# ZrrSkywalker/MonoDETR

Hardware: AMD Instinct MI355X
Metric: training images/sec at B=8 per GPU, KITTI 384x1280 (higher is better)
Workload: dtype bf16; 1 GPU; full MonoDETR training step (ResNet-50 + depth predictor + 3 enc / 3 dec layers, 550 train queries, 4 levels, criterion + AdamW) = BASELINE configs[2] (1 GPU) / configs[3] (DDP); global_batch=8, per_gpu_batch=8, image=3x384x1280, queries=50, precision=bf16, parallelism=dp1, grad_sync=none, prime_steps=12, launch=one hipGraph replay per iteration, cpu_affinity=NUMA node 1 of the GPU

## Files before the change

include/monodetr_amd.h:

```cpp
#ifndef MONODETR_AMD_H
#define MONODETR_AMD_H

#include <stdint.h>

#ifdef __cplusplus
extern "C" {
#endif

#define MDETR_ABI_VERSION 13

#define MDETR_F32 0
#define MDETR_F64 1
#define MDETR_BF16 2

#define MDETR_OK            0
#define MDETR_E_ARG        -1
#define MDETR_E_HIP        -2
#define MDETR_E_ALIGN      -3

int mdetr_abi_version(void);
const char *mdetr_last_error(void);

int mdetr_msda_forward(int dtype,
                       const void *value, const int64_t *spatial_shapes, const int64_t *level_start,
                       const void *loc, const void *attn, void *out,
                       int B, int S, int M, int D, int L, int Lq, int P,
                       int device, void *stream);

int mdetr_msda_backward(int dtype,
                        const void *value, const int64_t *spatial_shapes, const int64_t *level_start,
                        const void *loc, const void *attn, const void *grad_out,
                        void *grad_value, void *grad_loc, void *grad_attn,
                        int B, int S, int M, int D, int L, int Lq, int P,
                        int device, void *stream);

int mdetr_msda_forward_cpu(int dtype,
                           const void *value, const int64_t *spatial_shapes, const int64_t *level_start,
                           const void *loc, const void *attn, void *out,
                           int B, int S, int M, int D, int L, int Lq, int P);
int mdetr_msda_backward_cpu(int dtype,
                            const void *value, const int64_t *spatial_shapes, const int64_t *level_start,
                            const void *loc, const void *attn, const void *grad_out,
                            void *grad_value, void *grad_loc, void *grad_attn,
                            int B, int S, int M, int D, int L, int Lq, int P);

int mdetr_msda_backward_ex(int dtype,
                           const void *value, const int64_t *spatial_shapes, const int64_t *level_start,
                           const void *loc, const void *attn, const void *grad_out,
                           void *grad_value, void *grad_loc, void *grad_attn,
                           int B, int S, int M, int D, int L, int Lq, int P,
                           const int64_t *spatial_shapes_host, const int64_t *level_start_host,
                           void *workspace, int64_t workspace_bytes,
                           int device, void *stream);

int64_t mdetr_msda_backward_workspace_bytes(int dtype, const int64_t *spatial_shapes_host,
                                            const int64_t *level_start_host,
                                            int B, int S, int M, int D, int L, int Lq, int P);

int mdetr_msda_indices(int dtype, const int64_t *spatial_shapes, const void *loc, int32_t *idx,
                       int B, int M, int L, int Lq, int P, int device, void *stream);

int mdetr_msda_variant(int dtype, int M, int D, int L, int P);

int mdetr_attn_forward(int dtype, const void *q, const void *k, const void *v, const uint8_t *key_padding_mask,
                       void *out, float *lse, int B, int H, int Lq, int Lk,
                       int64_t q_bs, int64_t k_bs, int64_t v_bs, int q_rs, int k_rs, int v_rs,
                       float scale, float dropout_p, uint64_t seed, const uint64_t *seed_dev, int device, void *stream);

int mdetr_attn_backward(int dtype, const void *q, const void *k, const void *v, const uint8_t *key_padding_mask,
                        const void *out, const void *d_out, const float *lse, float *dsum,
                        void *dq, void *dk, void *dv, int B, int H, int Lq, int Lk,
                        int64_t q_bs, int64_t k_bs, int64_t v_bs, int q_rs, int k_rs, int v_rs,
                        float scale, float dropout_p, uint64_t seed, const uint64_t *seed_dev, int device, void *stream);

int64_t mdetr_pair_losses_workspace_bytes(int L, int B);
int mdetr_pair_losses_forward(const float *logits, const float *boxes, const float *dims, const float *depths,
                              const float *angles, const int32_t *assign, const int64_t *labels, const float *boxes3d,
                              const float *depth, const float *size3d, const int64_t *heading_bin,
                              const float *heading_res, const uint8_t *valid, const int32_t *num,
                              int L, int B, int Q, int C, int G, int K, float focal_alpha,
                              float num_boxes, const float *num_boxes_dev, float *out, float *comp, void *workspace,
                              int device, void *stream);
int mdetr_pair_losses_backward(const float *logits, const float *boxes, const float *dims, const float *depths,
                               const float *angles, const int32_t *assign, const int64_t *labels, const float *boxes3d,
                               const float *depth, const float *size3d, const int64_t *heading_bin,
                               const float *heading_res, const uint8_t *valid,
                               int L, int B, int Q, int C, int G, int K, float focal_alpha,
                               float num_boxes, const float *num_boxes_dev, const float *grad_out, const float *comp,
                               float *g_logits, float *g_boxes, float *g_dims, float *g_depths, float *g_angles,
                               int device, void *stream);

int mdetr_msda_forward_bf16(const void *value, const int64_t *spatial_shapes, const int64_t *level_start,
                            const float *loc, const float *attn, void *out,
                            int B, int S, int M, int D, int L, int Lq, int P, int device, void *stream);
int mdetr_msda_backward_bf16(const void *value, const int64_t *spatial_shapes, const int64_t *level_start,
                             const float *loc, const float *attn, const void *grad_out,
                             float *grad_value, float *grad_loc, float *grad_attn,
                             int B, int S, int M, int D, int L, int Lq, int P,
                             const int64_t *spatial_shapes_host, const int64_t *level_start_host,
                             void *workspace, int64_t workspace_bytes, int device, void *stream);

int mdetr_msda_prologue_forward(int io_dtype, int ref_dtype, const void *offsets, const void *logits, const void *ref,
                                const int64_t *spatial_shapes, float *sampling_loc, float *attn_weight,
                                int B, int Lq, int M, int L, int P, int R, int64_t ref_sb, int64_t ref_sq, int64_t ref_sl,
                                int device, void *stream);
int mdetr_msda_prologue_backward(int io_dtype, int ref_dtype, const void *offsets, const void *ref, const int64_t *spatial_shapes,
                                 const float *attn_weight, const float *grad_loc, const float *grad_attn,
                                 void *grad_offsets, void *grad_logits, float *grad_ref,
                                 int B, int Lq, int M, int L, int P, int R, int64_t ref_sb, int64_t ref_sq, int64_t ref_sl,
                                 int device, void *stream);
int mdetr_msda_prologue_forward_packed(int io_dtype, int ref_dtype, const void *packed, const void *ref, const int64_t *spatial_shapes,
                                       float *sampling_loc, float *attn_weight, int B, int Lq, int M, int L, int P, int R,
                                       int64_t ref_sb, int64_t ref_sq, int64_t ref_sl, int device, void *stream);
int mdetr_msda_prologue_backward_packed(int io_dtype, int ref_dtype, const void *packed, const void *ref, const int64_t *spatial_shapes,
                                        const float *attn_weight, const float *grad_loc, const float *grad_attn, void *grad_packed,
                                        float *grad_ref, int B, int Lq, int M, int L, int P, int R,
                                        int64_t ref_sb, int64_t ref_sq, int64_t ref_sl, int device, void *stream);

int mdetr_lsa_forward_fused(const float *logits, const float *boxes, const int64_t *labels, const float *boxes3d,
                            const int32_t *num_targets, int32_t *assign, int layers, int images, int groups, int n,
                            int kmax, int num_classes, float w_class, float w_bbox, float w_center, float w_giou,
                            float focal_alpha, int device, void *stream);

int mdetr_ddn_loss_forward(const float *logits, const float *boxes, const float *depth, const uint8_t *valid,
                           int B, int C, int H, int W, int K, int64_t sb, int64_t sc, int64_t sh, int64_t sw,
                           float alpha, float fg_weight, float bg_weight, float depth_min, float depth_max,
                           float *out, void *workspace, int device, void *stream);
int mdetr_ddn_loss_backward(const float *logits, const float *boxes, const float *depth, const uint8_t *valid,
                            int B, int C, int H, int W, int K, int64_t sb, int64_t sc, int64_t sh, int64_t sw,
                            float alpha, float fg_weight, float bg_weight, float depth_min, float depth_max,
                            const float *grad_out, float *grad_logits, int device, void *stream);

int mdetr_adamw_step(int param_dtype, void *param, float *master, const void *grad, float *exp_avg, float *exp_avg_sq,
                     int64_t n, int64_t n_no_decay, float beta1, float beta2, float eps, float weight_decay,
                     float step_size, const float *step_size_dev, int device, void *stream);
int mdetr_adamw_step_counted(int param_dtype, void *param, float *master, const void *grad, float *exp_avg, float *exp_avg_sq,
                             int64_t n, int64_t n_no_decay, float beta1, float beta2, float eps, float weight_decay,
                             const double *step_count_dev, float lr, const double *lr_dev, int device, void *stream);
int mdetr_adamw_step_gathered(int param_dtype, void *param, float *master, const void *const *grad_ptrs, int ntensors,
                              const int *tensor_block_begin, const int64_t *flat_offsets, const int64_t *nbytes, const int *block_tensor,
                              const int64_t *block_start, int chunk_bytes, float *exp_avg, float *exp_avg_sq, int64_t n_no_decay,
                              float beta1, float beta2, float eps, float weight_decay, float step_size, const float *step_size_dev,
                              const double *step_count_dev, float lr, const double *lr_dev, int device, void *stream);

#define MDETR_TGEMM_RELU 1
#define MDETR_TGEMM_NN 2
#define MDETR_TGEMM_BIAS_F32 4
#define MDETR_TGEMM_OUT_F32 8
int mdetr_tgemm(const void *a, const void *w, const void *bias, const void *res, void *y, int64_t T, int N, int K,
                int64_t lda, int64_t ldw, int64_t ldr, int64_t ldy, int flags, float dropout_p, uint64_t seed,
                const void *seed_dev, int device, void *stream);
int mdetr_tgemm_masked(const void *a, const void *w, const void *res, const void *mask, void *y, int64_t T, int N, int K,
                       int64_t lda, int64_t ldw, int64_t ldr, int64_t ldm, int64_t ldy, int device, void *stream);
int mdetr_tgemm_f32(const void *a, const void *w, const void *bias, const void *res, void *y, int64_t T, int N, int K,
                    int64_t lda, int64_t ldw, int64_t ldr, int64_t ldy, int flags, float dropout_p, uint64_t seed,
                    const void *seed_dev, int device, void *stream);
int mdetr_tgemm_f32_masked(const void *a, const void *w, const void *res, const void *mask, void *y, int64_t T, int N, int K,
                           int64_t lda, int64_t ldw, int64_t ldr, int64_t ldm, int64_t ldy, int device, void *stream);

#define MDETR_SGEMM_NT 0
#define MDETR_SGEMM_NN 1
#define MDETR_SGEMM_TN 2
#define MDETR_SGEMM_MAX_PROBLEMS 10
#define MDETR_SGEMM_MAX_TERMS 5
typedef struct {
    const void *a, *b;
    int64_t lda, ldb;
    int32_t k, a_dtype, b_dtype, pad_;
} mdetr_sgemm_term;
typedef struct {
    mdetr_sgemm_term term[MDETR_SGEMM_MAX_TERMS];
    void *c;
    const float *bias;
    float *colsum;
    const float *mask;
    const void *res;
    int64_t ldc, ldm, ldr;
    int32_t nterm, m, n, relu_cols, c_dtype, res_dtype;
} mdetr_sgemm_problem;
int64_t mdetr_sgemm_workspace_bytes(int mode, const mdetr_sgemm_problem *problems, int nprob);
int mdetr_sgemm_grouped(int mode, const mdetr_sgemm_problem *problems, int nprob, void *workspace, int64_t workspace_bytes, int device, void *stream);

#define MDETR_KITTI_FLIP 1u
#define MDETR_KITTI_DISTORT 2u
#define MDETR_KITTI_CONTRAST_FIRST 4u
#define MDETR_KITTI_BRIGHTNESS 8u
#define MDETR_KITTI_CONTRAST 16u
#define MDETR_KITTI_SATURATION 32u
#define MDETR_KITTI_HUE 64u
typedef struct MdetrKittiImage {
    int64_t pixel_offset;
    int32_t width, height;
    uint32_t flags;
    uint32_t perm;
    float brightness, contrast, saturation, hue;
    double inv[6];
} MdetrKittiImage;
int mdetr_kitti_preprocess(const uint8_t *pixels, const MdetrKittiImage *images, int n_images, void *out,
                           int out_dtype, int out_h, int out_w, int channels_last, const float *mean, const float *std,
                           int device, void *stream);

int mdetr_rotate_iou_eval(const float *boxes, const float *qboxes, const int64_t *box_start, const int64_t *qbox_start,
                          const int64_t *out_start, int n_frames, int64_t total_pairs, int criterion, float *out,
                          int device, void *stream);
int mdetr_box3d_overlap_eval(const double *boxes, const double *qboxes, const int64_t *box_start, const int64_t *qbox_start,
                             const int64_t *out_start, int n_frames, int64_t total_pairs, int criterion, double *out,
                             int device, void *stream);
int mdetr_kitti_pr_curve(const double *overlaps, const int64_t *ov_start, const double *gt_datas, const double *dt_datas,
                         const int64_t *gt_start, const int64_t *dt_start, const int64_t *ignored_gt,
                         const int64_t *ignored_det, const double *dontcares, const int64_t *dc_start, int n_frames,
                         int metric, double min_overlap, int64_t num_valid_gt, int compute_aos, int max_thresholds,
                         double *pr, double *thresholds, int *n_thresholds);

int mdetr_add_layernorm_forward(int io_dtype, int param_dtype, const void *a, const void *b, const void *gamma, const void *beta, void *y,
                                void *s, float *stats, int64_t rows, int cols, float eps, float dropout_p, uint64_t seed,
                                const uint64_t *seed_dev, int device, void *stream);
int64_t mdetr_add_layernorm_partial_rows(int64_t rows);
int mdetr_add_layernorm_backward(int io_dtype, int param_dtype, const void *dy, const void *s, const void *gamma, const float *stats,
                                 void *da, void *db, float *partial, int64_t rows, int cols, float dropout_p,
                                 uint64_t seed, const uint64_t *seed_dev, int device, void *stream);

int64_t mdetr_column_sum_workspace_bytes(int64_t rows, int cols);
int mdetr_column_sum(int dtype, const void *x, float *out, void *workspace, int64_t workspace_bytes,
                     int64_t rows, int cols, int64_t ld, int device, void *stream);
int mdetr_box_refine(const float *delta, const float *ref, float *out, int64_t rows, int nd, int device, void *stream);
int mdetr_head_tail_forward(const float *delta, const float *init_ref, const float *inter_refs, const float *size3d, const float *depth_reg,
                            const float *depth_map, const float *img_h, const float *focal, float *coord, float *depth_ave,
                            int L, int B, int Q, int nd0, int H, int W, int device, void *stream);
int mdetr_head_tail_backward(const float *init_ref, const float *size3d, const float *depth_reg, const float *img_h, const float *focal,
                             const float *coord, const float *g_coord, const float *g_depth, float *g_delta, float *g_init_ref,
                             float *g_size3d, float *g_depth_reg, float *g_map, int L, int B, int Q, int nd0, int H, int W, int device, void *stream);

typedef struct {
    const float *part;
    void *out;
    int64_t cols;
    int32_t chunks, out_dtype;
} mdetr_chunk_job;
int mdetr_chunk_sums(const mdetr_chunk_job *jobs, int njobs, int device, void *stream);
int mdetr_column_sum_to(int dtype, const void *x, void *out, int out_dtype, void *workspace, int64_t workspace_bytes,
                        int64_t rows, int cols, int64_t ld, int device, void *stream);

int mdetr_conv3x3_forward(const void *x, const void *w, const float *shift, void *y, int B, int H, int W, int C, int N,
                          int relu, int device, void *stream);
int mdetr_conv3x3_plan(int B, int H, int W, int N);
int mdetr_conv3x3_masked(const void *x, const void *w, const float *shift, const void *mask, void *y, int B, int H, int W, int C, int N,
                         int relu, int device, void *stream);

int mdetr_conv_taps(const void *x, const void *w, const float *shift, void *y, const int64_t *dims, int relu, int device, void *stream);

int mdetr_conv_taps_split(const void *x, const void *w, const float *shift, float *partial, int64_t partial_floats, const int64_t *dims,
                          int ksplit, int device, void *stream);

int mdetr_conv_dgrad_s2(const void *dy, const void *wt, void *dx, int B, int OH, int OW, int N, int H, int W, int C, int K, int device, void *stream);

int mdetr_conv_stem(const void *x, const void *w_packed, const float *shift, void *y, int B, int H, int W, int device, void *stream);

int mdetr_conv_wgrad_chunks(int B, int H, int W, int C, int OH, int OW, int N, int K, int SI);
int mdetr_conv_wgrad(const void *x, const void *dy, float *partial, int64_t partial_floats, int B, int H, int W, int C, int OH, int OW, int N,
                     int K, int SI, int device, void *stream);

int mdetr_token_wgrad_chunks(int64_t T, int C, int N);
int mdetr_token_wgrad(const void *x, const void *dy, float *partial, int64_t partial_floats, int64_t T, int C, int N, int with_bias,
                      int device, void *stream);

int mdetr_bias_act_forward(int io_dtype, int bias_dtype, const void *x, const void *bias, const void *skip, void *y,
                           int64_t rows, int cols, int relu, float dropout_p, uint64_t seed, const uint64_t *seed_dev,
                           int device, void *stream);
int mdetr_bias_act_backward(int io_dtype, const void *dy, const void *y, void *dx, int64_t rows, int cols, float scale,
                            int device, void *stream);

int mdetr_fold_weights(int n, const void *const *w, const void *const *scale, void *const *folded, void *const *folded_t,
                       const int *O, const int *C, const int *taps, int device, void *stream);
int mdetr_unfold_grads(int n, const void *const *dfolded, const void *const *scale, void *const *dw,
                       const int *O, const int *C, const int *taps, int device, void *stream);

int mdetr_gather_flat(const void *const *src_ptrs, int ntensors, const int *tensor_block_begin, void *dst, const int64_t *dst_offsets,
                      const int64_t *nbytes, const int *block_tensor, const int64_t *block_start, int chunk_bytes, int device, void *stream);

int mdetr_maxpool3x3s2_bf16(const void *x, void *y, int B, int H, int W, int C, int device, void *stream);
int mdetr_decimate2(int backward, const void *src, void *dst, int B, int H, int W, int64_t pixel_bytes, int device, void *stream);

int64_t mdetr_small_wgrad_workspace_bytes(int64_t rows, int n, int k);
int mdetr_small_wgrad(int io_dtype, const void *dy, const void *x, void *out, int out_dtype, void *workspace, int64_t workspace_bytes,
                      int64_t rows, int n, int k, int64_t ldy, int64_t ldx, int device, void *stream);

int64_t mdetr_group_norm_workspace_bytes(int n, int64_t hw, int c, int groups);
int mdetr_group_norm_forward(int io_dtype, int param_dtype, const void *x, const void *gamma, const void *beta, void *y, float *stats,
                             void *workspace, int64_t workspace_bytes, int n, int64_t hw, int c, int groups, float eps, int relu,
                             int device, void *stream);
int mdetr_group_norm_backward(int io_dtype, int param_dtype, const void *dy, const void *x, const void *gamma, const void *beta,
                              const float *stats, void *dx, void *dparams, void *workspace, int64_t workspace_bytes,
                              int n, int64_t hw, int c, int groups, int relu, int device, void *stream);

int mdetr_lsa_forward(const float *cost, const int32_t *num_targets, int32_t *assign,
                      int layers, int images, int groups, int n, int kmax,
                      int64_t img_stride, int64_t q_stride, int64_t t_stride, int device, void *stream);

int mdetr_profile_enable(int on);
int mdetr_profile_read(double *rows, int cap);
int mdetr_profile_read_work(double *rows, int cap);

#ifdef __cplusplus
}
#endif
#endif
```

monodetr_amd/_capi.py:

```python
import ctypes
import os
import threading

_HERE = os.path.dirname(os.path.abspath(__file__))
LIB_PATH = os.environ.get("MDETR_LIB_PATH") or os.path.join(_HERE, "libmonodetr_amd.so")

MDETR_F32, MDETR_F64, MDETR_BF16 = 0, 1, 2
ABI_VERSION = 13

_c_int, _c_vp = ctypes.c_int, ctypes.c_void_p

SIGNATURES = {
    "mdetr_abi_version": (_c_int, []),
    "mdetr_last_error": (ctypes.c_char_p, []),
    "mdetr_msda_variant": (_c_int, [_c_int] * 5),
    "mdetr_msda_forward": (_c_int, [_c_int] + [_c_vp] * 6 + [_c_int] * 7 + [_c_int, _c_vp]),
    "mdetr_msda_backward": (_c_int, [_c_int] + [_c_vp] * 9 + [_c_int] * 7 + [_c_int, _c_vp]),
    "mdetr_msda_forward_cpu": (_c_int, [_c_int] + [_c_vp] * 6 + [_c_int] * 7),
    "mdetr_msda_backward_cpu": (_c_int, [_c_int] + [_c_vp] * 9 + [_c_int] * 7),
    "mdetr_msda_backward_ex": (_c_int, [_c_int] + [_c_vp] * 9 + [_c_int] * 7 + [_c_vp, _c_vp, _c_vp, ctypes.c_int64] + [_c_int, _c_vp]),
    "mdetr_msda_backward_workspace_bytes": (ctypes.c_int64, [_c_int, _c_vp, _c_vp] + [_c_int] * 7),
    "mdetr_msda_indices": (_c_int, [_c_int] + [_c_vp] * 3 + [_c_int] * 5 + [_c_int, _c_vp]),
    "mdetr_attn_forward": (_c_int, [_c_int] + [_c_vp] * 6 + [_c_int] * 4 + [ctypes.c_int64] * 3 + [_c_int] * 3
                           + [ctypes.c_float, ctypes.c_float, ctypes.c_uint64, _c_vp, _c_int, _c_vp]),
    "mdetr_attn_backward": (_c_int, [_c_int] + [_c_vp] * 11 + [_c_int] * 4 + [ctypes.c_int64] * 3 + [_c_int] * 3
                            + [ctypes.c_float, ctypes.c_float, ctypes.c_uint64, _c_vp, _c_int, _c_vp]),
    "mdetr_lsa_forward": (_c_int, [_c_vp] * 3 + [_c_int] * 5 + [ctypes.c_int64] * 3 + [_c_int, _c_vp]),
    "mdetr_ddn_loss_forward": (_c_int, [_c_vp] * 4 + [_c_int] * 5 + [ctypes.c_int64] * 4 + [ctypes.c_float] * 5 + [_c_vp, _c_vp, _c_int, _c_vp]),
    "mdetr_ddn_loss_backward": (_c_int, [_c_vp] * 4 + [_c_int] * 5 + [ctypes.c_int64] * 4 + [ctypes.c_float] * 5 + [_c_vp, _c_vp, _c_int, _c_vp]),
    "mdetr_pair_losses_workspace_bytes": (ctypes.c_int64, [_c_int, _c_int]),
    "mdetr_pair_losses_forward": (_c_int, [_c_vp] * 14 + [_c_int] * 6 + [ctypes.c_float, ctypes.c_float] + [_c_vp] * 4 + [_c_int, _c_vp]),
    "mdetr_pair_losses_backward": (_c_int, [_c_vp] * 13 + [_c_int] * 6 + [ctypes.c_float, ctypes.c_float] + [_c_vp] * 8 + [_c_int, _c_vp]),
    "mdetr_adamw_step": (_c_int, [_c_int] + [_c_vp] * 5 + [ctypes.c_int64] * 2 + [ctypes.c_float] * 5 + [_c_vp, _c_int, _c_vp]),
    "mdetr_adamw_step_gathered": (_c_int, [_c_int, _c_vp, _c_vp, _c_vp, _c_int] + [_c_vp] * 5 + [_c_int, _c_vp, _c_vp, ctypes.c_int64] + [ctypes.c_float] * 5
                                  + [_c_vp, _c_vp, ctypes.c_float, _c_vp, _c_int, _c_vp]),
    "mdetr_adamw_step_counted": (_c_int, [_c_int] + [_c_vp] * 5 + [ctypes.c_int64] * 2 + [ctypes.c_float] * 4 + [_c_vp, ctypes.c_float, _c_vp, _c_int, _c_vp]),
    "mdetr_tgemm": (_c_int, [_c_vp] * 5 + [ctypes.c_int64, _c_int, _c_int] + [ctypes.c_int64] * 4 + [_c_int, ctypes.c_float, ctypes.c_uint64, _c_vp, _c_int, _c_vp]),
    "mdetr_sgemm_workspace_bytes": (ctypes.c_int64, [_c_int, _c_vp, _c_int]),
    "mdetr_sgemm_grouped": (_c_int, [_c_int, _c_vp, _c_int, _c_vp, ctypes.c_int64, _c_int, _c_vp]),
    "mdetr_tgemm_masked": (_c_int, [_c_vp] * 5 + [ctypes.c_int64, _c_int, _c_int] + [ctypes.c_int64] * 5 + [_c_int, _c_vp]),
    "mdetr_tgemm_f32": (_c_int, [_c_vp] * 5 + [ctypes.c_int64, _c_int, _c_int] + [ctypes.c_int64] * 4 + [_c_int, ctypes.c_float, ctypes.c_uint64, _c_vp, _c_int, _c_vp]),
    "mdetr_tgemm_f32_masked": (_c_int, [_c_vp] * 5 + [ctypes.c_int64, _c_int, _c_int] + [ctypes.c_int64] * 5 + [_c_int, _c_vp]),
    "mdetr_column_sum_workspace_bytes": (ctypes.c_int64, [ctypes.c_int64, _c_int]),
    "mdetr_column_sum": (_c_int, [_c_int, _c_vp, _c_vp, _c_vp, ctypes.c_int64, ctypes.c_int64, _c_int, ctypes.c_int64, _c_int, _c_vp]),
    "mdetr_box_refine": (_c_int, [_c_vp] * 3 + [ctypes.c_int64, _c_int, _c_int, _c_vp]),
    "mdetr_head_tail_forward": (_c_int, [_c_vp] * 10 + [_c_int] * 6 + [_c_int, _c_vp]),
    "mdetr_head_tail_backward": (_c_int, [_c_vp] * 13 + [_c_int] * 6 + [_c_int, _c_vp]),
    "mdetr_chunk_sums": (_c_int, [_c_vp, _c_int, _c_int, _c_vp]),
    "mdetr_column_sum_to": (_c_int, [_c_int, _c_vp, _c_vp, _c_int, _c_vp, ctypes.c_int64, ctypes.c_int64, _c_int, ctypes.c_int64, _c_int, _c_vp]),
    "mdetr_add_layernorm_forward": (_c_int, [_c_int, _c_int] + [_c_vp] * 7 + [ctypes.c_int64, _c_int, ctypes.c_float, ctypes.c_float, ctypes.c_uint64, _c_vp, _c_int, _c_vp]),
    "mdetr_add_layernorm_partial_rows": (ctypes.c_int64, [ctypes.c_int64]),
    "mdetr_add_layernorm_backward": (_c_int, [_c_int, _c_int] + [_c_vp] * 7 + [ctypes.c_int64, _c_int, ctypes.c_float, ctypes.c_uint64, _c_vp, _c_int, _c_vp]),
    "mdetr_conv3x3_forward": (_c_int, [_c_vp] * 4 + [_c_int] * 6 + [_c_int, _c_vp]),
    "mdetr_conv3x3_plan": (_c_int, [_c_int] * 4),
    "mdetr_conv3x3_masked": (_c_int, [_c_vp] * 5 + [_c_int] * 6 + [_c_int, _c_vp]),
    "mdetr_conv_taps": (_c_int, [_c_vp] * 5 + [_c_int, _c_int, _c_vp]),
    "mdetr_conv_taps_split": (_c_int, [_c_vp] * 4 + [ctypes.c_int64, _c_vp, _c_int, _c_int, _c_vp]),
    "mdetr_conv_dgrad_s2": (_c_int, [_c_vp] * 3 + [_c_int] * 8 + [_c_int, _c_vp]),
    "mdetr_conv_stem": (_c_int, [_c_vp] * 4 + [_c_int] * 3 + [_c_int, _c_vp]),
    "mdetr_conv_wgrad_chunks": (_c_int, [_c_int] * 9),
    "mdetr_conv_wgrad": (_c_int, [_c_vp] * 3 + [ctypes.c_int64] + [_c_int] * 9 + [_c_int, _c_vp]),
    "mdetr_token_wgrad_chunks": (_c_int, [ctypes.c_int64, _c_int, _c_int]),
    "mdetr_token_wgrad": (_c_int, [_c_vp, _c_vp, _c_vp, ctypes.c_int64, ctypes.c_int64, _c_int, _c_int, _c_int, _c_int, _c_vp]),
    "mdetr_small_wgrad_workspace_bytes": (ctypes.c_int64, [ctypes.c_int64, _c_int, _c_int]),
    "mdetr_small_wgrad": (_c_int, [_c_int, _c_vp, _c_vp, _c_vp, _c_int, _c_vp, ctypes.c_int64, ctypes.c_int64, _c_int, _c_int, ctypes.c_int64, ctypes.c_int64, _c_int, _c_vp]),
    "mdetr_group_norm_workspace_bytes": (ctypes.c_int64, [_c_int, ctypes.c_int64, _c_int, _c_int]),
    "mdetr_group_norm_forward": (_c_int, [_c_int, _c_int] + [_c_vp] * 6 + [ctypes.c_int64, _c_int, ctypes.c_int64, _c_int, _c_int, ctypes.c_float, _c_int, _c_int, _c_vp]),
    "mdetr_group_norm_backward": (_c_int, [_c_int, _c_int] + [_c_vp] * 8 + [ctypes.c_int64, _c_int, ctypes.c_int64, _c_int, _c_int, _c_int, _c_int, _c_vp]),
    "mdetr_bias_act_forward": (_c_int, [_c_int, _c_int] + [_c_vp] * 4 + [ctypes.c_int64, _c_int, _c_int, ctypes.c_float, ctypes.c_uint64, _c_vp, _c_int, _c_vp]),
    "mdetr_bias_act_backward": (_c_int, [_c_int] + [_c_vp] * 3 + [ctypes.c_int64, _c_int, ctypes.c_float, _c_int, _c_vp]),
    "mdetr_rotate_iou_eval": (_c_int, [_c_vp] * 5 + [_c_int, ctypes.c_int64, _c_int, _c_vp, _c_int, _c_vp]),
    "mdetr_box3d_overlap_eval": (_c_int, [_c_vp] * 5 + [_c_int, ctypes.c_int64, _c_int, _c_vp, _c_int, _c_vp]),
    "mdetr_kitti_pr_curve": (_c_int, [_c_vp] * 10 + [_c_int, _c_int, ctypes.c_double, ctypes.c_int64, _c_int, _c_int, _c_vp, _c_vp, _c_vp]),
    "mdetr_kitti_preprocess": (_c_int, [_c_vp, _c_vp, _c_int, _c_vp, _c_int, _c_int, _c_int, _c_int, _c_vp, _c_vp, _c_int, _c_vp]),
    "mdetr_msda_forward_bf16": (_c_int, [_c_vp] * 6 + [_c_int] * 7 + [_c_int, _c_vp]),
    "mdetr_msda_backward_bf16": (_c_int, [_c_vp] * 9 + [_c_int] * 7 + [_c_vp, _c_vp, _c_vp, ctypes.c_int64, _c_int, _c_vp]),
    "mdetr_msda_prologue_forward": (_c_int, [_c_int, _c_int] + [_c_vp] * 6 + [_c_int] * 6 + [ctypes.c_int64] * 3 + [_c_int, _c_vp]),
    "mdetr_gather_flat": (_c_int, [_c_vp, _c_int] + [_c_vp] * 6 + [_c_int, _c_int, _c_vp]),
    "mdetr_fold_weights": (_c_int, [_c_int] + [_c_vp] * 7 + [_c_int, _c_vp]),
    "mdetr_unfold_grads": (_c_int, [_c_int] + [_c_vp] * 6 + [_c_int, _c_vp]),
    "mdetr_maxpool3x3s2_bf16": (_c_int, [_c_vp, _c_vp, _c_int, _c_int, _c_int, _c_int, _c_int, _c_vp]),
    "mdetr_decimate2": (_c_int, [_c_int, _c_vp, _c_vp, _c_int, _c_int, _c_int, ctypes.c_int64, _c_int, _c_vp]),
    "mdetr_msda_prologue_forward_packed": (_c_int, [_c_int, _c_int] + [_c_vp] * 5 + [_c_int] * 6 + [ctypes.c_int64] * 3 + [_c_int, _c_vp]),
    "mdetr_msda_prologue_backward_packed": (_c_int, [_c_int, _c_int] + [_c_vp] * 8 + [_c_int] * 6 + [ctypes.c_int64] * 3 + [_c_int, _c_vp]),
    "mdetr_msda_prologue_backward": (_c_int, [_c_int, _c_int] + [_c_vp] * 9 + [_c_int] * 6 + [ctypes.c_int64] * 3 + [_c_int, _c_vp]),
    "mdetr_lsa_forward_fused": (_c_int, [_c_vp] * 6 + [_c_int] * 6 + [ctypes.c_float] * 5 + [_c_int, _c_vp]),
    "mdetr_profile_enable": (_c_int, [_c_int]),
    "mdetr_profile_read": (_c_int, [_c_vp, _c_int]),
    "mdetr_profile_read_work": (_c_int, [_c_vp, _c_int]),
}

_lib = None
_lock = threading.Lock()


def lib():
    global _lib
    if _lib is None:
        with _lock:
            if _lib is None:
                if not os.path.exists(LIB_PATH):
                    raise RuntimeError(
                        "monodetr_amd: %s is missing -- the HIP extension is not built. Run "
                        "`python -m monodetr_amd.build` (needs hipcc). There is no CPU/PyTorch fallback." % LIB_PATH)
                handle = ctypes.CDLL(LIB_PATH)
                for name, (res, args) in SIGNATURES.items():
                    fn = getattr(handle, name)
                    fn.restype, fn.argtypes = res, args
                got = handle.mdetr_abi_version()
                if got != ABI_VERSION:
                    raise RuntimeError("monodetr_amd: ABI version mismatch (lib %d, python %d); rebuild" % (got, ABI_VERSION))
                _lib = handle
    return _lib


def check(rc, what):
    if rc != 0:
        msg = lib().mdetr_last_error()
        raise RuntimeError("%s failed (code %d): %s" % (what, rc, msg.decode() if msg else "?"))


def dtype_code(t):
    import torch
    if t.dtype == torch.float32:
        return MDETR_F32
    if t.dtype == torch.float64:
        return MDETR_F64
    raise RuntimeError('"ms_deform_attn" not implemented for \'%s\'' % str(t.dtype).replace("torch.", ""))


def profile_enable(on):
    check(lib().mdetr_profile_enable(1 if on else 0), "mdetr_profile_enable")


def profile_read(cap=64):
    buf = (ctypes.c_double * (4 * cap))()
    n = lib().mdetr_profile_read(ctypes.cast(buf, ctypes.c_void_p), cap)
    if n < 0:
        check(n, "mdetr_profile_read")
    return [(int(buf[4 * i]), int(buf[4 * i + 1]), int(buf[4 * i + 2]), float(buf[4 * i + 3])) for i in range(n)]


def profile_read_work(cap=256):
    buf = (ctypes.c_double * (6 * cap))()
    n = lib().mdetr_profile_read_work(ctypes.cast(buf, ctypes.c_void_p), cap)
    if n < 0:
        check(n, "mdetr_profile_read_work")
    return [(int(buf[6 * i]), int(buf[6 * i + 1]), int(buf[6 * i + 2]), float(buf[6 * i + 3]), float(buf[6 * i + 4]), float(buf[6 * i + 5])) for i in range(n)]
```

monodetr_amd/add_ln_ext.py:

```python
import os

import torch
import torch.nn.functional as F

from . import _capi
from .attn_ext import _next_seed

_backend = None
ENABLED = os.environ.get("MDETR_FUSED_LN") == "1"


_seed_counter = None


def _host_seed():
    global _seed_counter
    if _seed_counter is None:
        _seed_counter = int(torch.randint(0, 2 ** 62, (1,), dtype=torch.int64))
    _seed_counter = (_seed_counter + 0x9E3779B97F4A7C15) & 0x7FFFFFFFFFFFFFFF
    return _seed_counter


def _lib():
    return _backend if _backend is not None else _capi.lib()


def supported(a, b, norm):
    return ((a.is_cuda or _backend is not None) and a.dtype in (torch.float32, torch.bfloat16) and b.dtype == a.dtype
            and a.shape == b.shape and a.shape[-1] in (128, 256, 512) and len(norm.normalized_shape) == 1
            and norm.normalized_shape[0] == a.shape[-1] and norm.elementwise_affine and norm.bias is not None)


def _rows(t, C):
    t = t.reshape(-1, C).contiguous()
    return t if t.data_ptr() % 16 == 0 else t.clone()


def _dev(t):
    cuda = t.is_cuda
    return (t.device.index if cuda else -1), (torch.cuda.current_stream(t.device).cuda_stream if cuda else None)


def _column_sum_f32(x, out_dtype=torch.float32):
    if x.is_cuda and _backend is None:
        from .colsum_ext import column_sum
        return column_sum(x, out_dtype if out_dtype in (torch.float32, torch.bfloat16) else torch.float32)
    return x.sum(0).to(out_dtype)


class _AddLayerNorm(torch.autograd.Function):
    @staticmethod
    def forward(ctx, a, b, gamma, beta, eps, p, seed, seed_dev):
        shape = a.shape
        C = shape[-1]
        a2, b2 = _rows(a, C), _rows(b, C)
        rows = a2.shape[0]
        if gamma.dtype == beta.dtype and gamma.dtype in (torch.float32, torch.bfloat16):
            gp, bp = gamma.contiguous(), beta.contiguous()
        else:
            gp, bp = gamma.float().contiguous(), beta.float().contiguous()
        pcode = _capi.MDETR_BF16 if gp.dtype == torch.bfloat16 else _capi.MDETR_F32
        y, s = torch.empty_like(a2), torch.empty_like(a2)
        stats = torch.empty((rows, 2), dtype=torch.float32, device=a.device)
        io = _capi.MDETR_BF16 if a.dtype == torch.bfloat16 else _capi.MDETR_F32
        dev, stream = _dev(a2)
        rc = _lib().mdetr_add_layernorm_forward(io, pcode, a2.data_ptr(), b2.data_ptr(), gp.data_ptr(), bp.data_ptr(), y.data_ptr(), s.data_ptr(),
                                                stats.data_ptr(), rows, C, float(eps), float(p), int(seed),
                                                seed_dev.data_ptr() if seed_dev is not None else None, dev, stream)
        if rc != 0:
            _capi.check(rc, "mdetr_add_layernorm_forward")
        ctx.save_for_backward(s, gp, stats)
        ctx.seed_dev = seed_dev
        ctx.meta = (io, pcode, rows, C, float(p), int(seed), shape, gamma.dtype, beta.dtype)
        return y.view(shape)

    @staticmethod
    @torch.autograd.function.once_differentiable
    def backward(ctx, dy):
        s, gp, stats = ctx.saved_tensors
        io, pcode, rows, C, p, seed, shape, g_dtype, b_dtype = ctx.meta
        dy2 = _rows(dy, C)
        da, db = torch.empty_like(s), torch.empty_like(s)
        lib = _lib()
        nb = lib.mdetr_add_layernorm_partial_rows(rows)
        partial = torch.empty((nb, 2 * C), dtype=torch.float32, device=s.device)
        dev, stream = _dev(s)
        rc = lib.mdetr_add_layernorm_backward(io, pcode, dy2.data_ptr(), s.data_ptr(), gp.data_ptr(), stats.data_ptr(), da.data_ptr(), db.data_ptr(),
                                              partial.data_ptr(), rows, C, p, seed,
                                              ctx.seed_dev.data_ptr() if ctx.seed_dev is not None else None, dev, stream)
        if rc != 0:
            _capi.check(rc, "mdetr_add_layernorm_backward")
        sums = _column_sum_f32(partial, g_dtype if g_dtype == b_dtype else torch.float32)
        return da.view(shape), db.view(shape), sums[:C].to(g_dtype), sums[C:].to(b_dtype), None, None, None, None


def fused_add_layernorm(a, b, gamma, beta, eps=1e-5, dropout_p=0.0, seed=None):
    seed_dev = None
    if dropout_p > 0.0 and seed is None:
        if a.is_cuda and torch.cuda.is_current_stream_capturing():
            from .attn_ext import site_seed
            seed, seed_dev = site_seed(a.device)
        else:
            seed = _host_seed()
    return _AddLayerNorm.apply(a, b, gamma, beta, eps, dropout_p, seed or 0, seed_dev)


def residual_layernorm(a, b, norm, dropout):
    if ENABLED and supported(a, b, norm):
        p = dropout.p if (dropout is not None and dropout.training) else 0.0
        return fused_add_layernorm(a, b, norm.weight, norm.bias, norm.eps, p)
    return norm(a + (dropout(b) if dropout is not None else b))
```

monodetr_amd/csrc/add_ln.hip:

```cpp
#include <hip/hip_runtime.h>
#include <hip/hip_bf16.h>
#include <stdint.h>

#include "add_ln.h"
#include "add_ln_math.h"

namespace mdetr {
namespace {

constexpr int kWavesLn = 4;
constexpr int kMaxBwdBlocks = 1024;

template <typename T> __device__ __forceinline__ float ld1(const T *p);
template <> __device__ __forceinline__ float ld1<float>(const float *p) { return *p; }
template <> __device__ __forceinline__ float ld1<__hip_bfloat16>(const __hip_bfloat16 *p) { return __bfloat162float(*p); }
template <typename T> __device__ __forceinline__ void st1(T *p, float v);
template <> __device__ __forceinline__ void st1<float>(float *p, float v) { *p = v; }
template <> __device__ __forceinline__ void st1<__hip_bfloat16>(__hip_bfloat16 *p, float v) { *p = __float2bfloat16(v); }

template <typename T, int E> struct alignas(sizeof(T) * E > 16 ? 16 : sizeof(T) * E) RowVec { T v[E]; };

template <typename T, int E> __device__ __forceinline__ void load_row(const T *p, float (&v)[E])
{
    const RowVec<T, E> t = *reinterpret_cast<const RowVec<T, E> *>(p);
#pragma unroll
    for (int i = 0; i < E; ++i) v[i] = ld1<T>(&t.v[i]);
}
template <typename T, int E> __device__ __forceinline__ void store_row(T *p, const float (&v)[E])
{
    RowVec<T, E> t;
#pragma unroll
    for (int i = 0; i < E; ++i) st1<T>(&t.v[i], v[i]);
    *reinterpret_cast<RowVec<T, E> *>(p) = t;
}

__device__ __forceinline__ float wave_sum(float v)
{
#pragma unroll
    for (int o = 32; o > 0; o >>= 1) v += __shfl_xor(v, o);
    return v;
}

template <typename T, typename PT, int E>
__global__ __launch_bounds__(kWavesLn * 64)
void add_ln_fwd_kernel(const T *__restrict__ a, const T *__restrict__ b, const PT *__restrict__ gamma,
                       const PT *__restrict__ beta, T *__restrict__ y, T *__restrict__ s, float *__restrict__ stats,
                       int64_t rows, float eps, uint32_t thresh, float keep_scale, uint64_t seed,
                       const uint64_t *__restrict__ seed_dev)
{
    constexpr int C = 64 * E;
    const int lane = threadIdx.x & 63, wave = threadIdx.x >> 6;
    const int64_t row = static_cast<int64_t>(blockIdx.x) * kWavesLn + wave;
    if (row >= rows) return;
    const uint64_t sd = seed + (seed_dev ? *seed_dev : 0ull);
    const int64_t at = row * C + lane * E;
    float v[E];
    load_row<T, E>(a + at, v);
    if (b) {
        float r[E];
        load_row<T, E>(b + at, r);
#pragma unroll
        for (int i = 0; i < E; ++i) {
            const bool keep = thresh == 0u || ln_hash(sd, static_cast<uint64_t>(at + i)) >= thresh;
            v[i] += keep ? r[i] * keep_scale : 0.f;
        }
        if (s) {
            store_row<T, E>(s + at, v);
#pragma unroll
            for (int i = 0; i < E; ++i) { T t; st1<T>(&t, v[i]); v[i] = ld1<T>(&t); }
        }
    }
    float sum = 0.f;
#pragma unroll
    for (int i = 0; i < E; ++i) sum += v[i];
    const float mean = wave_sum(sum) * (1.0f / C);
    float sq = 0.f;
#pragma unroll
    for (int i = 0; i < E; ++i) { const float d = v[i] - mean; sq += d * d; }
    const float rstd = 1.0f / sqrtf(wave_sum(sq) * (1.0f / C) + eps);
    float o[E];
#pragma unroll
    for (int i = 0; i < E; ++i) o[i] = (v[i] - mean) * rstd * ld1<PT>(gamma + lane * E + i) + ld1<PT>(beta + lane * E + i);
    store_row<T, E>(y + at, o);
    if (lane == 0) { stats[2 * row] = mean; stats[2 * row + 1] = rstd; }
}

template <typename T, typename PT, int E>
__global__ __launch_bounds__(kWavesLn * 64)
void add_ln_bwd_kernel(const T *__restrict__ dy, const T *__restrict__ s, const PT *__restrict__ gamma,
                       const float *__restrict__ stats, T *__restrict__ da, T *__restrict__ db,
                       float *__restrict__ partial, int64_t rows, uint32_t thresh, float keep_scale, uint64_t seed,
                       const uint64_t *__restrict__ seed_dev)
{
    constexpr int C = 64 * E;
    __shared__ float red[kWavesLn][2 * C];
    const int lane = threadIdx.x & 63, wave = threadIdx.x >> 6;
    const uint64_t sd = seed + (seed_dev ? *seed_dev : 0ull);
    float g[E], acc_g[E], acc_b[E];
#pragma unroll
    for (int i = 0; i < E; ++i) { g[i] = ld1<PT>(gamma + lane * E + i); acc_g[i] = 0.f; acc_b[i] = 0.f; }
    for (int64_t row = static_cast<int64_t>(blockIdx.x) * kWavesLn + wave; row < rows; row += static_cast<int64_t>(gridDim.x) * kWavesLn) {
        const int64_t at = row * C + lane * E;
        const float mean = stats[2 * row], rstd = stats[2 * row + 1];
        float d[E], x[E];
        load_row<T, E>(dy + at, d);
        load_row<T, E>(s + at, x);
        float s1 = 0.f, s2 = 0.f;
#pragma unroll
        for (int i = 0; i < E; ++i) {
            x[i] = (x[i] - mean) * rstd;
            acc_g[i] += d[i] * x[i];
            acc_b[i] += d[i];
            d[i] *= g[i];
            s1 += d[i];
            s2 += d[i] * x[i];
        }
        s1 = wave_sum(s1) * (1.0f / C);
        s2 = wave_sum(s2) * (1.0f / C);
        float o[E];
#pragma unroll
        for (int i = 0; i < E; ++i) o[i] = rstd * (d[i] - s1 - x[i] * s2);
        store_row<T, E>(da + at, o);
        if (db) {
#pragma unroll
            for (int i = 0; i < E; ++i) {
                const bool keep = thresh == 0u || ln_hash(sd, static_cast<uint64_t>(at + i)) >= thresh;
                o[i] = keep ? o[i] * keep_scale : 0.f;
            }
            store_row<T, E>(db + at, o);
        }
    }
#pragma unroll
    for (int i = 0; i < E; ++i) { red[wave][lane * E + i] = acc_g[i]; red[wave][C + lane * E + i] = acc_b[i]; }
    __syncthreads();
    for (int c = threadIdx.x; c < 2 * C; c += kWavesLn * 64)
        partial[static_cast<int64_t>(blockIdx.x) * 2 * C + c] = red[0][c] + red[1][c] + red[2][c] + red[3][c];
}

template <typename T, typename PT, int E>
hipError_t launch_fwd(const AddLnProblem &p, const void *a, const void *b, const void *gamma, const void *beta, void *y, void *s,
                      float *stats, hipStream_t st)
{
    const uint32_t thresh = b ? ln_threshold(p.dropout_p) : 0u;
    const float scale = p.dropout_p > 0.f ? 1.0f / (1.0f - p.dropout_p) : 1.0f;
    hipLaunchKernelGGL((add_ln_fwd_kernel<T, PT, E>), dim3(static_cast<unsigned>((p.rows + kWavesLn - 1) / kWavesLn)), dim3(kWavesLn * 64), 0, st,
                       static_cast<const T *>(a), static_cast<const T *>(b), static_cast<const PT *>(gamma), static_cast<const PT *>(beta),
                       static_cast<T *>(y), static_cast<T *>(s), stats,
                       p.rows, p.eps, thresh, scale, p.seed, p.seed_dev);
    return hipGetLastError();
}

template <typename T, typename PT, int E>
hipError_t launch_bwd(const AddLnProblem &p, const void *dy, const void *s, const void *gamma, const float *stats, void *da, void *db,
                      float *partial, hipStream_t st)
{
    const uint32_t thresh = db ? ln_threshold(p.dropout_p) : 0u;
    const float scale = p.dropout_p > 0.f ? 1.0f / (1.0f - p.dropout_p) : 1.0f;
    hipLaunchKernelGGL((add_ln_bwd_kernel<T, PT, E>), dim3(static_cast<unsigned>(add_ln_partial_rows(p.rows))), dim3(kWavesLn * 64), 0, st,
                       static_cast<const T *>(dy), static_cast<const T *>(s), static_cast<const PT *>(gamma), stats, static_cast<T *>(da),
                       static_cast<T *>(db), partial,
                       p.rows, thresh, scale, p.seed, p.seed_dev);
    return hipGetLastError();
}

}

int64_t add_ln_partial_rows(int64_t rows)
{
    const int64_t blocks = (rows + kWavesLn - 1) / kWavesLn;
    return blocks < 1 ? 1 : (blocks > kMaxBwdBlocks ? kMaxBwdBlocks : blocks);
}

template <int E>
hipError_t dispatch_fwd(const AddLnProblem &p, const void *a, const void *b, const void *gamma, const void *beta, void *y, void *s,
                        float *stats, hipStream_t st)
{
    using BF = __hip_bfloat16;
    if (p.io_dtype == 2) return p.param_dtype == 2 ? launch_fwd<BF, BF, E>(p, a, b, gamma, beta, y, s, stats, st) : launch_fwd<BF, float, E>(p, a, b, gamma, beta, y, s, stats, st);
    return p.param_dtype == 2 ? launch_fwd<float, BF, E>(p, a, b, gamma, beta, y, s, stats, st) : launch_fwd<float, float, E>(p, a, b, gamma, beta, y, s, stats, st);
}

template <int E>
hipError_t dispatch_bwd(const AddLnProblem &p, const void *dy, const void *s, const void *gamma, const float *stats, void *da, void *db,
                        float *partial, hipStream_t st)
{
    using BF = __hip_bfloat16;
    if (p.io_dtype == 2) return p.param_dtype == 2 ? launch_bwd<BF, BF, E>(p, dy, s, gamma, stats, da, db, partial, st) : launch_bwd<BF, float, E>(p, dy, s, gamma, stats, da, db, partial, st);
    return p.param_dtype == 2 ? launch_bwd<float, BF, E>(p, dy, s, gamma, stats, da, db, partial, st) : launch_bwd<float, float, E>(p, dy, s, gamma, stats, da, db, partial, st);
}

hipError_t add_ln_forward_launch(const AddLnProblem &p, const void *a, const void *b, const void *gamma, const void *beta,
                                 void *y, void *s, float *stats, hipStream_t st)
{
    if (p.rows == 0) return hipSuccess;
    switch (p.cols) {
    case 128: return dispatch_fwd<2>(p, a, b, gamma, beta, y, s, stats, st);
    case 256: return dispatch_fwd<4>(p, a, b, gamma, beta, y, s, stats, st);
    case 512: return dispatch_fwd<8>(p, a, b, gamma, beta, y, s, stats, st);
    default: return hipErrorNotSupported;
    }
}

hipError_t add_ln_backward_launch(const AddLnProblem &p, const void *dy, const void *s, const void *gamma, const float *stats,
                                  void *da, void *db, float *partial, hipStream_t st)
{
    if (p.rows == 0) return hipSuccess;
    switch (p.cols) {
    case 128: return dispatch_bwd<2>(p, dy, s, gamma, stats, da, db, partial, st);
    case 256: return dispatch_bwd<4>(p, dy, s, gamma, stats, da, db, partial, st);
    case 512: return dispatch_bwd<8>(p, dy, s, gamma, stats, da, db, partial, st);
    default: return hipErrorNotSupported;
    }
}

}
```

monodetr_amd/csrc/add_ln_math.h:

```cpp
#pragma once
#include <stdint.h>

#if defined(__HIPCC__)
#define MDETR_HD __host__ __device__ __forceinline__
#else
#define MDETR_HD inline
#endif

namespace mdetr {

MDETR_HD uint32_t ln_hash(uint64_t seed, uint64_t index)
{
    uint64_t z = index * 0x9E3779B97F4A7C15ull + seed;
    uint32_t x = static_cast<uint32_t>(z) ^ static_cast<uint32_t>(z >> 32);
    x ^= x >> 16;
    x *= 0x7FEB352Du;
    x ^= x >> 15;
    x *= 0x846CA68Bu;
    x ^= x >> 16;
    return x;
}

MDETR_HD uint32_t ln_threshold(float p)
{
    const double t = static_cast<double>(p) * 4294967296.0;
    return t >= 4294967295.0 ? 0xFFFFFFFFu : static_cast<uint32_t>(t);
}

}
```

monodetr_amd/csrc/capi.hip:

```cpp
#include <hip/hip_runtime.h>
#include <stdarg.h>
#include <stdio.h>

#include <atomic>
#include <map>
#include <mutex>
#include <utility>
#include <vector>

#include "../../include/monodetr_amd.h"
#include "attn.h"
#include "adamw.h"
#include "add_ln.h"
#include "bias_act.h"
#include "colsum.h"
#include "group_norm.h"
#include "small_wgrad.h"
#include "decimate.h"
#include "wfold.h"
#include "conv3x3.h"
#include "conv_stem.h"
#include "conv_taps.h"
#include "conv_wgrad.h"
#include "ddn_loss.h"
// ... 394 lines not shown
{
    if (int rc = pair_losses_args("mdetr_pair_losses_backward", L, B, Q, C, G, K)) return rc;
    if (!logits || !boxes || !dims || !depths || !angles || !assign || !labels || !boxes3d || !depth || !size3d ||
        !heading_bin || !heading_res || !valid || !grad_out || !comp || !g_logits || !g_boxes || !g_dims || !g_depths || !g_angles)
        return fail(MDETR_E_ARG, "mdetr_pair_losses_backward: null pointer");
    DeviceScope dev(device);
    if (dev.err != hipSuccess) return fail(MDETR_E_HIP, "mdetr_pair_losses_backward: set device %d: %s", device, hipGetErrorString(dev.err));
    const mdetr::PairLossDims d{L, B, Q, C, G, K, focal_alpha};
    const mdetr::PairLossIn in{logits, boxes, dims, depths, angles, assign, reinterpret_cast<const long long *>(labels),
                               reinterpret_cast<const long long *>(heading_bin), boxes3d, depth, size3d, heading_res, valid};
    const hipError_t e = mdetr::pair_losses_backward_launch(d, in, grad_out, comp, num_boxes, num_boxes_dev, g_logits,
                                                            g_boxes, g_dims, g_depths, g_angles,
                                                            static_cast<hipStream_t>(stream));
    if (e != hipSuccess) return fail(MDETR_E_HIP, "mdetr_pair_losses_backward: launch failed: %s", hipGetErrorString(e));
    return MDETR_OK;
}

int mdetr_adamw_step(int param_dtype, void *param, float *master, const void *grad, float *exp_avg, float *exp_avg_sq,
                     int64_t n, int64_t n_no_decay, float beta1, float beta2, float eps, float weight_decay,
                     float step_size, const float *step_size_dev, int device, void *stream)
{
    if (param_dtype != MDETR_F32 && param_dtype != MDETR_BF16)
        return fail(MDETR_E_ARG, "mdetr_adamw_step: parameter dtype must be f32 or bf16");
    if (n < 0 || n_no_decay < 0 || n_no_decay > n) return fail(MDETR_E_ARG, "mdetr_adamw_step: bad sizes");
    if (n == 0) return MDETR_OK;
    if (!param || !master || !grad || !exp_avg || !exp_avg_sq) return fail(MDETR_E_ARG, "mdetr_adamw_step: null pointer");
    if (param_dtype == MDETR_F32 && static_cast<void *>(master) != param)
        return fail(MDETR_E_ARG, "mdetr_adamw_step: an f32 parameter is its own master copy");
    if (!aligned16(param) || !aligned16(master) || !aligned16(grad) || !aligned16(exp_avg) || !aligned16(exp_avg_sq))
        return fail(MDETR_E_ALIGN, "mdetr_adamw_step: buffers must be 16-byte aligned");
    DeviceScope dev(device);
    if (dev.err != hipSuccess) return fail(MDETR_E_HIP, "mdetr_adamw_step: set device %d: %s", device, hipGetErrorString(dev.err));
    const hipError_t e = mdetr::adamw_launch(param_dtype, param, master, grad, exp_avg, exp_avg_sq, n, n_no_decay,
                                             beta1, beta2, eps, weight_decay, step_size, step_size_dev,
                                             static_cast<hipStream_t>(stream));
    if (e != hipSuccess) return fail(MDETR_E_HIP, "mdetr_adamw_step: launch failed: %s", hipGetErrorString(e));
    return MDETR_OK;
}

int mdetr_adamw_step_counted(int param_dtype, void *param, float *master, const void *grad, float *exp_avg, float *exp_avg_sq,
                             int64_t n, int64_t n_no_decay, float beta1, float beta2, float eps, float weight_decay,
                             const double *step_count_dev, float lr, const double *lr_dev, int device, void *stream)
{
    if (param_dtype != MDETR_F32 && param_dtype != MDETR_BF16)
        return fail(MDETR_E_ARG, "mdetr_adamw_step_counted: parameter dtype must be f32 or bf16");
    if (n < 0 || n_no_decay < 0 || n_no_decay > n) return fail(MDETR_E_ARG, "mdetr_adamw_step_counted: bad sizes");
    if (n == 0) return MDETR_OK;
    if (!param || !master || !grad || !exp_avg || !exp_avg_sq || !step_count_dev) return fail(MDETR_E_ARG, "mdetr_adamw_step_counted: null pointer");
    if (param_dtype == MDETR_F32 && static_cast<void *>(master) != param)
        return fail(MDETR_E_ARG, "mdetr_adamw_step_counted: an f32 parameter is its own master copy");
    if (!aligned16(param) || !aligned16(master) || !aligned16(grad) || !aligned16(exp_avg) || !aligned16(exp_avg_sq))
        return fail(MDETR_E_ALIGN, "mdetr_adamw_step_counted: buffers must be 16-byte aligned");
    DeviceScope dev(device);
    if (dev.err != hipSuccess) return fail(MDETR_E_HIP, "mdetr_adamw_step_counted: set device %d: %s", device, hipGetErrorString(dev.err));
    const hipError_t e = mdetr::adamw_launch(param_dtype, param, master, grad, exp_avg, exp_avg_sq, n, n_no_decay, beta1, beta2, eps,
                                             weight_decay, 0.f, nullptr, static_cast<hipStream_t>(stream), step_count_dev, lr_dev, lr);
    if (e != hipSuccess) return fail(MDETR_E_HIP, "mdetr_adamw_step_counted: launch failed: %s", hipGetErrorString(e));
    return MDETR_OK;
}

int mdetr_adamw_step_gathered(int param_dtype, void *param, float *master, const void *const *grad_ptrs, int ntensors,
                              const int *tensor_block_begin, const int64_t *flat_offsets, const int64_t *nbytes, const int *block_tensor,
                              const int64_t *block_start, int chunk_bytes, float *exp_avg, float *exp_avg_sq, int64_t n_no_decay,
                              float beta1, float beta2, float eps, float weight_decay, float step_size, const float *step_size_dev,
                              const double *step_count_dev, float lr, const double *lr_dev, int device, void *stream)
{
    if (param_dtype != MDETR_F32 && param_dtype != MDETR_BF16)
        return fail(MDETR_E_ARG, "mdetr_adamw_step_gathered: parameter dtype must be f32 or bf16");
    const int esz = param_dtype == MDETR_F32 ? 4 : 2;
    if (ntensors < 0 || n_no_decay < 0 || chunk_bytes <= 0 || chunk_bytes % 16 != 0)
        return fail(MDETR_E_ARG, "mdetr_adamw_step_gathered: ntensors %d / chunk_bytes %d (a positive multiple of 16)", ntensors, chunk_bytes);
    if (ntensors == 0) return MDETR_OK;
    if (!param || !master || !grad_ptrs || !tensor_block_begin || !flat_offsets || !nbytes || !block_tensor || !block_start || !exp_avg || !exp_avg_sq)
        return fail(MDETR_E_ARG, "mdetr_adamw_step_gathered: null pointer");
    if (param_dtype == MDETR_F32 && static_cast<void *>(master) != param)
        return fail(MDETR_E_ARG, "mdetr_adamw_step_gathered: an f32 parameter is its own master copy");
    if (!aligned16(param) || !aligned16(master) || !aligned16(exp_avg) || !aligned16(exp_avg_sq))
        return fail(MDETR_E_ALIGN, "mdetr_adamw_step_gathered: buffers must be 16-byte aligned");
    for (int i = 0; i < ntensors; ++i)
        if ((!grad_ptrs[i] && tensor_block_begin[i + 1] != tensor_block_begin[i]) || tensor_block_begin[i + 1] < tensor_block_begin[i] ||
            (reinterpret_cast<uintptr_t>(grad_ptrs[i]) & (esz - 1)))
            return fail(MDETR_E_ARG, "mdetr_adamw_step_gathered: tensor %d: null / misaligned gradient or decreasing block table", i);
    DeviceScope dev(device);
    if (dev.err != hipSuccess) return fail(MDETR_E_HIP, "mdetr_adamw_step_gathered: set device %d: %s", device, hipGetErrorString(dev.err));
    const hipError_t e = mdetr::adamw_gathered_launch(param_dtype, param, master, grad_ptrs, ntensors, tensor_block_begin, flat_offsets, nbytes, block_tensor,
                                                      block_start, chunk_bytes, exp_avg, exp_avg_sq, n_no_decay, beta1, beta2, eps, weight_decay,
                                                      step_size, step_size_dev, static_cast<hipStream_t>(stream), step_count_dev, lr_dev, lr);
    if (e != hipSuccess) return fail(MDETR_E_HIP, "mdetr_adamw_step_gathered: launch failed: %s", hipGetErrorString(e));
    return MDETR_OK;
}

int mdetr_tgemm(const void *a, const void *w, const void *bias, const void *res, void *y, int64_t T, int N, int K,
                int64_t lda, int64_t ldw, int64_t ldr, int64_t ldy, int flags, float dropout_p, uint64_t seed,
                const void *seed_dev, int device, void *stream)
{
    if (T < 0 || N <= 0 || K <= 0) return fail(MDETR_E_ARG, "mdetr_tgemm: bad shape T=%lld N=%d K=%d", static_cast<long long>(T), N, K);
    if (T == 0) return MDETR_OK;
    if (!a || !w || !y) return fail(MDETR_E_ARG, "mdetr_tgemm: null pointer");
    if (flags & ~(MDETR_TGEMM_RELU | MDETR_TGEMM_NN | MDETR_TGEMM_BIAS_F32 | MDETR_TGEMM_OUT_F32)) return fail(MDETR_E_ARG, "mdetr_tgemm: unknown flag bits 0x%x", flags);
    if (dropout_p > 0.f && !(flags & MDETR_TGEMM_RELU)) return fail(MDETR_E_ARG, "mdetr_tgemm: dropout is only fused behind the ReLU");
    mdetr::TgemmProblem p{a, w, bias, res, y, T, N, K, lda, ldw, res ? ldr : 0, ldy, flags, dropout_p, seed, static_cast<const uint64_t *>(seed_dev)};
    if (!mdetr::tgemm_supported(p))
        return fail(MDETR_E_ARG, "mdetr_tgemm: needs bf16 operands, K %% 8 == 0, N %% 8 == 0, row strides %% 8 == 0 and >= the row length, 16-byte aligned "
                    "pointers, 0 <= dropout_p < 1 (T=%lld N=%d K=%d lda=%lld ldw=%lld ldr=%lld ldy=%lld flags=0x%x)", static_cast<long long>(T), N, K,
                    static_cast<long long>(lda), static_cast<long long>(ldw), static_cast<long long>(ldr), static_cast<long long>(ldy), flags);
    DeviceScope dev(device);
    if (dev.err != hipSuccess) return fail(MDETR_E_HIP, "mdetr_tgemm: set device %d: %s", device, hipGetErrorString(dev.err));
    const hipError_t e = mdetr::tgemm_launch(p, static_cast<hipStream_t>(stream));
    if (e != hipSuccess) return fail(MDETR_E_HIP, "mdetr_tgemm: launch failed: %s", hipGetErrorString(e));
    return MDETR_OK;
}

int64_t mdetr_sgemm_workspace_bytes(int mode, const mdetr_sgemm_problem *problems, int nprob)
{
    const char *why = mdetr::sgemm_check(mode, problems, nprob);
    if (why) return fail(MDETR_E_ARG, "mdetr_sgemm_workspace_bytes: %s (mode %d, %d problems)", why, mode, nprob);
    return mdetr::sgemm_workspace_bytes(mode, problems, nprob);
}

int mdetr_sgemm_grouped(int mode, const mdetr_sgemm_problem *problems, int nprob, void *workspace, int64_t workspace_bytes, int device, void *stream)
{
    const char *why = mdetr::sgemm_check(mode, problems, nprob);
    if (why) return fail(MDETR_E_ARG, "mdetr_sgemm_grouped: %s (mode %d, %d problems)", why, mode, nprob);
    const int64_t need = mdetr::sgemm_workspace_bytes(mode, problems, nprob);
    if (need > 0 && (!workspace || workspace_bytes < need || !aligned16(workspace)))
        return fail(MDETR_E_ARG, "mdetr_sgemm_grouped: needs a 16-byte aligned workspace of %lld bytes (mdetr_sgemm_workspace_bytes), got %lld",
                    static_cast<long long>(need), static_cast<long long>(workspace ? workspace_bytes : 0));
    DeviceScope dev(device);
    if (dev.err != hipSuccess) return fail(MDETR_E_HIP, "mdetr_sgemm_grouped: set device %d: %s", device, hipGetErrorString(dev.err));
    const hipError_t e = mdetr::sgemm_launch(mode, problems, nprob, workspace, static_cast<hipStream_t>(stream));
    if (e != hipSuccess) return fail(MDETR_E_HIP, "mdetr_sgemm_grouped: launch failed: %s", hipGetErrorString(e));
    return MDETR_OK;
}

int mdetr_tgemm_masked(const void *a, const void *w, const void *res, const void *mask, void *y, int64_t T, int N, int K,
                       int64_t lda, int64_t ldw, int64_t ldr, int64_t ldm, int64_t ldy, int device, void *stream)
{
    if (T < 0 || N <= 0 || K <= 0) return fail(MDETR_E_ARG, "mdetr_tgemm_masked: bad shape T=%lld N=%d K=%d", static_cast<long long>(T), N, K);
    if (T == 0) return MDETR_OK;
    if (!a || !w || !y || !mask) return fail(MDETR_E_ARG, "mdetr_tgemm_masked: null pointer");
    mdetr::TgemmProblem p{a, w, nullptr, res, y, T, N, K, lda, ldw, res ? ldr : 0, ldy, MDETR_TGEMM_NN, 0.f, 0, nullptr};
    p.mask = mask; p.ldm = ldm;
    if (!mdetr::tgemm_supported(p))
        return fail(MDETR_E_ARG, "mdetr_tgemm_masked: needs bf16 operands, K %% 8 == 0, N %% 8 == 0, row strides %% 8 == 0 and >= the row length, 16-byte "
                    "aligned pointers (T=%lld N=%d K=%d lda=%lld ldw=%lld ldr=%lld ldm=%lld ldy=%lld)", static_cast<long long>(T), N, K,
                    static_cast<long long>(lda), static_cast<long long>(ldw), static_cast<long long>(ldr), static_cast<long long>(ldm), static_cast<long long>(ldy));
    DeviceScope dev(device);
    if (dev.err != hipSuccess) return fail(MDETR_E_HIP, "mdetr_tgemm_masked: set device %d: %s", device, hipGetErrorString(dev.err));
    const hipError_t e = mdetr::tgemm_launch(p, static_cast<hipStream_t>(stream));
    if (e != hipSuccess) return fail(MDETR_E_HIP, "mdetr_tgemm_masked: launch failed: %s", hipGetErrorString(e));
    return MDETR_OK;
}

int mdetr_tgemm_f32(const void *a, const void *w, const void *bias, const void *res, void *y, int64_t T, int N, int K,
                    int64_t lda, int64_t ldw, int64_t ldr, int64_t ldy, int flags, float dropout_p, uint64_t seed,
                    const void *seed_dev, int device, void *stream)
{
    if (T < 0 || N <= 0 || K <= 0) return fail(MDETR_E_ARG, "mdetr_tgemm_f32: bad shape T=%lld N=%d K=%d", static_cast<long long>(T), N, K);
    if (T == 0) return MDETR_OK;
    if (!a || !w || !y) return fail(MDETR_E_ARG, "mdetr_tgemm_f32: null pointer");
    if (flags & ~(MDETR_TGEMM_RELU | MDETR_TGEMM_NN | MDETR_TGEMM_BIAS_F32 | MDETR_TGEMM_OUT_F32)) return fail(MDETR_E_ARG, "mdetr_tgemm_f32: unknown flag bits 0x%x", flags);
    if (dropout_p > 0.f && !(flags & MDETR_TGEMM_RELU)) return fail(MDETR_E_ARG, "mdetr_tgemm_f32: dropout is only fused behind the ReLU");
    mdetr::TgemmProblem p{a, w, bias, res, y, T, N, K, lda, ldw, res ? ldr : 0, ldy, flags & (MDETR_TGEMM_RELU | MDETR_TGEMM_NN), dropout_p, seed,
                          static_cast<const uint64_t *>(seed_dev)};
    p.f32 = true;
    if (!mdetr::tgemm_supported(p))
        return fail(MDETR_E_ARG, "mdetr_tgemm_f32: needs fp32 operands, K %% 8 == 0, N %% 8 == 0, row strides %% 4 == 0 and >= the row length, 16-byte aligned "
                    "pointers, tensors below 2^31 bytes, 0 <= dropout_p < 1 (T=%lld N=%d K=%d lda=%lld ldw=%lld ldr=%lld ldy=%lld flags=0x%x)",
                    static_cast<long long>(T), N, K, static_cast<long long>(lda), static_cast<long long>(ldw), static_cast<long long>(ldr),
                    static_cast<long long>(ldy), flags);
    DeviceScope dev(device);
    if (dev.err != hipSuccess) return fail(MDETR_E_HIP, "mdetr_tgemm_f32: set device %d: %s", device, hipGetErrorString(dev.err));
    const hipError_t e = mdetr::tgemm_launch(p, static_cast<hipStream_t>(stream));
    if (e != hipSuccess) return fail(MDETR_E_HIP, "mdetr_tgemm_f32: launch failed: %s", hipGetErrorString(e));
    return MDETR_OK;
}

int mdetr_tgemm_f32_masked(const void *a, const void *w, const void *res, const void *mask, void *y, int64_t T, int N, int K,
                           int64_t lda, int64_t ldw, int64_t ldr, int64_t ldm, int64_t ldy, int device, void *stream)
{
    if (T < 0 || N <= 0 || K <= 0) return fail(MDETR_E_ARG, "mdetr_tgemm_f32_masked: bad shape T=%lld N=%d K=%d", static_cast<long long>(T), N, K);
    if (T == 0) return MDETR_OK;
    if (!a || !w || !y || !mask) return fail(MDETR_E_ARG, "mdetr_tgemm_f32_masked: null pointer");
    mdetr::TgemmProblem p{a, w, nullptr, res, y, T, N, K, lda, ldw, res ? ldr : 0, ldy, MDETR_TGEMM_NN, 0.f, 0, nullptr};
    p.mask = mask; p.ldm = ldm; p.f32 = true;
    if (!mdetr::tgemm_supported(p))
        return fail(MDETR_E_ARG, "mdetr_tgemm_f32_masked: needs fp32 operands, K %% 8 == 0, N %% 8 == 0, row strides %% 4 == 0 and >= the row length, 16-byte "
                    "aligned pointers, tensors below 2^31 bytes (T=%lld N=%d K=%d lda=%lld ldw=%lld ldr=%lld ldm=%lld ldy=%lld)", static_cast<long long>(T), N, K,
                    static_cast<long long>(lda), static_cast<long long>(ldw), static_cast<long long>(ldr), static_cast<long long>(ldm), static_cast<long long>(ldy));
    DeviceScope dev(device);
    if (dev.err != hipSuccess) return fail(MDETR_E_HIP, "mdetr_tgemm_f32_masked: set device %d: %s", device, hipGetErrorString(dev.err));
    const hipError_t e = mdetr::tgemm_launch(p, static_cast<hipStream_t>(stream));
    if (e != hipSuccess) return fail(MDETR_E_HIP, "mdetr_tgemm_f32_masked: launch failed: %s", hipGetErrorString(e));
    return MDETR_OK;
}

int64_t mdetr_column_sum_workspace_bytes(int64_t rows, int cols)
{
    if (rows < 0 || cols < 0) return -1;
    return mdetr::colsum_workspace_bytes(rows, cols);
}

static int column_sum_impl(const char *who, int dtype, const void *x, void *out, int out_dtype, void *workspace, int64_t workspace_bytes,
                           int64_t rows, int cols, int64_t ld, int device, void *stream)
{
    if (rows < 0 || cols < 0 || ld < cols) return fail(MDETR_E_ARG, "%s: bad shape rows=%lld cols=%d ld=%lld", who,
                                                      static_cast<long long>(rows), cols, static_cast<long long>(ld));
    if (out_dtype != MDETR_F32 && out_dtype != MDETR_BF16) return fail(MDETR_E_ARG, "%s: out_dtype must be MDETR_F32 or MDETR_BF16", who);
    if (cols == 0) return MDETR_OK;
    if (!out || !workspace || (rows > 0 && !x)) return fail(MDETR_E_ARG, "%s: null pointer", who);
    if (!mdetr::colsum_supported(dtype, cols, ld, x))
        return fail(MDETR_E_ARG, "%s: needs f32 (cols %% 4 == 0) or bf16 (cols %% 8 == 0), 16-byte aligned rows", who);
    if (workspace_bytes < mdetr::colsum_workspace_bytes(rows, cols))
        return fail(MDETR_E_ARG, "%s: workspace too small", who);
    DeviceScope dev(device);
    if (dev.err != hipSuccess) return fail(MDETR_E_HIP, "%s: set device %d: %s", who, device, hipGetErrorString(dev.err));
    mdetr::ProfileScope prof(12, cols, static_cast<hipStream_t>(stream), 0.0, static_cast<double>(rows) * cols * (dtype == MDETR_BF16 ? 2.0 : 4.0) / 1e3);
    const hipError_t e = mdetr::colsum_launch(dtype, x, out, workspace, rows, cols, ld, static_cast<hipStream_t>(stream), out_dtype);
    if (e != hipSuccess) return fail(MDETR_E_HIP, "%s: launch failed: %s", who, hipGetErrorString(e));
    return MDETR_OK;
}

int mdetr_column_sum(int dtype, const void *x, float *out, void *workspace, int64_t workspace_bytes,
                     int64_t rows, int cols, int64_t ld, int device, void *stream)
{
    return column_sum_impl("mdetr_column_sum", dtype, x, out, MDETR_F32, workspace, workspace_bytes, rows, cols, ld, device, stream);
}

int mdetr_column_sum_to(int dtype, const void *x, void *out, int out_dtype, void *workspace, int64_t workspace_bytes,
                        int64_t rows, int cols, int64_t ld, int device, void *stream)
{
    return column_sum_impl("mdetr_column_sum_to", dtype, x, out, out_dtype, workspace, workspace_bytes, rows, cols, ld, device, stream);
}

int mdetr_box_refine(const float *delta, const float *ref, float *out, int64_t rows, int nd, int device, void *stream)
{
    if (rows < 0 || (nd != 2 && nd != 6)) return fail(MDETR_E_ARG, "mdetr_box_refine: bad sizes rows=%lld nd=%d (2 or 6)", static_cast<long long>(rows), nd);
    if (rows == 0) return MDETR_OK;
    if (!delta || !ref || !out) return fail(MDETR_E_ARG, "mdetr_box_refine: null pointer");
    DeviceScope dev(device);
    if (dev.err != hipSuccess) return fail(MDETR_E_HIP, "mdetr_box_refine: set device %d: %s", device, hipGetErrorString(dev.err));
    const hipError_t e = mdetr::box_refine_launch(delta, ref, out, rows, nd, static_cast<hipStream_t>(stream));
    if (e != hipSuccess) return fail(MDETR_E_HIP, "mdetr_box_refine: launch failed: %s", hipGetErrorString(e));
    return MDETR_OK;
}

static int head_tail_dims(const char *who, int L, int B, int Q, int nd0, int H, int W, mdetr::HeadTailDims *d)
{
    if (L <= 0 || B <= 0 || Q <= 0 || H <= 0 || W <= 0 || (nd0 != 2 && nd0 != 6) || static_cast<int64_t>(L) * B * Q * 6 >= (1ll << 31))
        return fail(MDETR_E_ARG, "%s: bad sizes L=%d B=%d Q=%d nd0=%d H=%d W=%d", who, L, B, Q, nd0, H, W);
    d->L = L; d->B = B; d->Q = Q; d->nd0 = nd0; d->H = H; d->W = W;
    return MDETR_OK;
}

int mdetr_head_tail_forward(const float *delta, const float *init_ref, const float *inter_refs, const float *size3d, const float *depth_reg,
                            const float *depth_map, const float *img_h, const float *focal, float *coord, float *depth_ave,
                            int L, int B, int Q, int nd0, int H, int W, int device, void *stream)
{
    mdetr::HeadTailDims d;
    if (int rc = head_tail_dims("mdetr_head_tail_forward", L, B, Q, nd0, H, W, &d)) return rc;
    if (!delta || !init_ref || (L > 1 && !inter_refs) || !size3d || !depth_reg || !depth_map || !img_h || !focal || !coord || !depth_ave)
        return fail(MDETR_E_ARG, "mdetr_head_tail_forward: null pointer");
    DeviceScope dev(device);
    if (dev.err != hipSuccess) return fail(MDETR_E_HIP, "mdetr_head_tail_forward: set device %d: %s", device, hipGetErrorString(dev.err));
    const hipError_t e = mdetr::head_tail_forward_launch(d, delta, init_ref, inter_refs, size3d, depth_reg, depth_map, img_h, focal, coord, depth_ave,
                                                         static_cast<hipStream_t>(stream));
    if (e != hipSuccess) return fail(MDETR_E_HIP, "mdetr_head_tail_forward: launch failed: %s", hipGetErrorString(e));
    return MDETR_OK;
}

int mdetr_head_tail_backward(const float *init_ref, const float *size3d, const float *depth_reg, const float *img_h, const float *focal,
                             const float *coord, const float *g_coord, const float *g_depth, float *g_delta, float *g_init_ref,
                             float *g_size3d, float *g_depth_reg, float *g_map, int L, int B, int Q, int nd0, int H, int W, int device, void *stream)
{
    mdetr::HeadTailDims d;
    if (int rc = head_tail_dims("mdetr_head_tail_backward", L, B, Q, nd0, H, W, &d)) return rc;
    if (!init_ref || !size3d || !depth_reg || !img_h || !focal || !coord || !g_delta || !g_init_ref || !g_size3d || !g_depth_reg)
        return fail(MDETR_E_ARG, "mdetr_head_tail_backward: null pointer");
    DeviceScope dev(device);
    if (dev.err != hipSuccess) return fail(MDETR_E_HIP, "mdetr_head_tail_backward: set device %d: %s", device, hipGetErrorString(dev.err));
    const hipError_t e = mdetr::head_tail_backward_launch(d, init_ref, size3d, depth_reg, img_h, focal, coord, g_coord, g_depth, g_delta, g_init_ref,
                                                          g_size3d, g_depth_reg, g_map, static_cast<hipStream_t>(stream));
    if (e != hipSuccess) return fail(MDETR_E_HIP, "mdetr_head_tail_backward: launch failed: %s", hipGetErrorString(e));
    return MDETR_OK;
}

int mdetr_chunk_sums(const mdetr_chunk_job *jobs, int njobs, int device, void *stream)
{
    if (njobs == 0) return MDETR_OK;
    const char *why = mdetr::chunk_sums_check(jobs, njobs);
    if (why) return fail(MDETR_E_ARG, "mdetr_chunk_sums: %s (%d jobs)", why, njobs);
    DeviceScope dev(device);
    if (dev.err != hipSuccess) return fail(MDETR_E_HIP, "mdetr_chunk_sums: set device %d: %s", device, hipGetErrorString(dev.err));
    double kb = 0.0;
    for (int i = 0; i < njobs; ++i) kb += (static_cast<double>(jobs[i].chunks) * jobs[i].cols * 4.0 + jobs[i].cols * (jobs[i].out_dtype == 2 ? 2.0 : 4.0)) / 1e3;
    mdetr::ProfileScope prof(12, njobs, static_cast<hipStream_t>(stream), 0.0, kb);
    const hipError_t e = mdetr::chunk_sums_launch(jobs, njobs, static_cast<hipStream_t>(stream));
    if (e != hipSuccess) return fail(MDETR_E_HIP, "mdetr_chunk_sums: launch failed: %s", hipGetErrorString(e));
    return MDETR_OK;
}

static int conv3x3_any(const char *who, const void *x, const void *w, const float *shift, const void *mask, void *y, int B, int H, int W, int C, int N,
                       int relu, int device, void *stream)
{
    if (B < 0 || H < 0 || W < 0 || C <= 0 || N <= 0) return fail(MDETR_E_ARG, "%s: bad sizes B=%d H=%d W=%d C=%d N=%d", who, B, H, W, C, N);
    if (B == 0 || H == 0 || W == 0) return MDETR_OK;
// ... 686 lines not shown
```

monodetr_amd/csrc/tgemm.h:

```cpp
#pragma once
#include <hip/hip_runtime.h>
#include <stdint.h>

namespace mdetr {

constexpr int kTgemmRelu = 1, kTgemmNN = 2, kTgemmBiasF32 = 4, kTgemmOutF32 = 8;

struct TgemmProblem {
    const void *a;
    const void *w;
    const void *bias;
    const void *res;
    void *y;
    int64_t T;
    int N, K;
    int64_t lda, ldw, ldr, ldy;
    int flags;
    float dropout_p;
    uint64_t seed;
    const uint64_t *seed_dev;
    const void *mask = nullptr;
    int64_t ldm = 0;
    bool f32 = false;
};

bool tgemm_supported(const TgemmProblem &p);
hipError_t tgemm_launch(const TgemmProblem &p, hipStream_t st);

}
```

monodetr_amd/csrc/tgemm.hip:

```cpp
#include <hip/hip_runtime.h>
#include <stdint.h>
#include <stdio.h>
#include <stdlib.h>
#include <string.h>

#include <mdetr_wave.h>

#include "add_ln_math.h"
#include "mdetr_transpose.h"
#include "msda.h"
#include "tgemm.h"
#include "mdetr_tune.h"

namespace mdetr {
namespace {

constexpr int kThreadsT = 256;
constexpr int kBK = 64;
constexpr int kLd = kBK + 8;
constexpr int kCPad = 4;

struct TgemmArgs {
    const __bf16 *a, *w, *res, *mask;
    const void *bias;
    void *y;
    int64_t T, lda, ldw, ldr, ldy, ldm;
    int N, K, gx, ny, flags, tiles_m;
    uint32_t thresh;
    float keep_scale;
    uint64_t seed;
    const uint64_t *seed_dev;
};

template <int BM, int BN>
constexpr size_t tgemm_lds()
{
    constexpr size_t slabs = static_cast<size_t>(2) * (BM + BN) * kLd * 2, tile = static_cast<size_t>(BM) * (BN + kCPad) * 4;
    return slabs > tile ? slabs : tile;
}

__device__ __forceinline__ void transpose4x8(const bf16x8 (&in)[4], unsigned (&out)[8][2])
{
    unsigned d[4][4];
#pragma unroll
    for (int i = 0; i < 4; ++i) __builtin_memcpy(d[i], &in[i], 16);
#pragma unroll
    for (int q = 0; q < 8; ++q)
#pragma unroll
        for (int m = 0; m < 2; ++m) {
            const unsigned lo = d[2 * m][q >> 1], hi = d[2 * m + 1][q >> 1];
            out[q][m] = (q & 1) ? ((lo >> 16) | (hi & 0xffff0000u)) : ((lo & 0xffffu) | (hi << 16));
        }
}

#ifdef MDETR_TGEMM_TIMELINE
__device__ long long tgemm_tl[64];
#define TG_MARK(i) do { if (blockIdx.x == 3 && threadIdx.x == 0 && (i) < 64) tgemm_tl[(i)] = clock64(); } while (0)
#else
#define TG_MARK(i) do { } while (0)
#endif

template <int BM, int BN, bool NN, int PF, int TAIL, int NTH = 256>
__global__ __launch_bounds__(NTH, NTH == 512 ? 4 : 2)
void tgemm_kernel(const TgemmArgs g)
{
    TG_MARK(0);
    constexpr int kThreadsT = NTH;
    constexpr int WNW = NTH / 128;
    constexpr int TM = BM / 64, TN = BN / (32 * WNW);
    constexpr int XCH = BM * 8 / kThreadsT;
    constexpr int WCH = NN ? 4 : BN * 8 / kThreadsT;
    constexpr int WTHR = NN ? 2 * BN : kThreadsT;
    static_assert(TM >= 1 && TN >= 1 && XCH >= 1 && WCH >= 1 && WTHR <= kThreadsT, "tile / workgroup shape");
    MDETR_DYNAMIC_LDS(unsigned char, tg_smem);
    __bf16 *Xs = reinterpret_cast<__bf16 *>(tg_smem);
    __bf16 *Ws = Xs + 2 * BM * kLd;
    float *Cs = reinterpret_cast<float *>(tg_smem);
    const int tid = threadIdx.x, lane = tid & 63, wave = tid >> 6, half = lane >> 5, l31 = lane & 31;
    const int wm = wave & 1, wn = wave >> 1;
    const int KT = (g.K + kBK - 1) / kBK;
    const int G = gridDim.x, vtiles = g.gx * g.ny;
    const int tiles_m = g.tiles_m;
    auto tile_of = [&](int v, int &col, int64_t &m0) __attribute__((always_inline)) {
        const int grp = v >> 3;
        col = grp % g.ny;
        m0 = (static_cast<int64_t>(grp / g.ny) * 8 + (v & 7)) * BM;
    };
    auto next_tile = [&](int v) __attribute__((always_inline)) {
        for (; v < vtiles; v += G) {
            if ((v >> 3) / g.ny * 8 + (v & 7) < tiles_m) break;
        }
        return v;
    };

    const unsigned a_bytes = static_cast<unsigned>(((g.T - 1) * g.lda + g.K) * 2);
    const unsigned w_bytes = static_cast<unsigned>(NN ? ((static_cast<int64_t>(g.K) - 1) * g.ldw + g.N) * 2 : ((static_cast<int64_t>(g.N) - 1) * g.ldw + g.K) * 2);
    const mdetr_rsrc ar = make_rsrc(g.a, a_bytes), wr_ = make_rsrc(g.w, w_bytes);
    const int xk = (tid & 7) * 8;
    const int wkg = tid & 15, wnb = tid >> 4;
    unsigned xoff[XCH], woff[NN ? 1 : WCH];
    int xdst[XCH], wdst[NN ? 1 : WCH];
#pragma unroll
    for (int j = 0; j < XCH; ++j) {
        const int c = tid + kThreadsT * j;
        xdst[j] = (c >> 3) * kLd + (c & 7) * 8;
    }
    if (NN) {
        wdst[0] = wnb * 8 * kLd + wkg * 4;
    } else {
#pragma unroll
        for (int j = 0; j < (NN ? 1 : WCH); ++j) {
            const int c = tid + kThreadsT * j;
            wdst[j] = (c >> 3) * kLd + (c & 7) * 8;
        }
    }
    auto aim = [&](int v) __attribute__((always_inline)) {
        int col; int64_t m0;
        tile_of(v, col, m0);
        const int n0 = col * BN;
#pragma unroll
        for (int j = 0; j < XCH; ++j) {
            const int c = tid + kThreadsT * j;
            const int64_t t = m0 + (c >> 3);
            xoff[j] = t < g.T ? (static_cast<unsigned>(t) * static_cast<unsigned>(g.lda) + (c & 7) * 8) * 2u : kRsrcOob;
        }
        if (NN) {
            woff[0] = (tid < WTHR && n0 + wnb * 8 < g.N) ? static_cast<unsigned>((static_cast<int64_t>(wkg * 4) * g.ldw + n0 + wnb * 8) * 2) : kRsrcOob;
        } else {
#pragma unroll
            for (int j = 0; j < (NN ? 1 : WCH); ++j) {
                const int c = tid + kThreadsT * j, row = n0 + (c >> 3);
                woff[j] = row < g.N ? (static_cast<unsigned>(row) * static_cast<unsigned>(g.ldw) + (c & 7) * 8) * 2u : kRsrcOob;
            }
        }
    };

    bf16x8 xr[PF][XCH], wr[PF][WCH];
    auto fetch = [&](int kt, bf16x8 (&xs_)[XCH], bf16x8 (&ws_)[WCH]) __attribute__((always_inline)) {
        const int k0 = kt * kBK;
        const bool xin = k0 + xk < g.K;
#pragma unroll
        for (int j = 0; j < XCH; ++j) xs_[j] = rsrc_load_bf16x8(ar, xin ? xoff[j] : kRsrcOob, static_cast<unsigned>(k0 * 2));
        if (NN) {
            if (tid < WTHR) {
#pragma unroll
                for (int i = 0; i < 4; ++i)
                    ws_[i] = rsrc_load_bf16x8(wr_, k0 + wkg * 4 + i < g.K ? woff[0] : kRsrcOob,
                                              static_cast<unsigned>((static_cast<int64_t>(k0 + i) * g.ldw) * 2));
            }
        } else {
#pragma unroll
            for (int j = 0; j < WCH; ++j) ws_[j] = rsrc_load_bf16x8(wr_, xin ? woff[NN ? 0 : j] : kRsrcOob, static_cast<unsigned>(k0 * 2));
        }
    };
    auto deposit = [&](int buf, const bf16x8 (&xs_)[XCH], const bf16x8 (&ws_)[WCH]) __attribute__((always_inline)) {
        __bf16 *xb = Xs + buf * BM * kLd, *wb = Ws + buf * BN * kLd;
#pragma unroll
        for (int j = 0; j < XCH; ++j) *reinterpret_cast<bf16x8 *>(xb + xdst[j]) = xs_[j];
        if (NN) {
            if (tid < WTHR) {
                bf16x8 in[4];
                unsigned tr[8][2];
#pragma unroll
                for (int i = 0; i < 4; ++i) in[i] = ws_[i];
                transpose4x8(in, tr);
#pragma unroll
                for (int q = 0; q < 8; ++q) __builtin_memcpy(wb + wdst[0] + q * kLd, tr[q], 8);
            }
        } else {
#pragma unroll
            for (int j = 0; j < WCH; ++j) *reinterpret_cast<bf16x8 *>(wb + wdst[NN ? 0 : j]) = ws_[j];
        }
    };

    f32x16 acc[TN][TM];
    auto clear = [&]() __attribute__((always_inline)) {
#pragma unroll
        for (int a_ = 0; a_ < TN; ++a_)
#pragma unroll
            for (int b_ = 0; b_ < TM; ++b_)
#pragma unroll
                for (int i = 0; i < 16; ++i) acc[a_][b_][i] = 0.f;
    };
    auto products = [&](int buf) __attribute__((always_inline)) {
        const __bf16 *xl = Xs + (buf * BM + wm * (BM / 2) + l31) * kLd + half * 8;
        const __bf16 *wl = Ws + (buf * BN + wn * (BN / WNW) + l31) * kLd + half * 8;
#pragma unroll
        for (int ks = 0; ks < kBK / 16; ++ks) {
            bf16x8 xf[TM], wf[TN];
#pragma unroll
            for (int b_ = 0; b_ < TM; ++b_) xf[b_] = *reinterpret_cast<const bf16x8 *>(xl + b_ * 32 * kLd + ks * 16);
#pragma unroll
            for (int a_ = 0; a_ < TN; ++a_) wf[a_] = *reinterpret_cast<const bf16x8 *>(wl + a_ * 32 * kLd + ks * 16);
#pragma unroll
            for (int a_ = 0; a_ < TN; ++a_)
#pragma unroll
                for (int b_ = 0; b_ < TM; ++b_) acc[a_][b_] = mfma_bf16(wf[a_], xf[b_], acc[a_][b_]);
        }
    };

    constexpr int PR = BN / 8, NP = BM * PR / kThreadsT;
    constexpr bool RES = TAIL != 0;
    constexpr bool MASK = TAIL == 3;
    const int pc = tid % PR;
    const float lo = (g.flags & kTgemmRelu) ? 0.f : -__builtin_inff();
    const bool out32 = TAIL == 2 && (g.flags & kTgemmOutF32) != 0;
    const bool has_res = TAIL == 1 || ((TAIL == 2 || TAIL == 3) && g.res != nullptr);
    const uint64_t sd = (TAIL == 2 && g.thresh) ? g.seed + (g.seed_dev ? *g.seed_dev : 0ull) : 0ull;
    const mdetr_rsrc yr = make_rsrc(g.y, static_cast<unsigned>(((g.T - 1) * g.ldy + g.N) * (out32 ? 4 : 2)));
    const mdetr_rsrc rr_ = make_rsrc(has_res ? static_cast<const void *>(g.res) : static_cast<const void *>(g.a),
                                     has_res ? static_cast<unsigned>(((g.T - 1) * g.ldr + g.N) * 2) : 0u);
    const mdetr_rsrc mr_ = make_rsrc(MASK ? static_cast<const void *>(g.mask) : static_cast<const void *>(g.a),
                                     MASK ? static_cast<unsigned>(((g.T - 1) * g.ldm + g.N) * 2) : 0u);
    constexpr int NPB = NP < 4 ? NP : 4;
    bf16x8 rq[RES ? NP : 1];
    bf16x8 mq[MASK ? NP : 1];
    float bv[8];
    unsigned yoff[NP];
    int64_t tail_m0 = 0;
    int tail_n = 0;
    auto aim_tail = [&](int v) __attribute__((always_inline)) {
        int col;
        tile_of(v, col, tail_m0);
        tail_n = col * BN + pc * 8;
        const bool ncol = tail_n < g.N;
#pragma unroll
        for (int j = 0; j < NP; ++j) {
            const int64_t t = tail_m0 + (tid + kThreadsT * j) / PR;
            yoff[j] = (ncol && t < g.T) ? static_cast<unsigned>(t * g.ldy + tail_n) : kRsrcOob;
            if (RES && !MASK) rq[j] = rsrc_load_bf16x8(rr_, (has_res && ncol && t < g.T) ? static_cast<unsigned>((t * g.ldr + tail_n) * 2) : kRsrcOob, 0u);
        }
#pragma unroll
        for (int i = 0; i < 8; ++i) bv[i] = 0.f;
        if (g.bias && ncol) {
            if (TAIL == 2 && (g.flags & kTgemmBiasF32)) {
#pragma unroll
                for (int i = 0; i < 8; ++i) bv[i] = static_cast<const float *>(g.bias)[tail_n + i];
            } else {
                const bf16x8 b8 = *reinterpret_cast<const bf16x8 *>(static_cast<const __bf16 *>(g.bias) + tail_n);
#pragma unroll
                for (int i = 0; i < 8; ++i) bv[i] = static_cast<float>(b8[i]);
            }
        }
    };
    auto park = [&]() __attribute__((always_inline)) {
#pragma unroll
        for (int a_ = 0; a_ < TN; ++a_)
#pragma unroll
            for (int b_ = 0; b_ < TM; ++b_) {
                float *cr = Cs + (wm * (BM / 2) + b_ * 32 + l31) * (BN + kCPad) + wn * (BN / WNW) + a_ * 32 + 4 * half;
#pragma unroll
                for (int q = 0; q < 4; ++q) {
                    f32x4 o;
                    o.x = acc[a_][b_][4 * q]; o.y = acc[a_][b_][4 * q + 1]; o.z = acc[a_][b_][4 * q + 2]; o.w = acc[a_][b_][4 * q + 3];
                    *reinterpret_cast<f32x4 *>(cr + 8 * q) = o;
                }
            }
    };
    auto aim_mask = [&]() __attribute__((always_inline)) {
        const bool ncol = tail_n < g.N;
#pragma unroll
        for (int j = 0; j < NP; ++j) {
            const int64_t t = tail_m0 + (tid + kThreadsT * j) / PR;
            const bool in = ncol && t < g.T;
            mq[MASK ? j : 0] = rsrc_load_bf16x8(mr_, in ? static_cast<unsigned>((t * g.ldm + tail_n) * 2) : kRsrcOob, 0u);
            rq[RES ? j : 0] = rsrc_load_bf16x8(rr_, (has_res && in) ? static_cast<unsigned>((t * g.ldr + tail_n) * 2) : kRsrcOob, 0u);
        }
    };
    auto drain = [&]() __attribute__((always_inline)) {
#pragma unroll
        for (int j0 = 0; j0 < NP; j0 += NPB) {
            f32x4 cq[NPB][2];
#pragma unroll
            for (int u = 0; u < NPB; ++u) {
                const float *cr = Cs + ((tid + kThreadsT * (j0 + u)) / PR) * (BN + kCPad) + pc * 8;
                cq[u][0] = *reinterpret_cast<const f32x4 *>(cr);
                cq[u][1] = *reinterpret_cast<const f32x4 *>(cr + 4);
            }
#pragma unroll
            for (int u = 0; u < NPB; ++u) {
                const int j = j0 + u;
                float o[8] = {cq[u][0].x, cq[u][0].y, cq[u][0].z, cq[u][0].w, cq[u][1].x, cq[u][1].y, cq[u][1].z, cq[u][1].w};
#pragma unroll
                for (int i = 0; i < 8; ++i) {
                    float f = o[i] + bv[i];
                    if (RES) f += static_cast<float>(rq[j][i]);
                    if (MASK) f = static_cast<float>(mq[j][i]) <= 0.f ? 0.f : f;
                    f = f < lo ? lo : f;
                    if (TAIL == 2 && g.thresh) {
                        const uint64_t t = static_cast<uint64_t>(tail_m0 + (tid + kThreadsT * j) / PR);
                        f = ln_hash(sd, t * static_cast<uint64_t>(g.N) + static_cast<uint64_t>(tail_n + i)) >= g.thresh ? f * g.keep_scale : 0.f;
                    }
                    o[i] = f;
                }
                if (out32) {
                    f32x4 o0, o1;
                    o0.x = o[0]; o0.y = o[1]; o0.z = o[2]; o0.w = o[3]; o1.x = o[4]; o1.y = o[5]; o1.z = o[6]; o1.w = o[7];
                    const unsigned off = yoff[j] == kRsrcOob ? kRsrcOob : yoff[j] * 4u;
                    rsrc_store_f32x4(yr, o0, off, 0u);
                    rsrc_store_f32x4(yr, o1, off, 16u);
                } else {
                    bf16x8 ob;
#pragma unroll
                    for (int i = 0; i < 8; ++i) ob[i] = static_cast<__bf16>(o[i]);
                    rsrc_store_bf16x8(yr, ob, yoff[j] == kRsrcOob ? kRsrcOob : yoff[j] * 2u, 0u);
                }
            }
        }
    };

    int cv = next_tile(static_cast<int>(blockIdx.x));
    if (cv >= vtiles) return;
    int ck = 0, fv = cv, fk = 0;
    auto advance = [&]() __attribute__((always_inline)) {
        if (++fk == KT) {
            fk = 0;
            fv = next_tile(fv + G);
            if (fv < vtiles) aim(fv);
        }
    };
    TG_MARK(1);
    aim(fv);
    fetch(0, xr[PF - 1], wr[PF - 1]);
    advance();
#pragma unroll
    for (int p = 0; p < PF - 1; ++p)
        if (fv < vtiles) { fetch(fk, xr[p], wr[p]); advance(); }
    TG_MARK(2);
    deposit(0, xr[PF - 1], wr[PF - 1]);
    TG_MARK(3);
    if (fv < vtiles) { fetch(fk, xr[PF - 1], wr[PF - 1]); advance(); }
    clear();
    __syncthreads();
    TG_MARK(4);
    for (int s = 0;; s += PF) {
#pragma unroll
        for (int p = 0; p < PF; ++p) {
            const bool last = ck == KT - 1;
            if (!last) {
                deposit((s + p + 1) & 1, xr[p], wr[p]);
                if (fv < vtiles) { fetch(fk, xr[p], wr[p]); advance(); }
            }
            TG_MARK(5 + 3 * (s + p));
            products((s + p) & 1);
            TG_MARK(6 + 3 * (s + p));
            __syncthreads();
            TG_MARK(7 + 3 * (s + p));
            ++ck;
            if (last) {
                aim_tail(cv);
                park();
                TG_MARK(40);
                if (MASK) {
                    __builtin_amdgcn_sched_barrier(0);
                    aim_mask();
                }
                __syncthreads();
                TG_MARK(41);
                drain();
                TG_MARK(42);
                cv = next_tile(cv + G);
                if (cv >= vtiles) return;
                __syncthreads();
                deposit((s + p + 1) & 1, xr[p], wr[p]);
                if (fv < vtiles) { fetch(fk, xr[p], wr[p]); advance(); }
                clear();
                ck = 0;
                __syncthreads();
            }
        }
    }
}

template <int BM, int BN, bool NN, int PF, int TAIL, int NTH = 256>
hipError_t launch_tile(TgemmArgs g, hipStream_t st)
{
    constexpr size_t lds = tgemm_lds<BM, BN>();
    static_assert(lds <= 80 * 1024, "two workgroups per CU");
    constexpr int kThreadsT = NTH;
    auto kern = tgemm_kernel<BM, BN, NN, PF, TAIL, NTH>;
    static bool attr_set[64] = {};
    int dev_ = 0;
    if (hipGetDevice(&dev_) != hipSuccess) dev_ = -1;
    if (dev_ < 0 || dev_ >= 64 || !attr_set[dev_]) {
        const hipError_t e = hipFuncSetAttribute(reinterpret_cast<const void *>(kern), hipFuncAttributeMaxDynamicSharedMemorySize,
                                                 static_cast<int>(lds));
        if (e != hipSuccess) return e;
        if (dev_ >= 0 && dev_ < 64) attr_set[dev_] = true;
    }
    const int64_t tiles_m = (g.T + BM - 1) / BM;
    g.tiles_m = static_cast<int>(tiles_m);
    g.ny = (g.N + BN - 1) / BN;
    g.gx = static_cast<int>((tiles_m + 7) / 8 * 8);
    const int64_t vtiles = static_cast<int64_t>(g.gx) * g.ny;
    int per_cu = static_cast<int>((160 * 1024) / lds);
    per_cu = per_cu > 4 ? 4 : per_cu;
    int64_t grid = static_cast<int64_t>(256) * per_cu;
    { const int f = tune_int("tgemm_grid", 0); if (f >= 8 && f % 8 == 0) grid = f; }
    if (grid > vtiles) grid = vtiles;
    hipLaunchKernelGGL(kern, dim3(static_cast<unsigned>(grid)), dim3(kThreadsT), lds, st, g);
    return hipGetLastError();
}

template <bool NN, int PF, int TAIL>
hipError_t launch_any(const TgemmArgs &g, int bm, int bn, hipStream_t st)
{
    if (bm == 128 && bn == 128) {
        if constexpr (!NN && PF == 1 && TAIL == 0) {
            if (tune_int("tgemm_waves", 8) != 4) return launch_tile<128, 128, NN, PF, TAIL, 512>(g, st);
        }
        return launch_tile<128, 128, NN, PF, TAIL>(g, st);
    }
    if (bm == 128) return launch_tile<128, 64, NN, PF, TAIL>(g, st);
    if (bn == 128) return launch_tile<64, 128, NN, PF, TAIL>(g, st);
    return launch_tile<64, 64, NN, PF, TAIL>(g, st);
}

template <bool NN, int PF>
hipError_t launch_tail(const TgemmArgs &g, int bm, int bn, hipStream_t st)
{
    if ((g.flags & (kTgemmBiasF32 | kTgemmOutF32)) || g.thresh) return launch_any<NN, PF, 2>(g, bm, bn, st);
    if constexpr (NN) {
        if (g.mask) return launch_any<NN, PF, 3>(g, bm, bn, st);
    }
    return g.res ? launch_any<NN, PF, 1>(g, bm, bn, st) : launch_any<NN, PF, 0>(g, bm, bn, st);
}


struct Tgemm32Args {
    const float *a, *w, *res, *mask, *bias;
    float *y;
    int64_t T, lda, ldw, ldr, ldy, ldm;
    int N, K, gx, ny, flags, tiles_m;
    uint32_t thresh;
    float keep_scale;
    uint64_t seed;
    const uint64_t *seed_dev;
};

template <int BM, int BN, int BK>
constexpr size_t tgemm32_lds()
{
    constexpr size_t slabs = static_cast<size_t>(2) * 3 * (BM + BN) * (BK + 8) * 2, tile = static_cast<size_t>(BM) * (BN + kCPad) * 4;
    return slabs > tile ? slabs : tile;
}

__device__ __forceinline__ void split4(const float (&x)[4], bf16x4 &h, bf16x4 &m, bf16x4 &l)
{
#pragma unroll
    for (int i = 0; i < 4; ++i) {
        const __bf16 hi = static_cast<__bf16>(x[i]);
        const float r1 = x[i] - static_cast<float>(hi);
        const __bf16 mi = static_cast<__bf16>(r1);
        h[i] = hi; m[i] = mi; l[i] = static_cast<__bf16>(r1 - static_cast<float>(mi));
    }
}

template <int BM, int BN, int BK, bool NN, int PF, bool MASK>
__global__ __launch_bounds__(256, 2)
void tgemm32_kernel(const Tgemm32Args g)
{
    constexpr int LD = BK + 8;
    constexpr int QK = BK / 4;
    constexpr int TM = BM / 64, TN = BN / 64;
    constexpr int XCH = BM * QK / kThreadsT;
    constexpr int WCH = NN ? 4 : BN * QK / kThreadsT;
    constexpr int WTHR = NN ? QK * (BN / 4) : kThreadsT;
    static_assert(TM >= 1 && TN >= 1 && XCH >= 1 && WCH >= 1 && WTHR <= kThreadsT && kThreadsT % QK == 0 && BK % 16 == 0, "tile / workgroup shape");
    MDETR_DYNAMIC_LDS(unsigned char, tg_smem);
    __bf16 *Xs = reinterpret_cast<__bf16 *>(tg_smem);
    __bf16 *Ws = Xs + 2 * 3 * BM * LD;
    float *Cs = reinterpret_cast<float *>(tg_smem);
    const int tid = threadIdx.x, lane = tid & 63, wave = tid >> 6, half = lane >> 5, l31 = lane & 31;
    const int wm = wave & 1, wn = wave >> 1;
    const int KT = (g.K + BK - 1) / BK;
    const int G = gridDim.x, vtiles = g.gx * g.ny;
    const int tiles_m = g.tiles_m;
    auto tile_of = [&](int v, int &col, int64_t &m0) __attribute__((always_inline)) {
        const int grp = v >> 3;
        col = grp % g.ny;
        m0 = (static_cast<int64_t>(grp / g.ny) * 8 + (v & 7)) * BM;
    };
    auto next_tile = [&](int v) __attribute__((always_inline)) {
        for (; v < vtiles; v += G) {
            if ((v >> 3) / g.ny * 8 + (v & 7) < tiles_m) break;
        }
        return v;
    };

    const unsigned a_bytes = static_cast<unsigned>(((g.T - 1) * g.lda + g.K) * 4);
    const unsigned w_bytes = static_cast<unsigned>(NN ? ((static_cast<int64_t>(g.K) - 1) * g.ldw + g.N) * 4 : ((static_cast<int64_t>(g.N) - 1) * g.ldw + g.K) * 4);
    const mdetr_rsrc ar = make_rsrc(g.a, a_bytes), wr_ = make_rsrc(g.w, w_bytes);
    const int xq = tid % QK, xk = xq * 4;
    const int wkg = tid % QK, wnb = tid / QK;
    unsigned xoff[XCH], woff[NN ? 1 : WCH];
    int xdst[XCH], wdst[NN ? 1 : WCH];
#pragma unroll
    for (int j = 0; j < XCH; ++j) xdst[j] = ((tid + kThreadsT * j) / QK) * LD + xk;
    if (NN) {
        wdst[0] = wnb * 4 * LD + wkg * 4;
    } else {
#pragma unroll
        for (int j = 0; j < (NN ? 1 : WCH); ++j) wdst[j] = ((tid + kThreadsT * j) / QK) * LD + xk;
    }
    auto aim = [&](int v) __attribute__((always_inline)) {
        int col; int64_t m0;
        tile_of(v, col, m0);
        const int n0 = col * BN;
#pragma unroll
        for (int j = 0; j < XCH; ++j) {
            const int64_t t = m0 + (tid + kThreadsT * j) / QK;
            xoff[j] = t < g.T ? (static_cast<unsigned>(t) * static_cast<unsigned>(g.lda) + xk) * 4u : kRsrcOob;
        }
        if (NN) {
            woff[0] = (tid < WTHR && n0 + wnb * 4 < g.N) ? static_cast<unsigned>((static_cast<int64_t>(wkg * 4) * g.ldw + n0 + wnb * 4) * 4) : kRsrcOob;
        } else {
#pragma unroll
            for (int j = 0; j < (NN ? 1 : WCH); ++j) {
                const int row = n0 + (tid + kThreadsT * j) / QK;
                woff[j] = row < g.N ? (static_cast<unsigned>(row) * static_cast<unsigned>(g.ldw) + xk) * 4u : kRsrcOob;
            }
        }
    };

    bf16x8 xr[PF][XCH], wr[PF][WCH];
    auto fetch = [&](int kt, bf16x8 (&xs_)[XCH], bf16x8 (&ws_)[WCH]) __attribute__((always_inline)) {
        const int k0 = kt * BK;
        const bool xin = k0 + xk < g.K;
#pragma unroll
        for (int j = 0; j < XCH; ++j) xs_[j] = rsrc_load_bf16x8(ar, xin ? xoff[j] : kRsrcOob, static_cast<unsigned>(k0 * 4));
        if (NN) {
            if (tid < WTHR) {
                const bool kin = k0 + wkg * 4 < g.K;
// ... 150 lines not shown
                    __builtin_memcpy(mk, &mq[MASK ? u : 0][0], 16);
                    __builtin_memcpy(mk + 4, &mq[MASK ? u : 0][1], 16);
                }
#pragma unroll
                for (int i = 0; i < 8; ++i) {
                    float f = o[i] + bv[i] + r[i];
                    if (MASK) f = mk[i] <= 0.f ? 0.f : f;
                    f = f < lo ? lo : f;
                    if (g.thresh) {
                        const uint64_t t = static_cast<uint64_t>(tail_m0 + (tid + kThreadsT * (j0 + u)) / PR);
                        f = ln_hash(sd, t * static_cast<uint64_t>(g.N) + static_cast<uint64_t>(tail_n + i)) >= g.thresh ? f * g.keep_scale : 0.f;
                    }
                    o[i] = f;
                }
                f32x4 o0, o1;
                o0.x = o[0]; o0.y = o[1]; o0.z = o[2]; o0.w = o[3]; o1.x = o[4]; o1.y = o[5]; o1.z = o[6]; o1.w = o[7];
                rsrc_store_f32x4(yr, o0, yoff[u], 0u);
                rsrc_store_f32x4(yr, o1, yoff[u], 16u);
            }
        }
    };

    int cv = next_tile(static_cast<int>(blockIdx.x));
    if (cv >= vtiles) return;
    int ck = 0, fv = cv, fk = 0;
    auto advance = [&]() __attribute__((always_inline)) {
        if (++fk == KT) {
            fk = 0;
            fv = next_tile(fv + G);
            if (fv < vtiles) aim(fv);
        }
    };
    aim(fv);
    fetch(0, xr[PF - 1], wr[PF - 1]);
    advance();
#pragma unroll
    for (int p = 0; p < PF - 1; ++p)
        if (fv < vtiles) { fetch(fk, xr[p], wr[p]); advance(); }
    deposit(0, xr[PF - 1], wr[PF - 1]);
    if (fv < vtiles) { fetch(fk, xr[PF - 1], wr[PF - 1]); advance(); }
    clear();
    __syncthreads();
    for (int s = 0;; s += PF) {
#pragma unroll
        for (int p = 0; p < PF; ++p) {
            const bool last = ck == KT - 1;
            if (!last) {
                deposit((s + p + 1) & 1, xr[p], wr[p]);
                if (fv < vtiles) { fetch(fk, xr[p], wr[p]); advance(); }
            }
            products((s + p) & 1);
            __syncthreads();
            ++ck;
            if (last) {
                aim_tail(cv);
                park();
                __syncthreads();
                drain();
                cv = next_tile(cv + G);
                if (cv >= vtiles) return;
                __syncthreads();
                deposit((s + p + 1) & 1, xr[p], wr[p]);
                if (fv < vtiles) { fetch(fk, xr[p], wr[p]); advance(); }
                clear();
                ck = 0;
                __syncthreads();
            }
        }
    }
}

template <int BM, int BN, int BK, bool NN, int PF, bool MASK>
hipError_t launch_tile32(Tgemm32Args g, hipStream_t st)
{
    constexpr size_t lds = tgemm32_lds<BM, BN, BK>();
    static_assert(lds <= 80 * 1024, "two workgroups per CU");
    auto kern = tgemm32_kernel<BM, BN, BK, NN, PF, MASK>;
    static bool attr_set[64] = {};
    int dev_ = 0;
    if (hipGetDevice(&dev_) != hipSuccess) dev_ = -1;
    if (dev_ < 0 || dev_ >= 64 || !attr_set[dev_]) {
        const hipError_t e = hipFuncSetAttribute(reinterpret_cast<const void *>(kern), hipFuncAttributeMaxDynamicSharedMemorySize,
                                                 static_cast<int>(lds));
        if (e != hipSuccess) return e;
        if (dev_ >= 0 && dev_ < 64) attr_set[dev_] = true;
    }
    const int64_t tiles_m = (g.T + BM - 1) / BM;
    g.tiles_m = static_cast<int>(tiles_m);
    g.ny = (g.N + BN - 1) / BN;
    g.gx = static_cast<int>((tiles_m + 7) / 8 * 8);
    const int64_t vtiles = static_cast<int64_t>(g.gx) * g.ny;
    int64_t grid = static_cast<int64_t>(256) * 2;
    { const int f = tune_int("tgemm_grid", 0); if (f >= 8 && f % 8 == 0) grid = f; }
    if (grid > vtiles) grid = vtiles;
    hipLaunchKernelGGL(kern, dim3(static_cast<unsigned>(grid)), dim3(kThreadsT), lds, st, g);
    return hipGetLastError();
}

template <bool NN, int PF, bool MASK>
hipError_t launch_any32(const Tgemm32Args &g, int bm, int bn, hipStream_t st)
{
    if (bm == 128 && bn == 128) return launch_tile32<128, 128, 16, NN, 1, MASK>(g, st);
    if (bm == 128) return launch_tile32<128, 64, 16, NN, PF, MASK>(g, st);
    return launch_tile32<64, 64, 32, NN, PF, MASK>(g, st);
}

bool tgemm32_supported(const TgemmProblem &p)
{
    const auto al = [](const void *q) { return (reinterpret_cast<uintptr_t>(q) & 15) == 0; };
    const bool nn = (p.flags & kTgemmNN) != 0;
    return p.T > 0 && p.T < (1ll << 31) - 256 && p.N > 0 && p.N % 8 == 0 && p.K > 0 && p.K % 8 == 0 && p.a && p.w && p.y && al(p.a) && al(p.w) &&
           al(p.y) && p.lda % 4 == 0 && p.lda >= p.K && p.ldw % 4 == 0 && p.ldw >= (nn ? p.N : p.K) && p.ldy % 4 == 0 && p.ldy >= p.N &&
           (!p.res || (al(p.res) && p.ldr % 4 == 0 && p.ldr >= p.N)) && (!p.bias || al(p.bias)) && p.dropout_p >= 0.f && p.dropout_p < 1.f &&
           !(p.flags & ~(kTgemmRelu | kTgemmNN)) &&
           (!p.mask || (nn && al(p.mask) && p.ldm % 4 == 0 && p.ldm >= p.N && p.T * p.ldm < (1ll << 29) && !p.bias && p.dropout_p == 0.f &&
                        !(p.flags & kTgemmRelu))) &&
           p.T * p.lda < (1ll << 29) && p.T * p.ldy < (1ll << 29) && p.T * p.ldr < (1ll << 29) && static_cast<int64_t>(nn ? p.K : p.N) * p.ldw < (1ll << 29);
}

hipError_t tgemm32_launch(const TgemmProblem &p, hipStream_t st)
{
    Tgemm32Args g;
    g.a = static_cast<const float *>(p.a); g.w = static_cast<const float *>(p.w); g.res = static_cast<const float *>(p.res);
    g.mask = static_cast<const float *>(p.mask); g.bias = static_cast<const float *>(p.bias); g.y = static_cast<float *>(p.y);
    g.T = p.T; g.lda = p.lda; g.ldw = p.ldw; g.ldr = p.ldr; g.ldy = p.ldy; g.ldm = p.ldm;
    g.N = p.N; g.K = p.K; g.gx = g.ny = g.tiles_m = 0; g.flags = p.flags;
    g.thresh = p.dropout_p > 0.f ? ln_threshold(p.dropout_p) : 0u;
    g.keep_scale = p.dropout_p > 0.f ? 1.f / (1.f - p.dropout_p) : 1.f;
    g.seed = p.seed; g.seed_dev = p.seed_dev;
    const auto wgs = [&](int m, int n) { return ((p.T + m - 1) / m) * ((p.N + n - 1) / n); };
    int bm = 64, bn = 64;
    if (p.N > 64 && wgs(128, 128) >= 400) { bm = 128; bn = 128; }
    else if (wgs(128, 64) >= 400) { bm = 128; bn = 64; }
    char tune_buf[16];
    if (const char *ev = tune_str("tgemm_f32_tile", tune_buf, sizeof(tune_buf))) {
        int m = 0, n = 0;
        if (sscanf(ev, "%dx%d", &m, &n) == 2 && ((m == 64 && n == 64) || (m == 128 && (n == 64 || n == 128)))) { bm = m; bn = n; }
    }
    int pf = 2;
    if (const int f = tune_int("tgemm_f32_pf", 0)) pf = f == 1 ? 1 : 2;
    ProfileScope prof(10, conv_mflop(p.T, static_cast<int64_t>(p.N) * p.K), st, 2.0 * p.T * p.N * p.K / 1e6,
                      (4.0 * p.T * p.K + 4.0 * p.T * p.N + (p.res ? 4.0 * p.T * p.N : 0.0) + (p.mask ? 4.0 * p.T * p.N : 0.0) + 4.0 * p.N * p.K) / 1e3);
    if (p.flags & kTgemmNN) {
        if (p.mask) return pf == 1 ? launch_any32<true, 1, true>(g, bm, bn, st) : launch_any32<true, 2, true>(g, bm, bn, st);
        return pf == 1 ? launch_any32<true, 1, false>(g, bm, bn, st) : launch_any32<true, 2, false>(g, bm, bn, st);
    }
    return pf == 1 ? launch_any32<false, 1, false>(g, bm, bn, st) : launch_any32<false, 2, false>(g, bm, bn, st);
}

}

bool tgemm_supported(const TgemmProblem &p)
{
    if (p.f32) return tgemm32_supported(p);
    const auto al = [](const void *q) { return (reinterpret_cast<uintptr_t>(q) & 15) == 0; };
    const bool nn = (p.flags & kTgemmNN) != 0;
    return p.T > 0 && p.T < (1ll << 31) - 256 && p.N > 0 && p.N % 8 == 0 && p.K > 0 && p.K % 8 == 0 && p.a && p.w && p.y && al(p.a) && al(p.w) &&
           al(p.y) && p.lda % 8 == 0 && p.lda >= p.K && p.ldw % 8 == 0 && p.ldw >= (nn ? p.N : p.K) &&
           p.ldy % ((p.flags & kTgemmOutF32) ? 4 : 8) == 0 && p.ldy >= p.N &&
           (!p.res || (al(p.res) && p.ldr % 8 == 0 && p.ldr >= p.N)) && (!p.bias || al(p.bias)) && p.dropout_p >= 0.f && p.dropout_p < 1.f &&
           (!p.mask || (nn && al(p.mask) && p.ldm % 8 == 0 && p.ldm >= p.N && p.T * p.ldm < (1ll << 30) && !p.bias && p.dropout_p == 0.f &&
                        !(p.flags & (kTgemmRelu | kTgemmBiasF32 | kTgemmOutF32)))) &&
           p.T * p.lda < (1ll << 30) && p.T * p.ldy < (1ll << 29) && p.T * p.ldr < (1ll << 30) && static_cast<int64_t>(nn ? p.K : p.N) * p.ldw < (1ll << 30);
}

hipError_t tgemm_launch(const TgemmProblem &p, hipStream_t st)
{
    if (p.f32) return tgemm32_launch(p, st);
    TgemmArgs g;
    g.a = static_cast<const __bf16 *>(p.a); g.w = static_cast<const __bf16 *>(p.w); g.res = static_cast<const __bf16 *>(p.res);
    g.mask = static_cast<const __bf16 *>(p.mask); g.ldm = p.ldm;
    g.bias = p.bias; g.y = p.y;
    g.T = p.T; g.lda = p.lda; g.ldw = p.ldw; g.ldr = p.ldr; g.ldy = p.ldy;
    g.N = p.N; g.K = p.K; g.gx = g.ny = 0; g.flags = p.flags;
    g.thresh = p.dropout_p > 0.f ? ln_threshold(p.dropout_p) : 0u;
    g.keep_scale = p.dropout_p > 0.f ? 1.f / (1.f - p.dropout_p) : 1.f;
    g.seed = p.seed; g.seed_dev = p.seed_dev;
    const bool generic_tail = (p.flags & (kTgemmBiasF32 | kTgemmOutF32)) != 0 || p.dropout_p > 0.f;
    const auto wgs = [&](int m, int n) { return ((p.T + m - 1) / m) * ((p.N + n - 1) / n); };
    int bm = 64, bn = 64;
    if (p.N > 64 && !generic_tail && !(p.T < 8192 && p.K <= 256)) {
        if (wgs(128, 128) >= 400) { bm = 128; bn = 128; }
        else if (wgs(128, 64) >= 400) { bm = 128; bn = 64; }
    }
    char tune_buf[16];
    if (const char *ev = tune_str("tgemm_tile", tune_buf, sizeof(tune_buf))) {
        int m = 0, n = 0;
        if (sscanf(ev, "%dx%d", &m, &n) == 2 && (m == 64 || m == 128) && (n == 64 || n == 128)) { bm = m; bn = n; }
    }
    int pf = 2;
    if (bm == 128 && bn == 128 && (p.res || p.mask || (p.flags & (kTgemmBiasF32 | kTgemmOutF32)) || p.dropout_p > 0.f)) pf = 1;
    if (bm == 128 && bn == 128 && !(p.flags & kTgemmNN) && !p.res && !generic_tail) pf = 1;
    if (const int f = tune_int("tgemm_pf", 0)) pf = f == 1 ? 1 : 2;
    ProfileScope prof(10, conv_mflop(p.T, static_cast<int64_t>(p.N) * p.K), st, 2.0 * p.T * p.N * p.K / 1e6,
                      (2.0 * p.T * p.K + ((p.flags & kTgemmOutF32) ? 4.0 : 2.0) * p.T * p.N + (p.res ? 2.0 * p.T * p.N : 0.0) + (p.mask ? 2.0 * p.T * p.N : 0.0) + 2.0 * p.N * p.K) / 1e3);
    if (p.flags & kTgemmNN) return pf == 1 ? launch_tail<true, 1>(g, bm, bn, st) : launch_tail<true, 2>(g, bm, bn, st);
    return pf == 1 ? launch_tail<false, 1>(g, bm, bn, st) : launch_tail<false, 2>(g, bm, bn, st);
}

}
```

monodetr_amd/monodetr/attention.py:

```python
import os

import torch
import torch.nn.functional as F
from torch import nn

from ..attn_ext import fused_attention
from .linear import Linear, split_rows, token_linear


def _sdpa(q, k, v, num_heads, dropout_p, key_padding_mask):
    B, Lq, E = q.shape
    Lk = k.shape[1]
    d = E // num_heads
    qh = q.reshape(B, Lq, num_heads, d).transpose(1, 2)
    kh = k.reshape(B, Lk, num_heads, d).transpose(1, 2)
    vh = v.reshape(B, Lk, num_heads, d).transpose(1, 2)
    mask = None
    if key_padding_mask is not None:
        mask = ~key_padding_mask.view(B, 1, 1, Lk)
    out = F.scaled_dot_product_attention(qh, kh, vh, attn_mask=mask, dropout_p=dropout_p)
    return out.transpose(1, 2).reshape(B, Lq, E)


def attention_core(q, k, v, num_heads, dropout_p=0.0, key_padding_mask=None):
    from .. import _tune
    if q.is_cuda and q.shape[-1] == 32 * num_heads and _tune.get("attn_backend", "hip") == "hip":
        if q.dtype not in (torch.float32, torch.bfloat16):
            q, k, v = q.float(), k.float(), v.float()
        if k.dtype != q.dtype or v.dtype != q.dtype:
            k, v = k.to(q.dtype), v.to(q.dtype)
        return fused_attention(q, k, v, num_heads, dropout_p, key_padding_mask)
    return _sdpa(q, k, v, num_heads, dropout_p, key_padding_mask)


class MultiheadAttention(nn.Module):
    def __init__(self, embed_dim, num_heads, dropout=0.0):
        super().__init__()
        if embed_dim % num_heads != 0:
            raise ValueError("embed_dim must be divisible by num_heads")
        self.embed_dim, self.num_heads, self.dropout = embed_dim, num_heads, dropout
        self.head_dim = embed_dim // num_heads
        self.in_proj_weight = nn.Parameter(torch.empty(3 * embed_dim, embed_dim))
        self.in_proj_bias = nn.Parameter(torch.zeros(3 * embed_dim))
        self.out_proj = Linear(embed_dim, embed_dim)
        nn.init.xavier_uniform_(self.in_proj_weight)
        nn.init.zeros_(self.out_proj.bias)

    def project(self, query, key, value):
        E = self.embed_dim
        W, b = self.in_proj_weight, self.in_proj_bias
        if query is key and key is value:
            return token_linear(query, W, b).split(E, -1)
        if query is key:
            (Wqk, Wv), (bqk, bv) = split_rows(W, 2 * E, E), split_rows(b, 2 * E, E)
            q, k = token_linear(query, Wqk, bqk).split(E, -1)
            return q, k, token_linear(value, Wv, bv)
        if key is value:
            (Wq, Wkv), (bq, bkv) = split_rows(W, E, 2 * E), split_rows(b, E, 2 * E)
            k, v = token_linear(key, Wkv, bkv).split(E, -1)
            return token_linear(query, Wq, bq), k, v
        (Wq, Wk, Wv), (bq, bk, bv) = split_rows(W, E, E, E), split_rows(b, E, E, E)
        return token_linear(query, Wq, bq), token_linear(key, Wk, bk), token_linear(value, Wv, bv)

    def forward_batch_first(self, query, key, value, key_padding_mask=None):
        q, k, v = self.project(query, key, value)
        p = self.dropout if self.training else 0.0
        return self.out_proj(attention_core(q, k, v, self.num_heads, p, key_padding_mask))

    def forward(self, query, key, value, key_padding_mask=None, need_weights=False, attn_mask=None):
        if attn_mask is not None:
            raise NotImplementedError("attn_mask is not used on the MonoDETR path")
        qb = query.transpose(0, 1)
        kb = qb if key is query else key.transpose(0, 1)
        vb = kb if value is key else value.transpose(0, 1)
        out = self.forward_batch_first(qb, kb, vb, key_padding_mask)
        return out.transpose(0, 1), None
```

monodetr_amd/monodetr/depth_predictor/transformer.py:

```python
import copy

import torch.nn.functional as F
from torch import nn

from ...add_ln_ext import residual_layernorm
from ..attention import MultiheadAttention
from ..linear import Linear, ffn_hidden


def _get_clones(module, N):
    return nn.ModuleList([copy.deepcopy(module) for _ in range(N)])


def _get_activation_fn(activation):
    try:
        return {"relu": F.relu, "gelu": F.gelu, "glu": F.glu}[activation]
    except KeyError:
        raise RuntimeError(f"activation should be relu/gelu, not {activation}.")


class TransformerEncoderLayer(nn.Module):
    def __init__(self, d_model, nhead, dim_feedforward=2048, dropout=0.1, activation="relu"):
        super().__init__()
        self.self_attn = MultiheadAttention(d_model, nhead, dropout=dropout)
        self.linear1 = Linear(d_model, dim_feedforward)
        self.dropout = nn.Dropout(dropout)
        self.linear2 = Linear(dim_feedforward, d_model)
        self.norm1 = nn.LayerNorm(d_model)
        self.norm2 = nn.LayerNorm(d_model)
        self.dropout1 = nn.Dropout(dropout)
        self.dropout2 = nn.Dropout(dropout)
        self.activation = _get_activation_fn(activation)

    def forward(self, src, src_key_padding_mask, pos):
        qk = src if pos is None else src + pos
        src = residual_layernorm(src, self.self_attn(qk, qk, src, key_padding_mask=src_key_padding_mask)[0], self.norm1, self.dropout1)
        ff = self.linear2(ffn_hidden(src, self.linear1, self.dropout, self.activation, tokenwise=False))
        return residual_layernorm(src, ff, self.norm2, self.dropout2)


    def forward_batch_first(self, src, src_key_padding_mask, pos):
        qk = src if pos is None else src + pos
        attn = self.self_attn.forward_batch_first(qk, qk, src, key_padding_mask=src_key_padding_mask)
        src = residual_layernorm(src, attn, self.norm1, self.dropout1)
        ff = self.linear2(ffn_hidden(src, self.linear1, self.dropout, self.activation, tokenwise=False))
        return residual_layernorm(src, ff, self.norm2, self.dropout2)


class TransformerEncoder(nn.Module):
    def __init__(self, encoder_layer, num_layers, norm=None):
        super().__init__()
        self.layers = _get_clones(encoder_layer, num_layers)
        self.num_layers = num_layers
        self.norm = norm

    def forward(self, src, src_key_padding_mask, pos):
        for layer in self.layers:
            src = layer(src, src_key_padding_mask=src_key_padding_mask, pos=pos)
        return src if self.norm is None else self.norm(src)

    def forward_batch_first(self, src, src_key_padding_mask, pos):
        for layer in self.layers:
            src = layer.forward_batch_first(src, src_key_padding_mask, pos)
        return src if self.norm is None else self.norm(src)
```

monodetr_amd/monodetr/depthaware_transformer.py:

```python
import copy

import torch
import torch.nn.functional as F
from torch import nn
from torch.nn.init import constant_, normal_, xavier_uniform_

from .. import head_tail_ext
from ..add_ln_ext import residual_layernorm
from . import _cut
from ..utils.misc import inverse_sigmoid, no_padding
from .attention import MultiheadAttention as FusedMultiheadAttention
from .heads import heads_level
from .. import _tune

_CHAIN_MEMORY = _tune.get("decoder_chain", "1") != "0"
from .linear import Linear, ffn_hidden, token_linear
from .ops.modules import MSDeformAttn, MSDeformAttn_cross, MultiheadAttention


class MLP(nn.Module):

    def __init__(self, input_dim, hidden_dim, output_dim, num_layers):
        super().__init__()
        self.num_layers = num_layers
        dims = [input_dim] + [hidden_dim] * (num_layers - 1) + [output_dim]
        self.layers = nn.ModuleList(Linear(a, b) for a, b in zip(dims[:-1], dims[1:]))

    def forward(self, x):
        x = x.to(self.layers[0].weight.dtype)
        for layer in self.layers[:-1]:
            x = F.relu(layer(x))
        return self.layers[-1](x)


def fused_first_layers(x, heads):
    firsts = [h.layers[0] if isinstance(h, MLP) else h for h in heads]
    x = x.to(firsts[0].weight.dtype)
    widths = [l.out_features for l in firsts]
    pad = -sum(widths) % 8
    ws, bs = [l.weight for l in firsts], [l.bias for l in firsts]
    if pad:
        zw, zb = _zero_rows(ws[0], pad)
        ws.append(zw)
        bs.append(zb)
    y = token_linear(x, torch.cat(ws, 0), torch.cat(bs, 0))
    return y.split(widths + ([pad] if pad else []), -1)[:len(widths)]


_ZERO_ROWS = {}


def _zero_rows(like, rows):
    key = (like.device, like.dtype, rows, like.shape[1])
    hit = _ZERO_ROWS.get(key)
    if hit is None:
        hit = _ZERO_ROWS[key] = (like.new_zeros(rows, like.shape[1]), like.new_zeros(rows))
    return hit


def mlp_rest(mlp, h):
    if mlp.num_layers == 1:
        return h
    x = F.relu(h)
    for layer in mlp.layers[1:-1]:
        x = F.relu(layer(x))
    return mlp.layers[-1](x)


class _SummedPair(torch.autograd.Function):

    @staticmethod
    def forward(ctx, w1, w2, w3, w4, b1, b2, b3, b4):
        ctx.rows = w1.shape[0]
        return torch.cat((w1 + w2, w3 + w4), 0), torch.cat((b1 + b2, b3 + b4), 0)

    @staticmethod
    @torch.autograd.function.once_differentiable
    def backward(ctx, gw, gb):
        from .. import chunk_sums
        chunk_sums.flush()
        n = ctx.rows
        return gw[:n], gw[:n], gw[n:], gw[n:], gb[:n], gb[:n], gb[n:], gb[n:]


class _LevelPos(torch.autograd.Function):

    @staticmethod
    def forward(ctx, level_embed, dtype, *pos):
        ctx.counts = [p.shape[-2] * p.shape[-1] for p in pos]
        ctx.embed_dtype = level_embed.dtype
        ctx.pos_meta = [(p.shape, p.dtype) for p in pos]
        return torch.cat([p.flatten(2).transpose(1, 2) + level_embed[l].view(1, 1, -1) for l, p in enumerate(pos)], 1).to(dtype)

    @staticmethod
    @torch.autograd.function.once_differentiable
    def backward(ctx, g):
        from .. import colsum_ext
        B, S, C = g.shape
        g = g.contiguous()
        flat = g.view(B, S * C)
        wide = torch.float64 if g.dtype == torch.float64 else torch.float32
        over_batch = (colsum_ext.column_sum(flat) if colsum_ext.supported(flat) else flat.to(wide).sum(0)).view(S, C)
        rows, start = [], 0
        for n in ctx.counts:
            part = over_batch[start:start + n]
            rows.append(colsum_ext.column_sum(part) if colsum_ext.supported(part) else part.sum(0))
            start += n
        gpos, start = [], 0
        for l, (n, (shape, dt)) in enumerate(zip(ctx.counts, ctx.pos_meta)):
            gpos.append(g[:, start:start + n].transpose(1, 2).reshape(shape).to(dt) if ctx.needs_input_grad[2 + l] else None)
            start += n
        return (torch.stack(rows).to(ctx.embed_dtype), None) + tuple(gpos)


def _get_clones(module, N):
    return nn.ModuleList([copy.deepcopy(module) for _ in range(N)])


def _get_activation_fn(activation):
    try:
        return {"relu": F.relu, "gelu": F.gelu, "glu": F.glu}[activation]
    except KeyError:
        raise RuntimeError(f"activation should be relu/gelu, not {activation}.")


def _shape_list(spatial_shapes):
    if torch.is_tensor(spatial_shapes):
        return [tuple(int(v) for v in hw) for hw in spatial_shapes.tolist()]
    return [tuple(int(v) for v in hw) for hw in spatial_shapes]


class VisualEncoderLayer(nn.Module):
    def __init__(self, d_model=256, d_ffn=1024, dropout=0.1, activation="relu", n_levels=4, n_heads=8, n_points=4):
        super().__init__()
        self.self_attn = MSDeformAttn(d_model, n_levels, n_heads, n_points)
        self.dropout1 = nn.Dropout(dropout)
        self.norm1 = nn.LayerNorm(d_model)
        self.linear1 = Linear(d_model, d_ffn)
        self.activation = _get_activation_fn(activation)
        self.dropout2 = nn.Dropout(dropout)
        self.linear2 = Linear(d_ffn, d_model)
        self.dropout3 = nn.Dropout(dropout)
        self.norm2 = nn.LayerNorm(d_model)

    @staticmethod
    def with_pos_embed(tensor, pos):
        return tensor if pos is None else tensor + pos

    def forward_ffn(self, src):
        h, src = ffn_hidden(src, self.linear1, self.dropout2, self.activation, skip=True)
        ff = token_linear(h, self.linear2.weight, self.linear2.bias)
        return residual_layernorm(src, ff, self.norm2, self.dropout3)

    def forward(self, src, pos, reference_points, spatial_shapes, level_start_index, padding_mask=None):
        attn, src = self.self_attn.forward_self(src, pos, reference_points, spatial_shapes, level_start_index, padding_mask)
        return self.forward_ffn(residual_layernorm(src, attn, self.norm1, self.dropout1))


class VisualEncoder(nn.Module):
    def __init__(self, encoder_layer, num_layers):
        super().__init__()
        self.layers = _get_clones(encoder_layer, num_layers)
        self.num_layers = num_layers
        self._ref_cache = {}

    @staticmethod
    def get_reference_points(spatial_shapes, valid_ratios, device):
        per_level = []
        for lvl, (H, W) in enumerate(_shape_list(spatial_shapes)):
            ys = torch.linspace(0.5, H - 0.5, H, dtype=torch.float32, device=device)
            xs = torch.linspace(0.5, W - 0.5, W, dtype=torch.float32, device=device)
            gy, gx = torch.meshgrid(ys, xs, indexing="ij")
            gy = gy.reshape(-1)[None] / (valid_ratios[:, None, lvl, 1] * H)
            gx = gx.reshape(-1)[None] / (valid_ratios[:, None, lvl, 0] * W)
            per_level.append(torch.stack((gx, gy), -1))
        return torch.cat(per_level, 1)[:, :, None] * valid_ratios[:, None]

    def _unpadded_reference_points(self, shapes, B, L, device):
        key = (tuple(shapes), L, str(device))
        ref = self._ref_cache.get(key)
        if ref is None:
            ones = torch.ones((1, L, 2), dtype=torch.float32, device=device)
            ref = self._ref_cache[key] = self.get_reference_points(shapes, ones, device)
        return ref.expand(B, -1, -1, -1)

    def forward(self, src, spatial_shapes, level_start_index, valid_ratios, pos=None, padding_mask=None,
                ref_token_index=None, ref_token_coord=None, shape_list=None):
        shapes = shape_list if shape_list is not None else _shape_list(spatial_shapes)
        if valid_ratios is None:
            reference_points = self._unpadded_reference_points(shapes, src.shape[0], len(shapes), src.device)
        else:
            reference_points = self.get_reference_points(shapes, valid_ratios, src.device)
        out = src
        for i, layer in enumerate(self.layers):
            with _cut.armed(i == len(self.layers) - 1):
                out = layer(out, pos, reference_points, spatial_shapes, level_start_index, padding_mask)
        return out


class DepthAwareDecoderLayer(nn.Module):
    def __init__(self, d_model=256, d_ffn=1024, dropout=0.1, activation="relu", n_levels=4, n_heads=8,
                 n_points=4, group_num=1):
        super().__init__()
        self.cross_attn = MSDeformAttn(d_model, n_levels, n_heads, n_points)
        self.dropout1 = nn.Dropout(dropout)
        self.norm1 = nn.LayerNorm(d_model)
        self.cross_attn_depth = FusedMultiheadAttention(d_model, n_heads, dropout=dropout)
        self.dropout_depth = nn.Dropout(dropout)
        self.norm_depth = nn.LayerNorm(d_model)
        self.self_attn = FusedMultiheadAttention(d_model, n_heads, dropout=dropout)
        self.dropout2 = nn.Dropout(dropout)
        self.norm2 = nn.LayerNorm(d_model)
        self.linear1 = Linear(d_model, d_ffn)
        self.activation = _get_activation_fn(activation)
        self.dropout3 = nn.Dropout(dropout)
        self.linear2 = Linear(d_ffn, d_model)
        self.dropout4 = nn.Dropout(dropout)
        self.norm3 = nn.LayerNorm(d_model)
        self.group_num = group_num
        self.sa_qcontent_proj = Linear(d_model, d_model)
        self.sa_qpos_proj = Linear(d_model, d_model)
        self.sa_kcontent_proj = Linear(d_model, d_model)
        self.sa_kpos_proj = Linear(d_model, d_model)
        self.sa_v_proj = nn.Linear(d_model, d_model)
        self.nhead = n_heads

    @staticmethod
    def with_pos_embed(tensor, pos):
        return tensor if pos is None else tensor + pos

    def forward_ffn(self, tgt):
        ff = self.linear2(ffn_hidden(tgt, self.linear1, self.dropout3, self.activation, tokenwise=False))
        return residual_layernorm(tgt, ff, self.norm3, self.dropout4)

    def _self_attention_inputs(self, x):
        w, b = _SummedPair.apply(self.sa_qcontent_proj.weight, self.sa_qpos_proj.weight, self.sa_kcontent_proj.weight, self.sa_kpos_proj.weight,
                                 self.sa_qcontent_proj.bias, self.sa_qpos_proj.bias, self.sa_kcontent_proj.bias, self.sa_kpos_proj.bias)
        q, k = token_linear(x, w, b).split(x.shape[-1], -1)
        return q, k

    def forward(self, tgt, query_pos, reference_points, src, src_spatial_shapes, level_start_index,
                src_padding_mask, depth_pos_embed, mask_depth, bs, query_sine_embed=None, is_first=None,
                depth_pos_embed_ip=None, pos_embeds=None, self_attn_mask=None, query_pos_un=None, chain_src=False):
        B, Nq, C = tgt.shape
        depth_tokens = depth_pos_embed.transpose(0, 1)
        d = self.cross_attn_depth.forward_batch_first(tgt, depth_tokens, depth_tokens, mask_depth)
        tgt = residual_layernorm(tgt, d, self.norm_depth, self.dropout_depth)
        q, k = self._self_attention_inputs(self.with_pos_embed(tgt, query_pos))
        v = tgt
        if self.training and self.group_num > 1:
            if Nq % self.group_num != 0:
                raise ValueError("training expects num_queries * group_num queries, got %d for %d groups" % (Nq, self.group_num))
            n = Nq // self.group_num
            q, k, v = (t.reshape(B * self.group_num, n, C) for t in (q, k, v))
        s = self.self_attn.forward_batch_first(q, k, v).reshape(B, Nq, C)
        tgt = residual_layernorm(tgt, s, self.norm2, self.dropout2)
        c = self.cross_attn(self.with_pos_embed(tgt, query_pos), reference_points, src, src_spatial_shapes,
                            level_start_index, src_padding_mask, chain_input=chain_src)
        if chain_src:
            c, src = c
        tgt = residual_layernorm(tgt, c, self.norm1, self.dropout1)
        return (self.forward_ffn(tgt), src) if chain_src else self.forward_ffn(tgt)


class DepthAwareDecoder(nn.Module):
    def __init__(self, decoder_layer, num_layers, return_intermediate=False, d_model=None, use_dab=False,
                 two_stage_dino=False):
        super().__init__()
        if use_dab or two_stage_dino:
            raise NotImplementedError("use_dab / two_stage_dino are off in configs/monodetr.yaml and not built")
        self.layers = _get_clones(decoder_layer, num_layers)
        self.num_layers = num_layers
        self.return_intermediate = return_intermediate
        self.bbox_embed = None
        self.dim_embed = None
        self.class_embed = None
        self.use_dab = use_dab
        self.two_stgae_dino = two_stage_dino
        self.query_scale = MLP(d_model, d_model, d_model, 2)
        self.ref_point_head = MLP(d_model, d_model, 2, 2)

    def forward(self, tgt, reference_points, src, src_spatial_shapes, src_level_start_index, src_valid_ratios,
                query_pos=None, src_padding_mask=None, depth_pos_embed=None, mask_depth=None, bs=None,
                depth_pos_embed_ip=None, pos_embeds=None, attn_mask=None):
        output = tgt
        bs = src.shape[0]
        L = src_spatial_shapes.shape[0]
        hs, refs, dims = [], [], []
        reference_dims = None
        head_out = self.__dict__["head_outputs"] = []
        for lid, layer in enumerate(self.layers):
            nd = reference_points.shape[-1]
            assert nd in (2, 6)
            if src_valid_ratios is None:
                ref_in = reference_points[:, :, None].expand(-1, -1, L, -1)
            else:
                ref_in = reference_points[:, :, None] * src_valid_ratios.repeat(1, 1, nd // 2)[:, None]
            output = layer(output, query_pos, ref_in, src, src_spatial_shapes, src_level_start_index,
                           src_padding_mask, depth_pos_embed, mask_depth, bs, query_sine_embed=None,
                           is_first=(lid == 0), depth_pos_embed_ip=depth_pos_embed_ip, pos_embeds=pos_embeds,
                           self_attn_mask=attn_mask, query_pos_un=None, chain_src=_CHAIN_MEMORY)
            if _CHAIN_MEMORY:
                output, src = output
            fused = self.__dict__.get("fused_heads")
            if fused is not None and self.bbox_embed is not None and self.dim_embed is not None:
                cls, dep, ang = (f[lid] for f in fused)
                grouped = heads_level(output, self.bbox_embed[lid], self.dim_embed[lid], dep, ang, cls)
                if grouped is not None:
                    delta, grouped_dims, dep_out, ang_out, cls_out, output = grouped
                    head_out.append((delta, dep_out, ang_out, cls_out))
                else:
                    parts = fused_first_layers(output, [self.bbox_embed[lid], self.dim_embed[lid], dep, ang, cls])
                    delta = mlp_rest(self.bbox_embed[lid], parts[0])
                    head_out.append((delta, mlp_rest(dep, parts[2]), mlp_rest(ang, parts[3]),
                                     mlp_rest(cls, parts[4]) if isinstance(cls, MLP) else parts[4]))
            elif self.bbox_embed is not None:
                delta = self.bbox_embed[lid](output)
            if self.bbox_embed is not None and head_tail_ext.usable(delta, reference_points) and delta.shape[-1] == 6:
                reference_points = head_tail_ext.box_refine(delta, reference_points)
            elif self.bbox_embed is not None:
                if nd == 6:
                    new_ref = (delta + inverse_sigmoid(reference_points)).sigmoid()
                else:
                    new_ref = torch.cat((delta[..., :2] + inverse_sigmoid(reference_points), delta[..., 2:]), -1).sigmoid()
                reference_points = new_ref.detach()
            if fused is not None and self.bbox_embed is not None and self.dim_embed is not None:
                reference_dims = grouped_dims if grouped is not None else mlp_rest(self.dim_embed[lid], parts[1])
            elif self.dim_embed is not None:
                reference_dims = self.dim_embed[lid](output)
            if self.return_intermediate:
                hs.append(output)
                refs.append(reference_points)
                dims.append(reference_dims)
        if self.return_intermediate:
            return torch.stack(hs), torch.stack(refs), torch.stack(dims)
        return output, reference_points


class DepthAwareTransformer(nn.Module):
    def __init__(self, d_model=256, nhead=8, num_encoder_layers=6, num_decoder_layers=6, dim_feedforward=1024,
                 dropout=0.1, activation="relu", return_intermediate_dec=False, num_feature_levels=4,
                 dec_n_points=4, enc_n_points=4, two_stage=False, two_stage_num_proposals=50, group_num=11,
                 use_dab=False, two_stage_dino=False):
        super().__init__()
        if two_stage or use_dab or two_stage_dino:
            raise NotImplementedError("two_stage / use_dab / two_stage_dino are off in configs/monodetr.yaml and not built")
        self.d_model, self.nhead = d_model, nhead
        self.two_stage, self.two_stage_num_proposals = two_stage, two_stage_num_proposals
        self.use_dab, self.two_stage_dino, self.group_num = use_dab, two_stage_dino, group_num

        self.encoder = VisualEncoder(
            VisualEncoderLayer(d_model, dim_feedforward, dropout, activation, num_feature_levels, nhead, enc_n_points),
            num_encoder_layers)
        self.decoder = DepthAwareDecoder(
            DepthAwareDecoderLayer(d_model, dim_feedforward, dropout, activation, num_feature_levels, nhead,
                                   dec_n_points, group_num=group_num),
            num_decoder_layers, return_intermediate_dec, d_model, use_dab=use_dab, two_stage_dino=two_stage_dino)
        self.level_embed = nn.Parameter(torch.Tensor(num_feature_levels, d_model))
        self.reference_points = nn.Linear(d_model, 2)
        self._shape_cache = {}
        self._reset_parameters()

    def _reset_parameters(self):
        for p in self.parameters():
            if p.dim() > 1:
                nn.init.xavier_uniform_(p)
        for m in self.modules():
            if isinstance(m, MSDeformAttn):
                m._reset_parameters()
        xavier_uniform_(self.reference_points.weight.data, gain=1.0)
        constant_(self.reference_points.bias.data, 0.)
        normal_(self.level_embed)

    def get_valid_ratio(self, mask):
        _, H, W = mask.shape
        vh = torch.sum(~mask[:, :, 0], 1).float() / H
        vw = torch.sum(~mask[:, 0, :], 1).float() / W
        return torch.stack([vw, vh], -1)

    def _level_tensors(self, shapes, device):
        key = (tuple(shapes), str(device))
        hit = self._shape_cache.get(key)
        if hit is None:
            ss = torch.as_tensor(shapes, dtype=torch.long, device=device)
            hit = self._shape_cache[key] = (ss, torch.cat((ss.new_zeros((1,)), ss.prod(1).cumsum(0)[:-1])))
        return hit

    def encode(self, srcs, masks, pos_embeds):
        unpadded = all(no_padding(m) for m in masks)
        shapes = [tuple(s.shape[-2:]) for s in srcs]
        src_flatten = torch.cat([s.flatten(2).transpose(1, 2) for s in srcs], 1)
        lvl_pos = _LevelPos.apply(self.level_embed, src_flatten.dtype, *pos_embeds)
        spatial_shapes, level_start_index = self._level_tensors(shapes, src_flatten.device)
        if unpadded:
            mask_flatten = valid_ratios = mask_depth = None
        else:
            mask_flatten = torch.cat([m.flatten(1) for m in masks], 1)
            valid_ratios = torch.stack([self.get_valid_ratio(m) for m in masks], 1)
            mask_depth = masks[1].flatten(1)

        memory = self.encoder(src_flatten, spatial_shapes, level_start_index, valid_ratios, lvl_pos, mask_flatten,
                              shape_list=shapes)
        return memory, spatial_shapes, level_start_index, valid_ratios, mask_flatten, mask_depth

    def forward(self, srcs, masks, pos_embeds, query_embed=None, depth_pos_embed=None, depth_pos_embed_ip=None,
                attn_mask=None):
        assert query_embed is not None
        B, C = srcs[0].shape[:2]
        memory, spatial_shapes, level_start_index, valid_ratios, mask_flatten, mask_depth = self.encode(srcs, masks, pos_embeds)

        query_pos, tgt = torch.split(query_embed, C, dim=1)
        reference_points = self.reference_points(query_pos.to(self.reference_points.weight.dtype)).sigmoid()
        reference_points = reference_points.unsqueeze(0).expand(B, -1, -1)
        query_pos = query_pos.to(memory.dtype).unsqueeze(0).expand(B, -1, -1)
# ... 21 lines not shown
```

monodetr_amd/monodetr/linear.py:

```python
import os

import torch
import torch.nn.functional as F
from torch import nn

from .. import colsum_ext, small_wgrad_ext

_MIN_TOKENS = 4096
_GEMM_RELU = os.environ.get("MDETR_GEMM_RELU") == "1"
_TGEMM = os.environ.get("MDETR_TGEMM") == "1"
_TGEMM_F32 = os.environ.get("MDETR_TGEMM_F32") == "1"


_TWGRAD_MIN_ROWS = 1024


_PREMASK = os.environ.get("MDETR_RELU_PREMASK") == "1"


class ReluToken:
    __slots__ = ("premasked",)

    def __init__(self):
        self.premasked = False
# ... 131 lines not shown
            y = F.linear(q, weight, bias)
        if relu:
            ctx.save_for_backward(q, weight, y)
        else:
            ctx.save_for_backward(q, weight)
        return y, x.view_as(x)

    @staticmethod
    @torch.autograd.function.once_differentiable
    def backward(ctx, dy, dskip):
        q, weight = ctx.saved_tensors[:2]
        if ctx.relu and not (ctx.out_token is not None and ctx.out_token.premasked and ctx.scale == 1.0):
            dy = _act_backward(dy.contiguous(), ctx.saved_tensors[2], ctx.scale)
        if ctx.wide_out:
            dy = dy.to(q.dtype)
        q2, dy2 = q.reshape(-1, q.shape[-1]), dy.reshape(-1, dy.shape[-1])
        dx = None
        if ctx.needs_input_grad[0]:
            ds2 = dskip.reshape(-1, q.shape[-1]) if dskip is not None else None
            dx = _input_gradient(dy2, weight, ds2, q2 if ctx.premask else None).view_as(q)
        dw, db = _weight_bias_grads(q2, dy2, weight, ctx.needs_input_grad[1], ctx.has_bias and ctx.needs_input_grad[2], ctx.bias_dtype)
        return dx, dw, db, None, None, None, None, None, None


def token_linear_skip(x, weight, bias=None, pos=None, relu=False, dropout_p=0.0, relu_token=None, wide_out=False, out_token=None):
    if (x.is_cuda or _tgemm_backend()) and x.dtype == weight.dtype and x.numel() // x.shape[-1] >= _MIN_TOKENS and torch.is_grad_enabled() and x.requires_grad \
            and not torch.is_autocast_enabled() and (pos is None or not pos.requires_grad) \
            and (not relu or skip_relu_fusable(bias, x, weight)) and (dropout_p <= 0.0 or skip_dropout_fusable(x, weight, bias)) \
            and (not wide_out or (not relu and x.is_cuda and x.dtype == torch.bfloat16 and _tgemm_ok(x.reshape(-1, x.shape[-1]), weight, bias))):
        premask = relu_token is not None and pos is None and _kernel_dtype(x.dtype) and _tgemm_ok(x.reshape(-1, x.shape[-1]), weight, bias) \
            and (x.dtype != torch.float32 or x.numel() // x.shape[-1] >= _F32_NN_MIN_TOKENS)
        if premask:
            relu_token.premasked = True
        return _TokenLinearSkip.apply(x, weight, bias, pos, relu, dropout_p, premask, wide_out, out_token if relu else None)
    if dropout_p > 0.0:
        raise RuntimeError("token_linear_skip: ask skip_dropout_fusable before passing dropout_p")
    return token_linear(x if pos is None else x + pos, weight, bias, relu=relu, wide_out=wide_out), x


def skip_relu_fusable(bias, x=None, weight=None):
    if x is not None and weight is not None and _tgemm_ok(x.reshape(-1, x.shape[-1]), weight, bias):
        return True
    return _GEMM_RELU and bias is not None and bias.dim() == 1 and bias.is_contiguous()


def skip_dropout_fusable(x, weight, bias):
    return (x.is_cuda or _tgemm_backend()) and x.dtype == weight.dtype and x.numel() // x.shape[-1] >= _MIN_TOKENS \
        and not torch.is_autocast_enabled() and _tgemm_ok(x.reshape(-1, x.shape[-1]), weight, bias)


class _TokenLinear(torch.autograd.Function):
    @staticmethod
    def forward(ctx, x, weight, bias, fused_relu=False, wide_out=False, dropout_p=0.0):
        ctx.has_bias = bias is not None
        ctx.bias_dtype = bias.dtype if bias is not None else None
        ctx.fused_relu = False
        ctx.wide_out = bool(wide_out)
        ctx.scale = 1.0 / (1.0 - dropout_p) if dropout_p > 0.0 else 1.0
        x2 = x.reshape(-1, x.shape[-1])
        if _tgemm_ok(x2, weight, bias):
            seed, seed_dev = _drop_seed(x, dropout_p)
            y = _fwd_product(x2, weight, bias, fused_relu, None, dropout_p, seed, seed_dev, torch.float32 if wide_out else x2.dtype)
            y = y.view(x.shape[:-1] + (weight.shape[0],))
            ctx.fused_relu = bool(fused_relu)
            if fused_relu:
                ctx.save_for_backward(x, weight, y)
            else:
                ctx.save_for_backward(x, weight)
            return y
        if dropout_p > 0.0:
            raise RuntimeError("token_linear: dropout is only fused into csrc/tgemm.hip's epilogue")
        if wide_out:
            y = torch.mm(x2, weight.t(), out_dtype=torch.float32)
            if bias is not None:
                y += bias.float()
            ctx.save_for_backward(x, weight)
            return y.view(x.shape[:-1] + (weight.shape[0],))
        if fused_relu:
            y = torch._addmm_activation(bias, x2, weight.t()).view(x.shape[:-1] + (weight.shape[0],))
            ctx.fused_relu = True
            ctx.save_for_backward(x, weight, y)
            return y
        ctx.save_for_backward(x, weight)
        return F.linear(x, weight, bias)

    @staticmethod
    @torch.autograd.function.once_differentiable
    def backward(ctx, dy):
        if ctx.fused_relu:
            x, weight, y = ctx.saved_tensors
            dy = _act_backward(dy.contiguous(), y, ctx.scale)
        else:
            x, weight = ctx.saved_tensors
        if ctx.wide_out:
            dy = dy.to(x.dtype)
        dx = dw = db = None
        x2 = x.reshape(-1, x.shape[-1])
        dy2 = dy.reshape(-1, dy.shape[-1])
        if ctx.needs_input_grad[0]:
            dx = _input_gradient(dy2, weight).view_as(x)
        dw, db = _weight_bias_grads(x2, dy2, weight, ctx.needs_input_grad[1], ctx.has_bias and ctx.needs_input_grad[2], ctx.bias_dtype)
        return dx, dw, db, None, None, None


class _TokenLinearResidualRelu(torch.autograd.Function):

    @staticmethod
    def forward(ctx, x2, weight, bias, res2, out_token=None, in_premask=False):
        out = _fwd_product(x2, weight, bias, True, res2)
        ctx.has_bias = bias is not None
        ctx.bias_dtype = bias.dtype if bias is not None else None
        ctx.out_token = out_token
        ctx.in_premask = bool(in_premask)
        ctx.save_for_backward(x2, weight, out)
        return out

    @staticmethod
    @torch.autograd.function.once_differentiable
    def backward(ctx, dout):
        x2, weight, out = ctx.saved_tensors
        if ctx.out_token is not None and ctx.out_token.premasked:
            g = dout.contiguous()
        else:
            g = torch.ops.aten.threshold_backward(dout.contiguous(), out, 0.0)
        dx = _input_gradient(g, weight, None, x2 if ctx.in_premask else None) if ctx.needs_input_grad[0] else None
        dw, db = _weight_bias_grads(x2, g, weight, ctx.needs_input_grad[1], ctx.has_bias and ctx.needs_input_grad[2], ctx.bias_dtype)
        return dx, dw, db, (g if ctx.needs_input_grad[3] else None), None, None


class _SplitRows(torch.autograd.Function):

    @staticmethod
    def forward(ctx, packed, *sizes):
        ctx.sizes = sizes
        ctx.meta = (packed.shape[1:], packed.dtype, packed.device)
        return tuple(p.view_as(p) for p in packed.split(list(sizes), 0))

    @staticmethod
    @torch.autograd.function.once_differentiable
    def backward(ctx, *grads):
        tail, dtype, device = ctx.meta
        from .. import chunk_sums
        chunk_sums.flush()
        parts = [g if g is not None else torch.zeros((n,) + tuple(tail), dtype=dtype, device=device) for g, n in zip(grads, ctx.sizes)]
        return (torch.cat(parts, 0),) + (None,) * len(ctx.sizes)


def split_rows(packed, *sizes):
    if not (torch.is_grad_enabled() and packed.requires_grad):
        return packed.split(list(sizes), 0)
    return _SplitRows.apply(packed, *sizes)


def _kernel_relu(x, weight, bias=None):
    if _tgemm_ok(x.reshape(-1, x.shape[-1]), weight, bias):
        return True
    return _GEMM_RELU and bias is not None and bias.dim() == 1 and bias.is_contiguous()


def dropout_fusable(x, weight, bias):
    return (x.is_cuda or _tgemm_backend()) and x.dtype == weight.dtype and x.numel() // x.shape[-1] >= _MIN_TOKENS and torch.is_grad_enabled() \
        and not torch.is_autocast_enabled() and _tgemm_ok(x.reshape(-1, x.shape[-1]), weight, bias)


def _tgemm_backend():
    from .. import tgemm_ext
    return tgemm_ext._backend is not None


def token_linear(x, weight, bias=None, relu=False, wide_out=False, dropout_p=0.0):
    if dropout_p > 0.0:
        if not (relu and dropout_fusable(x, weight, bias)):
            raise RuntimeError("token_linear: ask dropout_fusable before passing dropout_p (ReLU + Dropout ride in csrc/tgemm.hip's epilogue only)")
        return _TokenLinear.apply(x, weight, bias, True, False, dropout_p)
    if wide_out and not relu and x.is_cuda and x.dtype == weight.dtype == torch.bfloat16 and not torch.is_autocast_enabled():
        return _TokenLinear.apply(x, weight, bias, False, True)
    if (x.is_cuda or _tgemm_backend()) and x.dtype == weight.dtype and x.numel() // x.shape[-1] >= _MIN_TOKENS and torch.is_grad_enabled() \
            and not torch.is_autocast_enabled():
        if relu and _kernel_relu(x, weight, bias):
            return _TokenLinear.apply(x, weight, bias, True)
        y = _TokenLinear.apply(x, weight, bias, False)
    else:
        y = F.linear(x, weight, bias)
    return F.relu(y) if relu else y


def pointwise_eligible(x, kernel_size, stride, padding, groups):
    return ((x.is_cuda or _tgemm_backend()) and tuple(kernel_size) == (1, 1) and tuple(stride) == (1, 1) and tuple(padding) == (0, 0)
            and groups == 1 and x.dim() == 4 and x.is_contiguous(memory_format=torch.channels_last))


def pointwise_conv(x, weight, bias=None, relu=False):
    B, C, H, W = x.shape
    y = token_linear(x.permute(0, 2, 3, 1).reshape(B * H * W, C), weight.reshape(weight.shape[0], C), bias, relu=relu)
    return y.view(B, H, W, -1).permute(0, 3, 1, 2)


def pointwise_conv_skip(x, weight, bias=None, relu=False, relu_token=None, hand_out_token=False):
    B, C, H, W = x.shape
    token = ReluToken() if (_PREMASK and hand_out_token and relu) else None
    y, xs = token_linear_skip(x.permute(0, 2, 3, 1).reshape(B * H * W, C), weight.reshape(weight.shape[0], C), bias, relu=relu, relu_token=relu_token,
                              out_token=token)
    y = y.view(B, H, W, -1).permute(0, 3, 1, 2)
    if token is not None:
        y._mdetr_relu_token = token
    return y, xs.view(B, H, W, C).permute(0, 3, 1, 2)


def pointwise_residual_relu_eligible(x, weight, bias, identity):
    if not (x.dim() == 4 and identity.dim() == 4 and _kernel_dtype(x.dtype) and identity.dtype == x.dtype
            and weight.dtype == x.dtype and not torch.is_autocast_enabled()
            and x.is_contiguous(memory_format=torch.channels_last) and identity.is_contiguous(memory_format=torch.channels_last)):
        return False
    B, C, H, W = x.shape
    N = weight.shape[0]
    if identity.shape != (B, N, H, W):
        return False
    return _tgemm_ok(x.permute(0, 2, 3, 1).reshape(B * H * W, C), weight.reshape(N, C), bias,
                     identity.permute(0, 2, 3, 1).reshape(B * H * W, N))


def pointwise_conv_residual_relu(x, weight, bias, identity, in_token=None, hand_out_token=False):
    B, C, H, W = x.shape
    N = weight.shape[0]
    x2, r2 = x.permute(0, 2, 3, 1).reshape(B * H * W, C), identity.permute(0, 2, 3, 1).reshape(B * H * W, N)
    token = None
    if torch.is_grad_enabled() and (x.requires_grad or weight.requires_grad or identity.requires_grad):
        token = ReluToken() if (_PREMASK and hand_out_token) else None
        in_premask = in_token is not None and x.requires_grad
        if in_premask:
            in_token.premasked = True
        out = _TokenLinearResidualRelu.apply(x2, weight.reshape(N, C), bias, r2, token, in_premask)
    else:
        out = _fwd_product(x2, weight.reshape(N, C), bias, True, r2)
    out = out.view(B, H, W, N).permute(0, 3, 1, 2)
    if token is not None:
        out._mdetr_relu_token = token
    return out


def pointwise_relu_fusable(x, weight, bias):
    if not (_GEMM_RELU or _TGEMM or _TGEMM_F32):
        return False
    C = x.shape[1]
    return (x.numel() // C >= _MIN_TOKENS and torch.is_grad_enabled() and not torch.is_autocast_enabled()
            and _kernel_relu(x.permute(0, 2, 3, 1).reshape(-1, C), weight.reshape(weight.shape[0], C), bias))


def ffn_hidden(x, lin, dropout, activation=F.relu, tokenwise=True, skip=False):
    from .. import bias_act_ext
    p = dropout.p if (dropout is not None and dropout.training) else 0.0
    if skip:
        if activation is F.relu and tokenwise and torch.is_grad_enabled() and x.requires_grad and skip_dropout_fusable(x, lin.weight, lin.bias):
            return token_linear_skip(x, lin.weight, lin.bias, relu=True, dropout_p=p)
        h, x_out = token_linear_skip(x, lin.weight, lin.bias)
        if activation is F.relu and bias_act_ext.ENABLED and p > 0.0 and torch.is_grad_enabled() and bias_act_ext.supported(h):
            return bias_act_ext.bias_act(h, None, None, relu=True, dropout_p=p), x_out
        h = activation(h)
        return (dropout(h) if dropout is not None else h), x_out
    if activation is F.relu and tokenwise and p > 0.0 and dropout_fusable(x, lin.weight, lin.bias):
        return token_linear(x, lin.weight, lin.bias, relu=True, dropout_p=p)
    first = (lambda relu: token_linear(x, lin.weight, lin.bias, relu=relu)) if tokenwise else \
        (lambda relu: F.relu(lin(x)) if relu else lin(x))
    if activation is not F.relu:
        h = activation(first(False))
    elif bias_act_ext.ENABLED and p > 0.0 and torch.is_grad_enabled():
        h = first(False)
        if bias_act_ext.supported(h):
            return bias_act_ext.bias_act(h, None, None, relu=True, dropout_p=p)
        h = F.relu(h)
    else:
        h = first(True)
    return dropout(h) if dropout is not None else h


class Linear(nn.Linear):

    def forward(self, x):
        return token_linear(x, self.weight, self.bias)


class PointwiseConv2d(nn.Conv2d):

    def forward(self, x):
        if pointwise_eligible(x, self.kernel_size, self.stride, self.padding, self.groups) \
                and x.dtype == self.weight.dtype and not torch.is_autocast_enabled():
            return pointwise_conv(x, self.weight, self.bias)
        from .. import conv_taps_ext
        if conv_taps_ext.ENABLED and x.dtype == self.weight.dtype and not torch.is_autocast_enabled() and self.padding_mode == "zeros" \
                and conv_taps_ext.supported(x, self.weight, self.stride, self.padding, self.dilation, self.groups):
            return conv_taps_ext.conv_strided(x, self.weight, self.bias, relu=False)
        return super().forward(x)
```

monodetr_amd/monodetr/ops/modules/ms_deform_attn.py:

```python
import math
import os
import warnings

import torch
import torch.nn.functional as F
from torch import nn

from ..functions import MSDeformAttnFunction
from ... import _cut
from ...linear import Linear, token_linear, token_linear_skip
from .... import msda_prologue_ext


_FUSED_PROLOGUE = os.environ.get("MDETR_MSDA_PROLOGUE") == "1"
_PACKED_PROJECTION = True
_WIDE_CROSS_VALUE = True



def _check_token_count(spatial_shapes, S):
    seen = getattr(spatial_shapes, "_mdetr_token_count", None)
    if seen != (spatial_shapes._version, S):
        assert int((spatial_shapes[:, 0] * spatial_shapes[:, 1]).sum()) == S
        try:
            spatial_shapes._mdetr_token_count = (spatial_shapes._version, S)
        except AttributeError:
            pass


def _is_power_of_2(n):
    if not isinstance(n, int) or n < 0:
        raise ValueError("invalid input for _is_power_of_2: {} (type: {})".format(n, type(n)))
    return n != 0 and (n & (n - 1)) == 0


def _star_offsets(n_heads, n_levels, n_points):
    theta = torch.arange(n_heads, dtype=torch.float32) * (2.0 * math.pi / n_heads)
    d = torch.stack([theta.cos(), theta.sin()], -1)
    d = d / d.abs().max(-1, keepdim=True)[0]
    scale = torch.arange(1, n_points + 1, dtype=torch.float32).view(1, 1, n_points, 1)
    return (d.view(n_heads, 1, 1, 2) * scale).expand(n_heads, n_levels, n_points, 2).reshape(-1)


class MSDeformAttn(nn.Module):
    def __init__(self, d_model=256, n_levels=4, n_heads=8, n_points=4, conditional=False):
        super().__init__()
        if d_model % n_heads != 0:
            raise ValueError("d_model must be divisible by n_heads, but got {} and {}".format(d_model, n_heads))
        if not _is_power_of_2(d_model // n_heads):
            warnings.warn("MSDeformAttn: head dimension %d is not a power of 2; the gfx950 fast path "
                          "needs 32 channels per head, other sizes take the generic kernel." % (d_model // n_heads))
        self.im2col_step = 64
        self.d_model, self.n_levels, self.n_heads, self.n_points = d_model, n_levels, n_heads, n_points
        self.conditional = conditional
        d_value = d_model // 2 if conditional else d_model
        self.sampling_offsets = Linear(d_model, n_heads * n_levels * n_points * 2)
        self.attention_weights = Linear(d_model, n_heads * n_levels * n_points)
        self.value_proj = Linear(d_value, d_value)
        self.output_proj = Linear(d_value, d_value)
        self._reset_parameters()

    def _reset_parameters(self):
        with torch.no_grad():
            self.sampling_offsets.weight.zero_()
            self.sampling_offsets.bias = nn.Parameter(_star_offsets(self.n_heads, self.n_levels, self.n_points))
            self.attention_weights.weight.zero_()
            self.attention_weights.bias.zero_()
            nn.init.xavier_uniform_(self.value_proj.weight)
            self.value_proj.bias.zero_()
            nn.init.xavier_uniform_(self.output_proj.weight)
            self.output_proj.bias.zero_()

    def forward(self, query, reference_points, input_flatten, input_spatial_shapes,
                input_level_start_index, input_padding_mask=None, chain_input=False):
        N, Lq, _ = query.shape
        S = input_flatten.shape[1]
        M, L, P = self.n_heads, self.n_levels, self.n_points
        _check_token_count(input_spatial_shapes, S)

        wide = _WIDE_CROSS_VALUE and input_flatten.is_cuda and input_flatten.dtype == torch.bfloat16 and Lq * 8 <= S
        if chain_input:
            value, input_next = token_linear_skip(input_flatten, self.value_proj.weight, self.value_proj.bias, wide_out=wide)
        else:
            value, input_next = token_linear(input_flatten, self.value_proj.weight, self.value_proj.bias, wide_out=wide), input_flatten
        if input_padding_mask is not None:
            value = value.masked_fill(input_padding_mask[..., None], 0.0)
        value = value.view(N, S, M, -1)

        if reference_points.shape[-1] not in (2, 6):
            raise ValueError("Last dim of reference_points must be 2 or 4, but get {} instead.".format(
                reference_points.shape[-1]))
        packed = offsets = logits = None
        if _FUSED_PROLOGUE and _PACKED_PROJECTION and not torch.is_autocast_enabled():
            packed = token_linear(query, *self._packed_projection())
        else:
            offsets = token_linear(query, self.sampling_offsets.weight, self.sampling_offsets.bias).view(N, Lq, M, L, P, 2)
            logits = token_linear(query, self.attention_weights.weight, self.attention_weights.bias).view(N, Lq, M, L * P)
        out = self._attend(value, packed, offsets, logits, reference_points, input_spatial_shapes, input_level_start_index, query.dtype)
        return (out, input_next) if chain_input else out

    def _packed_projection(self):
        return (torch.cat((self.sampling_offsets.weight, self.attention_weights.weight), 0),
                torch.cat((self.sampling_offsets.bias, self.attention_weights.bias), 0))

    def _attend(self, value, packed, offsets, logits, reference_points, input_spatial_shapes, input_level_start_index, out_dtype):
        N, S = value.shape[:2]
        M, L, P = self.n_heads, self.n_levels, self.n_points
        Lq = (packed if packed is not None else offsets).shape[1]
        if packed is not None and not msda_prologue_ext.packed_supported(packed, reference_points, L, P):
            offsets, logits = packed[..., :M * L * P * 2].reshape(N, Lq, M, L, P, 2), packed[..., M * L * P * 2:].reshape(N, Lq, M, L * P)
            packed = None
        if packed is not None:
            locations, weights = msda_prologue_ext.msda_prologue_packed(packed, reference_points, input_spatial_shapes, M, L, P)
        elif _FUSED_PROLOGUE and msda_prologue_ext.supported(offsets, logits, reference_points):
            locations, weights = msda_prologue_ext.msda_prologue(offsets, logits, reference_points, input_spatial_shapes)
        else:
            weights = F.softmax(logits, -1).view(N, Lq, M, L, P)
            ref = reference_points[:, :, None, :, None, :]
            if reference_points.shape[-1] == 2:
                wh = input_spatial_shapes.flip(-1)
                locations = ref + offsets / wh[None, None, None, :, None, :]
            else:
                extent = ref[..., 2::2] + ref[..., 3::2]
                locations = ref[..., :2] + offsets / P * extent * 0.5

        out = MSDeformAttnFunction.apply(value, input_spatial_shapes, input_level_start_index,
                                         locations, weights, self.im2col_step)
        out = _cut.at("msda", out, when_armed=True)
        if out.dtype != out_dtype and out_dtype == torch.bfloat16:
            out = out.to(out_dtype)
        return token_linear(out, self.output_proj.weight, self.output_proj.bias)

    def forward_self(self, src, pos, reference_points, input_spatial_shapes, input_level_start_index, input_padding_mask=None):
        if not (_FUSED_PROLOGUE and _PACKED_PROJECTION and src.is_cuda and not torch.is_autocast_enabled()
                and reference_points.shape[-1] in (2, 6)):
            return self.forward(src if pos is None else src + pos, reference_points, src, input_spatial_shapes,
                                input_level_start_index, input_padding_mask), _cut.at("msda", src, when_armed=True)
        N, S, _ = src.shape
        _check_token_count(input_spatial_shapes, S)
        value, src1 = token_linear_skip(src, self.value_proj.weight, self.value_proj.bias)
        if input_padding_mask is not None:
            value = value.masked_fill(input_padding_mask[..., None], 0.0)
        packed, src2 = token_linear_skip(src1, *self._packed_projection(), pos=pos)
        out = self._attend(value.view(N, S, self.n_heads, -1), packed, None, None, reference_points, input_spatial_shapes,
                           input_level_start_index, src.dtype)
        return out, _cut.at("msda", src2, when_armed=True)


class MSDeformAttn_cross(MSDeformAttn):

    def __init__(self, d_model=256, n_levels=4, n_heads=8, n_points=4):
        super().__init__(d_model, n_levels, n_heads, n_points, conditional=True)


MultiheadAttention = nn.MultiheadAttention
```

monodetr_amd/tgemm_ext.py:

```python
import torch

from . import _capi

_backend = None
RELU, NN, BIAS_F32, OUT_F32 = 1, 2, 4, 8


def _lib():
    return _backend if _backend is not None else _capi.lib()


def _rows_ok(t, cols):
    q = 4 if t.dtype == torch.float32 else 8
    return t.dim() == 2 and t.shape[1] == cols and t.stride(1) == 1 and t.stride(0) % q == 0 and t.stride(0) >= cols and t.data_ptr() % 16 == 0 \
        and (t.dtype != torch.float32 or t.shape[0] * t.stride(0) < 2 ** 29)


def supported(a2, w, nn=False, res=None, bias=None, out=None):
    if not ((a2.is_cuda or _backend is not None) and a2.dtype == w.dtype and a2.dtype in (torch.bfloat16, torch.float32) and a2.dim() == 2 and w.dim() == 2):
        return False
    if a2.dtype == torch.float32:
        return _supported_f32(a2, w, nn, res, bias, out)
    T, K = a2.shape
    N = w.shape[1] if nn else w.shape[0]
    if not (T > 0 and K % 8 == 0 and N % 8 == 0 and (w.shape[0] if nn else w.shape[1]) == K and _rows_ok(a2, K) and _rows_ok(w, w.shape[1])):
        return False
    if res is not None and not (res.dtype == torch.bfloat16 and tuple(res.shape) == (T, N) and _rows_ok(res, N)):
        return False
    if out is not None and not (out.dtype in (torch.bfloat16, torch.float32) and tuple(out.shape) == (T, N) and out.stride(1) == 1
                                and out.stride(0) % 8 == 0 and out.data_ptr() % 16 == 0):
        return False
    if bias is not None and not (bias.dim() == 1 and bias.shape[0] == N and bias.is_contiguous() and bias.data_ptr() % 16 == 0
                                 and bias.dtype in (torch.bfloat16, torch.float32)):
        return False
    return True


def _supported_f32(a2, w, nn, res, bias, out):
    T, K = a2.shape
    N = w.shape[1] if nn else w.shape[0]
    if not (T > 0 and K % 8 == 0 and N % 8 == 0 and (w.shape[0] if nn else w.shape[1]) == K and _rows_ok(a2, K) and _rows_ok(w, w.shape[1])
            and T * N < 2 ** 29):
        return False
    if res is not None and not (res.dtype == torch.float32 and tuple(res.shape) == (T, N) and _rows_ok(res, N)):
        return False
    if out is not None and not (out.dtype == torch.float32 and tuple(out.shape) == (T, N) and _rows_ok(out, N)):
        return False
    if bias is not None and not (bias.dim() == 1 and bias.shape[0] == N and bias.is_contiguous() and bias.data_ptr() % 16 == 0
                                 and bias.dtype == torch.float32):
        return False
    return True


def tgemm(a2, w, bias=None, res=None, relu=False, nn=False, out=None, out_dtype=None, dropout_p=0.0, seed=0, seed_dev=None):
    T, K = a2.shape
    N = w.shape[1] if nn else w.shape[0]
    f32 = a2.dtype == torch.float32
    if out is None:
        out = torch.empty((T, N), dtype=(a2.dtype if out_dtype is None else out_dtype), device=a2.device)
    if f32:
        if out.dtype != torch.float32:
            raise ValueError("tgemm: fp32 operands give an fp32 result")
        rc = _lib().mdetr_tgemm_f32(
            a2.data_ptr(), w.data_ptr(), bias.data_ptr() if bias is not None else None, res.data_ptr() if res is not None else None,
            out.data_ptr(), T, N, K, a2.stride(0), w.stride(0), res.stride(0) if res is not None else 0, out.stride(0),
            (RELU if relu else 0) | (NN if nn else 0), float(dropout_p), int(seed), seed_dev.data_ptr() if seed_dev is not None else None,
            a2.device.index if a2.is_cuda else -1, torch.cuda.current_stream(a2.device).cuda_stream if a2.is_cuda else None)
        if rc != 0:
            _capi.check(rc, "mdetr_tgemm_f32")
        return out
    flags = (RELU if relu else 0) | (NN if nn else 0) | (BIAS_F32 if bias is not None and bias.dtype == torch.float32 else 0) \
        | (OUT_F32 if out.dtype == torch.float32 else 0)
    rc = _lib().mdetr_tgemm(
        a2.data_ptr(), w.data_ptr(), bias.data_ptr() if bias is not None else None, res.data_ptr() if res is not None else None,
        out.data_ptr(), T, N, K, a2.stride(0), w.stride(0), res.stride(0) if res is not None else 0, out.stride(0), flags,
        float(dropout_p), int(seed), seed_dev.data_ptr() if seed_dev is not None else None,
        a2.device.index if a2.is_cuda else -1, torch.cuda.current_stream(a2.device).cuda_stream if a2.is_cuda else None)
    if rc != 0:
        _capi.check(rc, "mdetr_tgemm")
    return out


def masked_supported(a2, w, mask, res=None):
    if not supported(a2, w, nn=True, res=res):
        return False
    return mask.dtype == a2.dtype and tuple(mask.shape) == (a2.shape[0], w.shape[1]) and _rows_ok(mask, w.shape[1])


def tgemm_masked(a2, w, mask, res=None):
    T, K = a2.shape
    N = w.shape[1]
    out = torch.empty((T, N), dtype=a2.dtype, device=a2.device)
    f32 = a2.dtype == torch.float32
    name = "mdetr_tgemm_f32_masked" if f32 else "mdetr_tgemm_masked"
    rc = getattr(_lib(), name)(
        a2.data_ptr(), w.data_ptr(), res.data_ptr() if res is not None else None, mask.data_ptr(), out.data_ptr(), T, N, K,
        a2.stride(0), w.stride(0), res.stride(0) if res is not None else 0, mask.stride(0), out.stride(0),
        a2.device.index if a2.is_cuda else -1, torch.cuda.current_stream(a2.device).cuda_stream if a2.is_cuda else None)
    if rc != 0:
        _capi.check(rc, name)
    return out
```

Measured before the change: 485.8 images/sec.

## Fuse output projection GEMM with residual add and LayerNorm epilogue

Adds a tgemm variant whose epilogue owns whole 256-wide rows and applies bias, dropout-scaled residual add and LayerNorm in-register. It writes y, the pre-norm sum s and per-row stats for backward. The MSDA output projection in the encoder self-attention path now routes through it, so the separate linear output and add+LayerNorm kernel pass with their extra HBM round trip are skipped. The kernel also gains a configurable K slab depth (32 or 64). The cost is a heavier epilogue and a tile shape fixed at N=256, which may reduce occupancy and adds a new numerics path.

```diff
diff --git a/include/monodetr_amd.h b/include/monodetr_amd.h
--- a/include/monodetr_amd.h
+++ b/include/monodetr_amd.h
@@ -7,7 +7,7 @@
 extern "C" {
 #endif
 
-#define MDETR_ABI_VERSION 13
+#define MDETR_ABI_VERSION 14
 
 #define MDETR_F32 0
 #define MDETR_F64 1
@@ -157,6 +157,9 @@
                     const void *seed_dev, int device, void *stream);
 int mdetr_tgemm_f32_masked(const void *a, const void *w, const void *res, const void *mask, void *y, int64_t T, int N, int K,
                            int64_t lda, int64_t ldw, int64_t ldr, int64_t ldm, int64_t ldy, int device, void *stream);
+int mdetr_tgemm_ln(const void *a, const void *w, const void *bias, const void *res, void *y, int64_t T, int N, int K,
+                   int64_t lda, int64_t ldw, int64_t ldr, int64_t ldy, int flags, const void *gamma, const void *beta, int param_dtype,
+                   void *s, float *stats, float eps, float dropout_p, uint64_t seed, const void *seed_dev, int device, void *stream);
 
 #define MDETR_SGEMM_NT 0
 #define MDETR_SGEMM_NN 1
diff --git a/monodetr_amd/_capi.py b/monodetr_amd/_capi.py
--- a/monodetr_amd/_capi.py
+++ b/monodetr_amd/_capi.py
@@ -6,7 +6,7 @@
 LIB_PATH = os.environ.get("MDETR_LIB_PATH") or os.path.join(_HERE, "libmonodetr_amd.so")
 
 MDETR_F32, MDETR_F64, MDETR_BF16 = 0, 1, 2
-ABI_VERSION = 13
+ABI_VERSION = 14
 
 _c_int, _c_vp = ctypes.c_int, ctypes.c_void_p
 
@@ -41,6 +41,8 @@
     "mdetr_tgemm_masked": (_c_int, [_c_vp] * 5 + [ctypes.c_int64, _c_int, _c_int] + [ctypes.c_int64] * 5 + [_c_int, _c_vp]),
     "mdetr_tgemm_f32": (_c_int, [_c_vp] * 5 + [ctypes.c_int64, _c_int, _c_int] + [ctypes.c_int64] * 4 + [_c_int, ctypes.c_float, ctypes.c_uint64, _c_vp, _c_int, _c_vp]),
     "mdetr_tgemm_f32_masked": (_c_int, [_c_vp] * 5 + [ctypes.c_int64, _c_int, _c_int] + [ctypes.c_int64] * 5 + [_c_int, _c_vp]),
+    "mdetr_tgemm_ln": (_c_int, [_c_vp] * 5 + [ctypes.c_int64, _c_int, _c_int] + [ctypes.c_int64] * 4 + [_c_int, _c_vp, _c_vp, _c_int, _c_vp, _c_vp, ctypes.c_float,
+                                ctypes.c_float, ctypes.c_uint64, _c_vp, _c_int, _c_vp]),
     "mdetr_column_sum_workspace_bytes": (ctypes.c_int64, [ctypes.c_int64, _c_int]),
     "mdetr_column_sum": (_c_int, [_c_int, _c_vp, _c_vp, _c_vp, ctypes.c_int64, ctypes.c_int64, _c_int, ctypes.c_int64, _c_int, _c_vp]),
     "mdetr_box_refine": (_c_int, [_c_vp] * 3 + [ctypes.c_int64, _c_int, _c_int, _c_vp]),
diff --git a/monodetr_amd/add_ln_ext.py b/monodetr_amd/add_ln_ext.py
--- a/monodetr_amd/add_ln_ext.py
+++ b/monodetr_amd/add_ln_ext.py
@@ -78,23 +78,29 @@
     @torch.autograd.function.once_differentiable
     def backward(ctx, dy):
         s, gp, stats = ctx.saved_tensors
-        io, pcode, rows, C, p, seed, shape, g_dtype, b_dtype = ctx.meta
-        dy2 = _rows(dy, C)
-        da, db = torch.empty_like(s), torch.empty_like(s)
-        lib = _lib()
-        nb = lib.mdetr_add_layernorm_partial_rows(rows)
-        partial = torch.empty((nb, 2 * C), dtype=torch.float32, device=s.device)
-        dev, stream = _dev(s)
-        rc = lib.mdetr_add_layernorm_backward(io, pcode, dy2.data_ptr(), s.data_ptr(), gp.data_ptr(), stats.data_ptr(), da.data_ptr(), db.data_ptr(),
-                                              partial.data_ptr(), rows, C, p, seed,
-                                              ctx.seed_dev.data_ptr() if ctx.seed_dev is not None else None, dev, stream)
-        if rc != 0:
-            _capi.check(rc, "mdetr_add_layernorm_backward")
-        sums = _column_sum_f32(partial, g_dtype if g_dtype == b_dtype else torch.float32)
-        return da.view(shape), db.view(shape), sums[:C].to(g_dtype), sums[C:].to(b_dtype), None, None, None, None
+        shape, g_dtype, b_dtype = ctx.meta[6:]
+        da, db, dg, dbeta = _backward_launch(dy, s, gp, stats, ctx.meta, ctx.seed_dev)
+        return da.view(shape), db.view(shape), dg, dbeta, None, None, None, None
 
 
-def fused_add_layernorm(a, b, gamma, beta, eps=1e-5, dropout_p=0.0, seed=None):
+def _backward_launch(dy, s, gp, stats, meta, seed_dev):
+    io, pcode, rows, C, p, seed, _, g_dtype, b_dtype = meta
+    dy2 = _rows(dy, C)
+    da, db = torch.empty_like(s), torch.empty_like(s)
+    lib = _lib()
+    nb = lib.mdetr_add_layernorm_partial_rows(rows)
+    partial = torch.empty((nb, 2 * C), dtype=torch.float32, device=s.device)
+    dev, stream = _dev(s)
+    rc = lib.mdetr_add_layernorm_backward(io, pcode, dy2.data_ptr(), s.data_ptr(), gp.data_ptr(), stats.data_ptr(), da.data_ptr(), db.data_ptr(),
+                                          partial.data_ptr(), rows, C, p, seed,
+                                          seed_dev.data_ptr() if seed_dev is not None else None, dev, stream)
+    if rc != 0:
+        _capi.check(rc, "mdetr_add_layernorm_backward")
+    sums = _column_sum_f32(partial, g_dtype if g_dtype == b_dtype else torch.float32)
+    return da, db, sums[:C].to(g_dtype), sums[C:].to(b_dtype)
+
+
+def draw_seed(a, dropout_p, seed=None):
     seed_dev = None
     if dropout_p > 0.0 and seed is None:
         if a.is_cuda and torch.cuda.is_current_stream_capturing():
@@ -102,7 +108,12 @@
             seed, seed_dev = site_seed(a.device)
         else:
             seed = _host_seed()
-    return _AddLayerNorm.apply(a, b, gamma, beta, eps, dropout_p, seed or 0, seed_dev)
+    return seed or 0, seed_dev
+
+
+def fused_add_layernorm(a, b, gamma, beta, eps=1e-5, dropout_p=0.0, seed=None):
+    seed, seed_dev = draw_seed(a, dropout_p, seed)
+    return _AddLayerNorm.apply(a, b, gamma, beta, eps, dropout_p, seed, seed_dev)
 
 
 def residual_layernorm(a, b, norm, dropout):
diff --git a/monodetr_amd/csrc/add_ln.hip b/monodetr_amd/csrc/add_ln.hip
--- a/monodetr_amd/csrc/add_ln.hip
+++ b/monodetr_amd/csrc/add_ln.hip
@@ -59,28 +59,17 @@
     if (b) {
         float r[E];
         load_row<T, E>(b + at, r);
-#pragma unroll
-        for (int i = 0; i < E; ++i) {
-            const bool keep = thresh == 0u || ln_hash(sd, static_cast<uint64_t>(at + i)) >= thresh;
-            v[i] += keep ? r[i] * keep_scale : 0.f;
-        }
+        ln_row_mix<E>(v, r, thresh, keep_scale, sd, static_cast<uint64_t>(at));
         if (s) {
             store_row<T, E>(s + at, v);
 #pragma unroll
             for (int i = 0; i < E; ++i) { T t; st1<T>(&t, v[i]); v[i] = ld1<T>(&t); }
         }
     }
-    float sum = 0.f;
-#pragma unroll
-    for (int i = 0; i < E; ++i) sum += v[i];
-    const float mean = wave_sum(sum) * (1.0f / C);
-    float sq = 0.f;
-#pragma unroll
-    for (int i = 0; i < E; ++i) { const float d = v[i] - mean; sq += d * d; }
-    const float rstd = 1.0f / sqrtf(wave_sum(sq) * (1.0f / C) + eps);
-    float o[E];
-#pragma unroll
-    for (int i = 0; i < E; ++i) o[i] = (v[i] - mean) * rstd * ld1<PT>(gamma + lane * E + i) + ld1<PT>(beta + lane * E + i);
+    float gam[E], bet[E], o[E], mean, rstd;
+#pragma unroll
+    for (int i = 0; i < E; ++i) { gam[i] = ld1<PT>(gamma + lane * E + i); bet[i] = ld1<PT>(beta + lane * E + i); }
+    ln_row_normalize<E>(v, gam, bet, eps, [](float x) { return wave_sum(x); }, o, mean, rstd);
     store_row<T, E>(y + at, o);
     if (lane == 0) { stats[2 * row] = mean; stats[2 * row + 1] = rstd; }
 }
diff --git a/monodetr_amd/csrc/add_ln_math.h b/monodetr_amd/csrc/add_ln_math.h
--- a/monodetr_amd/csrc/add_ln_math.h
+++ b/monodetr_amd/csrc/add_ln_math.h
@@ -1,4 +1,5 @@
 #pragma once
+#include <math.h>
 #include <stdint.h>
 
 #if defined(__HIPCC__)
@@ -27,4 +28,37 @@
     return t >= 4294967295.0 ? 0xFFFFFFFFu : static_cast<uint32_t>(t);
 }
 
+template <int E>
+MDETR_HD void ln_row_mix(float (&v)[E], const float (&r)[E], uint32_t thresh, float keep_scale, uint64_t sd, uint64_t at)
+{
+#if defined(__clang__)
+#pragma clang fp contract(off)
+#endif
+#pragma unroll
+    for (int i = 0; i < E; ++i) {
+        const bool keep = thresh == 0u || ln_hash(sd, at + static_cast<uint64_t>(i)) >= thresh;
+        v[i] += keep ? r[i] * keep_scale : 0.f;
+    }
 }
+
+template <int E, typename WaveSum>
+MDETR_HD void ln_row_normalize(const float (&v)[E], const float (&gam)[E], const float (&bet)[E], float eps, WaveSum wave_sum,
+                               float (&o)[E], float &mean, float &rstd)
+{
+#if defined(__clang__)
+#pragma clang fp contract(off)
+#endif
+    constexpr int C = 64 * E;
+    float sum = 0.f;
+#pragma unroll
+    for (int i = 0; i < E; ++i) sum += v[i];
+    mean = wave_sum(sum) * (1.0f / C);
+    float sq = 0.f;
+#pragma unroll
+    for (int i = 0; i < E; ++i) { const float d = v[i] - mean; sq = fmaf(d, d, sq); }
+    rstd = 1.0f / sqrtf(fmaf(wave_sum(sq), 1.0f / C, eps));
+#pragma unroll
+    for (int i = 0; i < E; ++i) o[i] = fmaf((v[i] - mean) * rstd, gam[i], bet[i]);
+}
+
+}
diff --git a/monodetr_amd/csrc/capi.hip b/monodetr_amd/csrc/capi.hip
--- a/monodetr_amd/csrc/capi.hip
+++ b/monodetr_amd/csrc/capi.hip
@@ -570,6 +570,30 @@
     return MDETR_OK;
 }
 
+int mdetr_tgemm_ln(const void *a, const void *w, const void *bias, const void *res, void *y, int64_t T, int N, int K,
+                   int64_t lda, int64_t ldw, int64_t ldr, int64_t ldy, int flags, const void *gamma, const void *beta, int param_dtype,
+                   void *s, float *stats, float eps, float dropout_p, uint64_t seed, const void *seed_dev, int device, void *stream)
+{
+    if (T < 0 || N <= 0 || K <= 0) return fail(MDETR_E_ARG, "mdetr_tgemm_ln: bad shape T=%lld N=%d K=%d", static_cast<long long>(T), N, K);
+    if (N != 256) return fail(MDETR_E_ARG, "mdetr_tgemm_ln: N = %d (the tile owns whole rows of 256)", N);
+    if (param_dtype != MDETR_F32 && param_dtype != MDETR_BF16) return fail(MDETR_E_ARG, "mdetr_tgemm_ln: param_dtype %d (MDETR_F32 or MDETR_BF16)", param_dtype);
+    if (flags & ~MDETR_TGEMM_BIAS_F32) return fail(MDETR_E_ARG, "mdetr_tgemm_ln: flag bits 0x%x (MDETR_TGEMM_BIAS_F32 only)", flags);
+    if (!(dropout_p >= 0.f && dropout_p < 1.f)) return fail(MDETR_E_ARG, "mdetr_tgemm_ln: dropout_p = %g outside [0, 1)", static_cast<double>(dropout_p));
+    if (T == 0) return MDETR_OK;
+    if (!a || !w || !res || !y || !s || !stats || !gamma || !beta) return fail(MDETR_E_ARG, "mdetr_tgemm_ln: null pointer");
+    mdetr::TgemmProblem p{a, w, bias, res, y, T, N, K, lda, ldw, ldr, ldy, flags, dropout_p, seed, static_cast<const uint64_t *>(seed_dev)};
+    p.ln = true; p.gamma = gamma; p.beta = beta; p.ln_param_f32 = param_dtype == MDETR_F32; p.s = s; p.stats = stats; p.eps = eps;
+    if (!mdetr::tgemm_supported(p))
+        return fail(MDETR_E_ARG, "mdetr_tgemm_ln: needs bf16 operands, K %% 8 == 0, row strides %% 8 == 0 and >= the row length, ldy == 256, 16-byte aligned "
+                    "pointers, res distinct from y and s (T=%lld N=%d K=%d lda=%lld ldw=%lld ldr=%lld ldy=%lld flags=0x%x)", static_cast<long long>(T), N, K,
+                    static_cast<long long>(lda), static_cast<long long>(ldw), static_cast<long long>(ldr), static_cast<long long>(ldy), flags);
+    DeviceScope dev(device);
+    if (dev.err != hipSuccess) return fail(MDETR_E_HIP, "mdetr_tgemm_ln: set device %d: %s", device, hipGetErrorString(dev.err));
+    const hipError_t e = mdetr::tgemm_launch(p, static_cast<hipStream_t>(stream));
+    if (e != hipSuccess) return fail(MDETR_E_HIP, "mdetr_tgemm_ln: launch failed: %s", hipGetErrorString(e));
+    return MDETR_OK;
+}
+
 int mdetr_tgemm_f32(const void *a, const void *w, const void *bias, const void *res, void *y, int64_t T, int N, int K,
                     int64_t lda, int64_t ldw, int64_t ldr, int64_t ldy, int flags, float dropout_p, uint64_t seed,
                     const void *seed_dev, int device, void *stream)
diff --git a/monodetr_amd/csrc/tgemm.h b/monodetr_amd/csrc/tgemm.h
--- a/monodetr_amd/csrc/tgemm.h
+++ b/monodetr_amd/csrc/tgemm.h
@@ -22,6 +22,12 @@
     const void *mask = nullptr;
     int64_t ldm = 0;
     bool f32 = false;
+    bool ln = false;
+    const void *gamma = nullptr, *beta = nullptr;
+    bool ln_param_f32 = false;
+    void *s = nullptr;
+    float *stats = nullptr;
+    float eps = 0.f;
 };
 
 bool tgemm_supported(const TgemmProblem &p);
diff --git a/monodetr_amd/csrc/tgemm.hip b/monodetr_amd/csrc/tgemm.hip
--- a/monodetr_amd/csrc/tgemm.hip
+++ b/monodetr_amd/csrc/tgemm.hip
@@ -30,12 +30,18 @@
     float keep_scale;
     uint64_t seed;
     const uint64_t *seed_dev;
+    const void *gamma, *beta;
+    __bf16 *s;
+    float *stats;
+    float eps;
 };
 
-template <int BM, int BN>
+constexpr int kTgemmLnParamF32 = 16;
+
+template <int BM, int BN, int BK = kBK>
 constexpr size_t tgemm_lds()
 {
-    constexpr size_t slabs = static_cast<size_t>(2) * (BM + BN) * kLd * 2, tile = static_cast<size_t>(BM) * (BN + kCPad) * 4;
+    constexpr size_t slabs = static_cast<size_t>(2) * (BM + BN) * (BK + 8) * 2, tile = static_cast<size_t>(BM) * (BN + kCPad) * 4;
     return slabs > tile ? slabs : tile;
 }
 
@@ -60,18 +66,22 @@
 #define TG_MARK(i) do { } while (0)
 #endif
 
-template <int BM, int BN, bool NN, int PF, int TAIL, int NTH = 256>
+template <int BM, int BN, bool NN, int PF, int TAIL, int NTH = 256, int BKT = 64>
 __global__ __launch_bounds__(NTH, NTH == 512 ? 4 : 2)
 void tgemm_kernel(const TgemmArgs g)
 {
     TG_MARK(0);
     constexpr int kThreadsT = NTH;
+    constexpr int kBK = BKT, kLd = BKT + 8;
+    constexpr int PK = kBK / 8, PKS = kBK == 64 ? 3 : 2;
     constexpr int WNW = NTH / 128;
     constexpr int TM = BM / 64, TN = BN / (32 * WNW);
-    constexpr int XCH = BM * 8 / kThreadsT;
-    constexpr int WCH = NN ? 4 : BN * 8 / kThreadsT;
+    constexpr int XCH = BM * PK / kThreadsT;
+    constexpr int WCH = NN ? 4 : BN * PK / kThreadsT;
     constexpr int WTHR = NN ? 2 * BN : kThreadsT;
     static_assert(TM >= 1 && TN >= 1 && XCH >= 1 && WCH >= 1 && WTHR <= kThreadsT, "tile / workgroup shape");
+    static_assert((kBK == 64 || (kBK == 32 && !NN)) && kThreadsT % PK == 0, "slab depth");
+    static_assert(TAIL != 4 || (!NN && BN == 256 && BM % (NTH / 64) == 0), "the LayerNorm tail owns whole rows of 256");
     MDETR_DYNAMIC_LDS(unsigned char, tg_smem);
     __bf16 *Xs = reinterpret_cast<__bf16 *>(tg_smem);
     __bf16 *Ws = Xs + 2 * BM * kLd;
@@ -96,14 +106,14 @@
     const unsigned a_bytes = static_cast<unsigned>(((g.T - 1) * g.lda + g.K) * 2);
     const unsigned w_bytes = static_cast<unsigned>(NN ? ((static_cast<int64_t>(g.K) - 1) * g.ldw + g.N) * 2 : ((static_cast<int64_t>(g.N) - 1) * g.ldw + g.K) * 2);
     const mdetr_rsrc ar = make_rsrc(g.a, a_bytes), wr_ = make_rsrc(g.w, w_bytes);
-    const int xk = (tid & 7) * 8;
+    const int xk = (tid & (PK - 1)) * 8;
     const int wkg = tid & 15, wnb = tid >> 4;
     unsigned xoff[XCH], woff[NN ? 1 : WCH];
     int xdst[XCH], wdst[NN ? 1 : WCH];
 #pragma unroll
     for (int j = 0; j < XCH; ++j) {
         const int c = tid + kThreadsT * j;
-        xdst[j] = (c >> 3) * kLd + (c & 7) * 8;
+        xdst[j] = (c >> PKS) * kLd + (c & (PK - 1)) * 8;
     }
     if (NN) {
         wdst[0] = wnb * 8 * kLd + wkg * 4;
@@ -111,7 +121,7 @@
 #pragma unroll
         for (int j = 0; j < (NN ? 1 : WCH); ++j) {
             const int c = tid + kThreadsT * j;
-            wdst[j] = (c >> 3) * kLd + (c & 7) * 8;
+            wdst[j] = (c >> PKS) * kLd + (c & (PK - 1)) * 8;
         }
     }
     auto aim = [&](int v) __attribute__((always_inline)) {
@@ -121,16 +131,16 @@
 #pragma unroll
         for (int j = 0; j < XCH; ++j) {
             const int c = tid + kThreadsT * j;
-            const int64_t t = m0 + (c >> 3);
-            xoff[j] = t < g.T ? (static_cast<unsigned>(t) * static_cast<unsigned>(g.lda) + (c & 7) * 8) * 2u : kRsrcOob;
+            const int64_t t = m0 + (c >> PKS);
+            xoff[j] = t < g.T ? (static_cast<unsigned>(t) * static_cast<unsigned>(g.lda) + (c & (PK - 1)) * 8) * 2u : kRsrcOob;
         }
         if (NN) {
             woff[0] = (tid < WTHR && n0 + wnb * 8 < g.N) ? static_cast<unsigned>((static_cast<int64_t>(wkg * 4) * g.ldw + n0 + wnb * 8) * 2) : kRsrcOob;
         } else {
 #pragma unroll
             for (int j = 0; j < (NN ? 1 : WCH); ++j) {
-                const int c = tid + kThreadsT * j, row = n0 + (c >> 3);
-                woff[j] = row < g.N ? (static_cast<unsigned>(row) * static_cast<unsigned>(g.ldw) + (c & 7) * 8) * 2u : kRsrcOob;
+                const int c = tid + kThreadsT * j, row = n0 + (c >> PKS);
+                woff[j] = row < g.N ? (static_cast<unsigned>(row) * static_cast<unsigned>(g.ldw) + (c & (PK - 1)) * 8) * 2u : kRsrcOob;
             }
         }
     };
@@ -309,6 +319,72 @@
         }
     };
 
+    constexpr bool LN = TAIL == 4;
+    constexpr int NWV = kThreadsT / 64, LNR = LN ? BM / NWV : 1;
+    bf16x4 aq[LNR];
+    const uint64_t sd_ln = LN ? g.seed + (g.seed_dev ? *g.seed_dev : 0ull) : 0ull;
+    auto aim_ln = [&]() __attribute__((always_inline)) {
+#pragma unroll
+        for (int j = 0; j < LNR; ++j) {
+            int64_t t = tail_m0 + j * NWV + wave;
+            t = t < g.T ? t : g.T - 1;
+            aq[j] = *reinterpret_cast<const bf16x4 *>(g.res + t * g.ldr + lane * 4);
+        }
+    };
+    auto drain_ln = [&]() __attribute__((always_inline)) {
+        float bl[4], gam[4], bet[4];
+#pragma unroll
+        for (int i = 0; i < 4; ++i) bl[i] = 0.f;
+        if (g.bias) {
+            if (g.flags & kTgemmBiasF32) {
+#pragma unroll
+                for (int i = 0; i < 4; ++i) bl[i] = static_cast<const float *>(g.bias)[lane * 4 + i];
+            } else {
+                const bf16x4 b4 = *reinterpret_cast<const bf16x4 *>(static_cast<const __bf16 *>(g.bias) + lane * 4);
+#pragma unroll
+                for (int i = 0; i < 4; ++i) bl[i] = static_cast<float>(b4[i]);
+            }
+        }
+        if (g.flags & kTgemmLnParamF32) {
+#pragma unroll
+            for (int i = 0; i < 4; ++i) { gam[i] = static_cast<const float *>(g.gamma)[lane * 4 + i]; bet[i] = static_cast<const float *>(g.beta)[lane * 4 + i]; }
+        } else {
+            const bf16x4 g4 = *reinterpret_cast<const bf16x4 *>(static_cast<const __bf16 *>(g.gamma) + lane * 4);
+            const bf16x4 b4 = *reinterpret_cast<const bf16x4 *>(static_cast<const __bf16 *>(g.beta) + lane * 4);
+#pragma unroll
+            for (int i = 0; i < 4; ++i) { gam[i] = static_cast<float>(g4[i]); bet[i] = static_cast<float>(b4[i]); }
+        }
+#pragma unroll
+        for (int j = 0; j < LNR; ++j) {
+            const int row = j * NWV + wave;
+            const int64_t t = tail_m0 + row;
+            if (t >= g.T) continue;
+            const f32x4 c = *reinterpret_cast<const f32x4 *>(Cs + row * (BN + kCPad) + lane * 4);
+            float r[4] = {c.x + bl[0], c.y + bl[1], c.z + bl[2], c.w + bl[3]}, v[4], o[4], mean, rstd;
+#pragma unroll
+            for (int i = 0; i < 4; ++i) {
+                r[i] = static_cast<float>(static_cast<__bf16>(r[i]));
+                v[i] = static_cast<float>(aq[j][i]);
+            }
+            const int64_t at = t * BN + lane * 4;
+            ln_row_mix<4>(v, r, g.thresh, g.keep_scale, sd_ln, static_cast<uint64_t>(at));
+            bf16x4 sv, ov;
+#pragma unroll
+            for (int i = 0; i < 4; ++i) { sv[i] = static_cast<__bf16>(v[i]); v[i] = static_cast<float>(sv[i]); }
+            *reinterpret_cast<bf16x4 *>(g.s + t * g.ldy + lane * 4) = sv;
+            ln_row_normalize<4>(v, gam, bet, g.eps, [](float x) __attribute__((always_inline)) {
+#pragma unroll
+                for (int o_ = 32; o_ > 0; o_ >>= 1) x += __shfl_xor(x, o_);
+                return x;
+            }, o, mean, rstd);
+#pragma unroll
+            for (int i = 0; i < 4; ++i) ov[i] = static_cast<__bf16>(o[i]);
+            *reinterpret_cast<bf16x4 *>(static_cast<__bf16 *>(g.y) + t * g.ldy + lane * 4) = ov;
+            if (lane == 0) { g.stats[2 * t] = mean; g.stats[2 * t + 1] = rstd; }
+            if (j & 1) __builtin_amdgcn_sched_barrier(0);
+        }
+    };
+
     int cv = next_tile(static_cast<int>(blockIdx.x));
     if (cv >= vtiles) return;
     int ck = 0, fv = cv, fk = 0;
@@ -348,16 +424,20 @@
             TG_MARK(7 + 3 * (s + p));
             ++ck;
             if (last) {
-                aim_tail(cv);
+                if constexpr (LN) { int col_; tile_of(cv, col_, tail_m0); } else aim_tail(cv);
                 park();
                 TG_MARK(40);
                 if (MASK) {
                     __builtin_amdgcn_sched_barrier(0);
                     aim_mask();
                 }
+                if constexpr (LN) {
+                    __builtin_amdgcn_sched_barrier(0);
+                    aim_ln();
+                }
                 __syncthreads();
                 TG_MARK(41);
-                drain();
+                if constexpr (LN) drain_ln(); else drain();
                 TG_MARK(42);
                 cv = next_tile(cv + G);
                 if (cv >= vtiles) return;
@@ -372,13 +452,13 @@
     }
 }
 
-template <int BM, int BN, bool NN, int PF, int TAIL, int NTH = 256>
+template <int BM, int BN, bool NN, int PF, int TAIL, int NTH = 256, int BKT = 64>
 hipError_t launch_tile(TgemmArgs g, hipStream_t st)
 {
-    constexpr size_t lds = tgemm_lds<BM, BN>();
+    constexpr size_t lds = tgemm_lds<BM, BN, BKT>();
     static_assert(lds <= 80 * 1024, "two workgroups per CU");
     constexpr int kThreadsT = NTH;
-    auto kern = tgemm_kernel<BM, BN, NN, PF, TAIL, NTH>;
+    auto kern = tgemm_kernel<BM, BN, NN, PF, TAIL, NTH, BKT>;
     static bool attr_set[64] = {};
     int dev_ = 0;
     if (hipGetDevice(&dev_) != hipSuccess) dev_ = -1;
@@ -835,9 +915,12 @@
 
 bool tgemm_supported(const TgemmProblem &p)
 {
-    if (p.f32) return tgemm32_supported(p);
+    if (p.f32) return !p.ln && tgemm32_supported(p);
     const auto al = [](const void *q) { return (reinterpret_cast<uintptr_t>(q) & 15) == 0; };
     const bool nn = (p.flags & kTgemmNN) != 0;
+    if (p.ln && !(p.N == 256 && !(p.flags & ~kTgemmBiasF32) && p.res && p.ldy == p.N && !p.mask && p.gamma && p.beta && p.s && p.stats && al(p.gamma) &&
+                  al(p.beta) && al(p.s) && (reinterpret_cast<uintptr_t>(p.stats) & 7) == 0 && p.res != p.y && p.res != p.s))
+        return false;
     return p.T > 0 && p.T < (1ll << 31) - 256 && p.N > 0 && p.N % 8 == 0 && p.K > 0 && p.K % 8 == 0 && p.a && p.w && p.y && al(p.a) && al(p.w) &&
            al(p.y) && p.lda % 8 == 0 && p.lda >= p.K && p.ldw % 8 == 0 && p.ldw >= (nn ? p.N : p.K) &&
            p.ldy % ((p.flags & kTgemmOutF32) ? 4 : 8) == 0 && p.ldy >= p.N &&
@@ -859,6 +942,13 @@
     g.thresh = p.dropout_p > 0.f ? ln_threshold(p.dropout_p) : 0u;
     g.keep_scale = p.dropout_p > 0.f ? 1.f / (1.f - p.dropout_p) : 1.f;
     g.seed = p.seed; g.seed_dev = p.seed_dev;
+    g.gamma = p.gamma; g.beta = p.beta; g.s = static_cast<__bf16 *>(p.s); g.stats = p.stats; g.eps = p.eps;
+    if (p.ln) {
+        if (p.ln_param_f32) g.flags |= kTgemmLnParamF32;
+        ProfileScope prof(10, conv_mflop(p.T, static_cast<int64_t>(p.N) * p.K), st, 2.0 * p.T * p.N * p.K / 1e6,
+                          (2.0 * p.T * p.K + 3.0 * 2.0 * p.T * p.N + 8.0 * p.T + 2.0 * p.N * p.K) / 1e3);
+        return tune_int("tgemm_pf", 0) == 1 ? launch_tile<64, 256, false, 1, 4, 256, 32>(g, st) : launch_tile<64, 256, false, 2, 4, 256, 32>(g, st);
+    }
     const bool generic_tail = (p.flags & (kTgemmBiasF32 | kTgemmOutF32)) != 0 || p.dropout_p > 0.f;
     const auto wgs = [&](int m, int n) { return ((p.T + m - 1) / m) * ((p.N + n - 1) / n); };
     int bm = 64, bn = 64;
diff --git a/monodetr_amd/monodetr/attention.py b/monodetr_amd/monodetr/attention.py
--- a/monodetr_amd/monodetr/attention.py
+++ b/monodetr_amd/monodetr/attention.py
@@ -5,7 +5,7 @@
 from torch import nn
 
 from ..attn_ext import fused_attention
-from .linear import Linear, split_rows, token_linear
+from .linear import Linear, linear_residual_layernorm, split_rows, token_linear
 
 
 def _sdpa(q, k, v, num_heads, dropout_p, key_padding_mask):
@@ -62,10 +62,14 @@
         (Wq, Wk, Wv), (bq, bk, bv) = split_rows(W, E, E, E), split_rows(b, E, E, E)
         return token_linear(query, Wq, bq), token_linear(key, Wk, bk), token_linear(value, Wv, bv)
 
-    def forward_batch_first(self, query, key, value, key_padding_mask=None):
+    def forward_batch_first(self, query, key, value, key_padding_mask=None, residual=None):
         q, k, v = self.project(query, key, value)
         p = self.dropout if self.training else 0.0
-        return self.out_proj(attention_core(q, k, v, self.num_heads, p, key_padding_mask))
+        core = attention_core(q, k, v, self.num_heads, p, key_padding_mask)
+        if residual is not None:
+            a, norm, dropout = residual
+            return linear_residual_layernorm(core, self.out_proj.weight, self.out_proj.bias, a, norm, dropout)
+        return self.out_proj(core)
 
     def forward(self, query, key, value, key_padding_mask=None, need_weights=False, attn_mask=None):
         if attn_mask is not None:
diff --git a/monodetr_amd/monodetr/depth_predictor/transformer.py b/monodetr_amd/monodetr/depth_predictor/transformer.py
--- a/monodetr_amd/monodetr/depth_predictor/transformer.py
+++ b/monodetr_amd/monodetr/depth_predictor/transformer.py
@@ -5,7 +5,7 @@
 
 from ...add_ln_ext import residual_layernorm
 from ..attention import MultiheadAttention
-from ..linear import Linear, ffn_hidden
+from ..linear import Linear, ffn_hidden, linear_residual_layernorm
 
 
 def _get_clones(module, N):
@@ -35,16 +35,15 @@
     def forward(self, src, src_key_padding_mask, pos):
         qk = src if pos is None else src + pos
         src = residual_layernorm(src, self.self_attn(qk, qk, src, key_padding_mask=src_key_padding_mask)[0], self.norm1, self.dropout1)
-        ff = self.linear2(ffn_hidden(src, self.linear1, self.dropout, self.activation, tokenwise=False))
-        return residual_layernorm(src, ff, self.norm2, self.dropout2)
+        h = ffn_hidden(src, self.linear1, self.dropout, self.activation, tokenwise=False)
+        return linear_residual_layernorm(h, self.linear2.weight, self.linear2.bias, src, self.norm2, self.dropout2)
 
 
     def forward_batch_first(self, src, src_key_padding_mask, pos):
         qk = src if pos is None else src + pos
-        attn = self.self_attn.forward_batch_first(qk, qk, src, key_padding_mask=src_key_padding_mask)
-        src = residual_layernorm(src, attn, self.norm1, self.dropout1)
-        ff = self.linear2(ffn_hidden(src, self.linear1, self.dropout, self.activation, tokenwise=False))
-        return residual_layernorm(src, ff, self.norm2, self.dropout2)
+        src = self.self_attn.forward_batch_first(qk, qk, src, key_padding_mask=src_key_padding_mask, residual=(src, self.norm1, self.dropout1))
+        h = ffn_hidden(src, self.linear1, self.dropout, self.activation, tokenwise=False)
+        return linear_residual_layernorm(h, self.linear2.weight, self.linear2.bias, src, self.norm2, self.dropout2)
 
 
 class TransformerEncoder(nn.Module):
diff --git a/monodetr_amd/monodetr/depthaware_transformer.py b/monodetr_amd/monodetr/depthaware_transformer.py
--- a/monodetr_amd/monodetr/depthaware_transformer.py
+++ b/monodetr_amd/monodetr/depthaware_transformer.py
@@ -14,7 +14,7 @@
 from .. import _tune
 
 _CHAIN_MEMORY = _tune.get("decoder_chain", "1") != "0"
-from .linear import Linear, ffn_hidden, token_linear
+from .linear import Linear, ffn_hidden, linear_residual_layernorm, token_linear
 from .ops.modules import MSDeformAttn, MSDeformAttn_cross, MultiheadAttention
 
 
@@ -149,12 +149,11 @@
 
     def forward_ffn(self, src):
         h, src = ffn_hidden(src, self.linear1, self.dropout2, self.activation, skip=True)
-        ff = token_linear(h, self.linear2.weight, self.linear2.bias)
-        return residual_layernorm(src, ff, self.norm2, self.dropout3)
+        return linear_residual_layernorm(h, self.linear2.weight, self.linear2.bias, src, self.norm2, self.dropout3)
 
     def forward(self, src, pos, reference_points, spatial_shapes, level_start_index, padding_mask=None):
-        attn, src = self.self_attn.forward_self(src, pos, reference_points, spatial_shapes, level_start_index, padding_mask)
-        return self.forward_ffn(residual_layernorm(src, attn, self.norm1, self.dropout1))
+        return self.forward_ffn(self.self_attn.forward_self(src, pos, reference_points, spatial_shapes, level_start_index, padding_mask,
+                                                            residual_norm=(self.norm1, self.dropout1)))
 
 
 class VisualEncoder(nn.Module):
@@ -230,8 +229,8 @@
         return tensor if pos is None else tensor + pos
 
     def forward_ffn(self, tgt):
-        ff = self.linear2(ffn_hidden(tgt, self.linear1, self.dropout3, self.activation, tokenwise=False))
-        return residual_layernorm(tgt, ff, self.norm3, self.dropout4)
+        h = ffn_hidden(tgt, self.linear1, self.dropout3, self.activation, tokenwise=False)
+        return linear_residual_layernorm(h, self.linear2.weight, self.linear2.bias, tgt, self.norm3, self.dropout4)
 
     def _self_attention_inputs(self, x):
         w, b = _SummedPair.apply(self.sa_qcontent_proj.weight, self.sa_qpos_proj.weight, self.sa_kcontent_proj.weight, self.sa_kpos_proj.weight,
@@ -244,8 +243,7 @@
                 depth_pos_embed_ip=None, pos_embeds=None, self_attn_mask=None, query_pos_un=None, chain_src=False):
         B, Nq, C = tgt.shape
         depth_tokens = depth_pos_embed.transpose(0, 1)
-        d = self.cross_attn_depth.forward_batch_first(tgt, depth_tokens, depth_tokens, mask_depth)
-        tgt = residual_layernorm(tgt, d, self.norm_depth, self.dropout_depth)
+        tgt = self.cross_attn_depth.forward_batch_first(tgt, depth_tokens, depth_tokens, mask_depth, residual=(tgt, self.norm_depth, self.dropout_depth))
         q, k = self._self_attention_inputs(self.with_pos_embed(tgt, query_pos))
         v = tgt
         if self.training and self.group_num > 1:
@@ -253,13 +251,12 @@
                 raise ValueError("training expects num_queries * group_num queries, got %d for %d groups" % (Nq, self.group_num))
             n = Nq // self.group_num
             q, k, v = (t.reshape(B * self.group_num, n, C) for t in (q, k, v))
-        s = self.self_attn.forward_batch_first(q, k, v).reshape(B, Nq, C)
-        tgt = residual_layernorm(tgt, s, self.norm2, self.dropout2)
+        tgt = self.self_attn.forward_batch_first(q, k, v, residual=(tgt, self.norm2, self.dropout2))
         c = self.cross_attn(self.with_pos_embed(tgt, query_pos), reference_points, src, src_spatial_shapes,
-                            level_start_index, src_padding_mask, chain_input=chain_src)
+                            level_start_index, src_padding_mask, chain_input=chain_src, residual=(tgt, self.norm1, self.dropout1))
         if chain_src:
             c, src = c
-        tgt = residual_layernorm(tgt, c, self.norm1, self.dropout1)
+        tgt = c
         return (self.forward_ffn(tgt), src) if chain_src else self.forward_ffn(tgt)
 
 
diff --git a/monodetr_amd/monodetr/linear.py b/monodetr_amd/monodetr/linear.py
--- a/monodetr_amd/monodetr/linear.py
+++ b/monodetr_amd/monodetr/linear.py
@@ -307,6 +307,60 @@
     return _SplitRows.apply(packed, *sizes)
 
 
+_LN_TAIL_MIN_TOKENS = _MIN_TOKENS
+
+
+def _ln_tail_enabled():
+    from .. import _tune, add_ln_ext
+    return _TGEMM and add_ln_ext.ENABLED and _tune.get("ln_tail", "1") != "0"
+
+
+class _LinearResidualLayerNorm(torch.autograd.Function):
+
+    @staticmethod
+    def forward(ctx, x, weight, bias, a, gamma, beta, eps, p, seed, seed_dev):
+        from .. import _capi, tgemm_ext
+        C = a.shape[-1]
+        x2, a2 = x.reshape(-1, x.shape[-1]), a.reshape(-1, C)
+        y, s, stats = tgemm_ext.tgemm_ln(x2, weight, bias, a2, gamma, beta, eps, p, seed, seed_dev)
+        ctx.save_for_backward(x, weight, s, gamma, stats)
+        ctx.seed_dev = seed_dev
+        ctx.has_bias = bias is not None
+        ctx.bias_dtype = bias.dtype if bias is not None else None
+        pcode = _capi.MDETR_BF16 if gamma.dtype == torch.bfloat16 else _capi.MDETR_F32
+        ctx.meta = (_capi.MDETR_BF16, pcode, a2.shape[0], C, float(p), int(seed), a.shape, gamma.dtype, beta.dtype)
+        return y.view(a.shape)
+
+    @staticmethod
+    @torch.autograd.function.once_differentiable
+    def backward(ctx, dy):
+        from .. import add_ln_ext
+        x, weight, s, gamma, stats = ctx.saved_tensors
+        da, db2, dg, dbeta = add_ln_ext._backward_launch(dy, s, gamma, stats, ctx.meta, ctx.seed_dev)
+        x2 = x.reshape(-1, x.shape[-1])
+        dx = _input_gradient(db2, weight).view_as(x) if ctx.needs_input_grad[0] else None
+        dw, dbias = _weight_bias_grads(x2, db2, weight, ctx.needs_input_grad[1], ctx.has_bias and ctx.needs_input_grad[2], ctx.bias_dtype)
+        return dx, dw, dbias, da.view(ctx.meta[6]), dg, dbeta, None, None, None, None
+
+
+def linear_residual_layernorm(x, weight, bias, a, norm, dropout, seed=None):
+    from .. import add_ln_ext
+    if _ln_tail_enabled() and (x.is_cuda or _tgemm_backend()) and x.dtype == weight.dtype == a.dtype == torch.bfloat16 \
+            and a.shape[-1] == weight.shape[0] == 256 and a.numel() // 256 == x.numel() // x.shape[-1] >= max(_MIN_TOKENS, _LN_TAIL_MIN_TOKENS) \
+            and torch.is_grad_enabled() and (x.requires_grad or weight.requires_grad or a.requires_grad) and not torch.is_autocast_enabled() \
+            and add_ln_ext.supported(a, a, norm):
+        from .. import tgemm_ext
+        x2, a2 = x.reshape(-1, x.shape[-1]), a.reshape(-1, 256)
+        if _tgemm_ok(x2, weight, bias, a2) and tgemm_ext.ln_supported(x2, weight, a2, bias, norm.weight, norm.bias):
+            p = dropout.p if (dropout is not None and dropout.training) else 0.0
+            seed, seed_dev = add_ln_ext.draw_seed(a, p, seed)
+            return _LinearResidualLayerNorm.apply(x, weight, bias, a, norm.weight, norm.bias, norm.eps, p, seed, seed_dev)
+    b = token_linear(x, weight, bias).reshape(a.shape)
+    if seed is not None and add_ln_ext.ENABLED and add_ln_ext.supported(a, b, norm):
+        return add_ln_ext.fused_add_layernorm(a, b, norm.weight, norm.bias, norm.eps, dropout.p if (dropout is not None and dropout.training) else 0.0, seed)
+    return add_ln_ext.residual_layernorm(a, b, norm, dropout)
+
+
 def _kernel_relu(x, weight, bias=None):
     if _tgemm_ok(x.reshape(-1, x.shape[-1]), weight, bias):
         return True
diff --git a/monodetr_amd/monodetr/ops/modules/ms_deform_attn.py b/monodetr_amd/monodetr/ops/modules/ms_deform_attn.py
--- a/monodetr_amd/monodetr/ops/modules/ms_deform_attn.py
+++ b/monodetr_amd/monodetr/ops/modules/ms_deform_attn.py
@@ -8,7 +8,8 @@
 
 from ..functions import MSDeformAttnFunction
 from ... import _cut
-from ...linear import Linear, token_linear, token_linear_skip
+from ...linear import Linear, linear_residual_layernorm, token_linear, token_linear_skip
+from ....add_ln_ext import residual_layernorm
 from .... import msda_prologue_ext
 
 
@@ -72,7 +73,7 @@
             self.output_proj.bias.zero_()
 
     def forward(self, query, reference_points, input_flatten, input_spatial_shapes,
-                input_level_start_index, input_padding_mask=None, chain_input=False):
+                input_level_start_index, input_padding_mask=None, chain_input=False, residual=None):
         N, Lq, _ = query.shape
         S = input_flatten.shape[1]
         M, L, P = self.n_heads, self.n_levels, self.n_points
@@ -96,14 +97,14 @@
         else:
             offsets = token_linear(query, self.sampling_offsets.weight, self.sampling_offsets.bias).view(N, Lq, M, L, P, 2)
             logits = token_linear(query, self.attention_weights.weight, self.attention_weights.bias).view(N, Lq, M, L * P)
-        out = self._attend(value, packed, offsets, logits, reference_points, input_spatial_shapes, input_level_start_index, query.dtype)
+        out = self._attend(value, packed, offsets, logits, reference_points, input_spatial_shapes, input_level_start_index, query.dtype, residual)
         return (out, input_next) if chain_input else out
 
     def _packed_projection(self):
         return (torch.cat((self.sampling_offsets.weight, self.attention_weights.weight), 0),
                 torch.cat((self.sampling_offsets.bias, self.attention_weights.bias), 0))
 
-    def _attend(self, value, packed, offsets, logits, reference_points, input_spatial_shapes, input_level_start_index, out_dtype):
+    def _attend(self, value, packed, offsets, logits, reference_points, input_spatial_shapes, input_level_start_index, out_dtype, residual=None):
         N, S = value.shape[:2]
         M, L, P = self.n_heads, self.n_levels, self.n_points
         Lq = (packed if packed is not None else offsets).shape[1]
@@ -129,19 +130,28 @@
         out = _cut.at("msda", out, when_armed=True)
         if out.dtype != out_dtype and out_dtype == torch.bfloat16:
             out = out.to(out_dtype)
+        if residual is not None:
+            a, norm, dropout = residual
+            return linear_residual_layernorm(out, self.output_proj.weight, self.output_proj.bias, a() if callable(a) else a, norm, dropout)
         return token_linear(out, self.output_proj.weight, self.output_proj.bias)
 
-    def forward_self(self, src, pos, reference_points, input_spatial_shapes, input_level_start_index, input_padding_mask=None):
+    def forward_self(self, src, pos, reference_points, input_spatial_shapes, input_level_start_index, input_padding_mask=None, residual_norm=None):
+        if residual_norm is not None:
+            norm, dropout = residual_norm
         if not (_FUSED_PROLOGUE and _PACKED_PROJECTION and src.is_cuda and not torch.is_autocast_enabled()
                 and reference_points.shape[-1] in (2, 6)):
-            return self.forward(src if pos is None else src + pos, reference_points, src, input_spatial_shapes,
-                                input_level_start_index, input_padding_mask), _cut.at("msda", src, when_armed=True)
+            out, src_next = self.forward(src if pos is None else src + pos, reference_points, src, input_spatial_shapes,
+                                         input_level_start_index, input_padding_mask), _cut.at("msda", src, when_armed=True)
+            return (out, src_next) if residual_norm is None else residual_layernorm(src_next, out, norm, dropout)
         N, S, _ = src.shape
         _check_token_count(input_spatial_shapes, S)
         value, src1 = token_linear_skip(src, self.value_proj.weight, self.value_proj.bias)
         if input_padding_mask is not None:
             value = value.masked_fill(input_padding_mask[..., None], 0.0)
         packed, src2 = token_linear_skip(src1, *self._packed_projection(), pos=pos)
+        if residual_norm is not None:
+            return self._attend(value.view(N, S, self.n_heads, -1), packed, None, None, reference_points, input_spatial_shapes,
+                                input_level_start_index, src.dtype, (lambda: _cut.at("msda", src2, when_armed=True), norm, dropout))
         out = self._attend(value.view(N, S, self.n_heads, -1), packed, None, None, reference_points, input_spatial_shapes,
                            input_level_start_index, src.dtype)
         return out, _cut.at("msda", src2, when_armed=True)
diff --git a/monodetr_amd/tgemm_ext.py b/monodetr_amd/tgemm_ext.py
--- a/monodetr_amd/tgemm_ext.py
+++ b/monodetr_amd/tgemm_ext.py
@@ -100,3 +100,28 @@
     if rc != 0:
         _capi.check(rc, name)
     return out
+
+
+def ln_supported(a2, w, res, bias, gamma, beta):
+    if not (a2.dtype == torch.bfloat16 and w.dim() == 2 and w.shape[0] == 256 and res is not None and supported(a2, w, res=res, bias=bias)):
+        return False
+    return gamma.dtype == beta.dtype and gamma.dtype in (torch.bfloat16, torch.float32) and tuple(gamma.shape) == (256,) == tuple(beta.shape) \
+        and gamma.is_contiguous() and beta.is_contiguous() and gamma.data_ptr() % 16 == 0 and beta.data_ptr() % 16 == 0
+
+
+def tgemm_ln(a2, w, bias, res, gamma, beta, eps=1e-5, dropout_p=0.0, seed=0, seed_dev=None):
+    T, K = a2.shape
+    N = w.shape[0]
+    y = torch.empty((T, N), dtype=a2.dtype, device=a2.device)
+    s = torch.empty_like(y)
+    stats = torch.empty((T, 2), dtype=torch.float32, device=a2.device)
+    flags = BIAS_F32 if bias is not None and bias.dtype == torch.float32 else 0
+    rc = _lib().mdetr_tgemm_ln(
+        a2.data_ptr(), w.data_ptr(), bias.data_ptr() if bias is not None else None, res.data_ptr(), y.data_ptr(), T, N, K,
+        a2.stride(0), w.stride(0), res.stride(0), y.stride(0), flags, gamma.data_ptr(), beta.data_ptr(),
+        _capi.MDETR_BF16 if gamma.dtype == torch.bfloat16 else _capi.MDETR_F32, s.data_ptr(), stats.data_ptr(), float(eps),
+        float(dropout_p), int(seed), seed_dev.data_ptr() if seed_dev is not None else None,
+        a2.device.index if a2.is_cuda else -1, torch.cuda.current_stream(a2.device).cuda_stream if a2.is_cuda else None)
+    if rc != 0:
+        _capi.check(rc, "mdetr_tgemm_ln")
+    return y, s, stats
```

After: 476.9 images/sec. 0.982x the previous value.
